# jnbraun/bcnn

Measured on AMD Instinct MI355X. Metric: images/sec fwd+bwd, higher is better.
Workload: dtype f32; 1 GPU; ResNet-18 224x224 (BASELINE configs[2]), N=128 per GPU, fwd+bwd+SGD through bcnn_net C API; CIFAR-example topology + ImageNet stem, fc-1000; batch_per_gpu=128, global_batch=128, parallelism=dp1, comm=none (one rank)

## Files before the change

### bcnn_amd/_lib.py

```python
import ctypes as C
import os
import subprocess

_HERE = os.path.dirname(os.path.abspath(__file__))
LIB_PATH = os.environ.get("BCNN_HIP_LIB", os.path.join(_HERE, "lib", "libbcnn_hip.so"))
CSRC = os.path.join(_HERE, "csrc")

vp, i, f, sz, u64 = C.c_void_p, C.c_int, C.c_float, C.c_size_t, C.c_uint64

SIGNATURES = {
    "bcnn_hip_device_count": (i, []),
    "bcnn_hip_set_device": (None, [i]),
    "bcnn_hip_get_device": (i, []),
    "bcnn_hip_device_name": (C.c_char_p, []),
    "bcnn_hip_malloc_f32": (vp, [sz]),
    "bcnn_hip_malloc_i32": (vp, [sz]),
    "bcnn_hip_free": (None, [vp]),
    "bcnn_hip_memcpy_h2d": (None, [vp, vp, sz]),
    "bcnn_hip_memcpy_d2h": (None, [vp, vp, sz]),
    "bcnn_hip_memcpy_d2d": (None, [vp, vp, sz]),
    "bcnn_hip_fill_f32": (None, [vp, sz, f]),
    "bcnn_hip_sync": (None, []),
    "bcnn_hip_stream_create": (vp, []),
    "bcnn_hip_stream_destroy": (None, [vp]),
    "bcnn_hip_set_stream": (None, [vp]),
    "bcnn_hip_get_stream": (vp, []),
    "bcnn_hip_event_create": (vp, []),
    "bcnn_hip_event_destroy": (None, [vp]),
    "bcnn_hip_event_record": (None, [vp]),
    "bcnn_hip_event_sync": (None, [vp]),
    "bcnn_hip_event_elapsed_ms": (f, [vp, vp]),
    "bcnn_hip_profile_enable": (None, [i]),
    "bcnn_hip_profile_reset": (None, []),
    "bcnn_hip_profile_num_classes": (i, []),
    "bcnn_hip_profile_class_name": (C.c_char_p, [i]),
    "bcnn_hip_profile_read": (None, [i, C.POINTER(C.c_double), C.POINTER(C.c_longlong), C.POINTER(C.c_double), C.POINTER(C.c_double)]),
    "bcnn_hip_profile_read_useful_flops": (C.c_double, [i]),
    "bcnn_hip_conv_side_stream_mode": (i, [i]),
    "bcnn_hip_conv_side_join": (None, []),
    "bcnn_hip_trace_enable": (None, [i]),
    "bcnn_hip_trace_read": (C.c_size_t, [C.c_char_p, C.c_size_t]),
    "bcnn_hip_axpy": (None, [sz, f, vp, vp]),
    "bcnn_hip_scal": (None, [sz, f, vp]),
    "bcnn_hip_copy_f32": (None, [sz, vp, vp]),
    "bcnn_hip_add_bias": (None, [vp, vp, i, i, i]),
    "bcnn_hip_grad_bias": (None, [vp, vp, i, i, i]),
    "bcnn_hip_scales": (None, [vp, vp, i, i, i]),
    "bcnn_hip_grad_scales": (None, [vp, vp, i, i, i, vp]),
    "bcnn_hip_gemm": (None, [i, i, i, i, i, f, vp, i, vp, i, f, vp, i]),
    "bcnn_hip_im2col": (None, [vp, i, i, i, i, i, i, vp]),
    "bcnn_hip_col2im": (None, [vp, i, i, i, i, i, i, vp]),
    "bcnn_hip_activation_forward": (None, [vp, sz, i, vp, i, i]),
    "bcnn_hip_activation_backward": (None, [vp, vp, sz, i, vp, vp, i, i]),
    "bcnn_hip_batchnorm_forward": (None, [vp] * 10 + [i, i, i, i, i]),
    "bcnn_hip_batchnorm_backward": (None, [vp, vp, vp, i] + [vp] * 9 + [i, i, i]),
    "bcnn_hip_conv_workspace_size": (sz, [i] * 9),
    "bcnn_hip_conv_forward": (None, [vp, vp, vp, vp] + [i] * 10 + [vp, i, vp, vp, vp, vp, vp, vp, vp, i]),
    "bcnn_hip_conv_forward_bf16": (i, [vp, vp, vp, vp] + [i] * 10 + [vp, i, vp, vp, vp, vp, vp, vp, vp, i]),
    "bcnn_hip_conv_backward": (None, [vp] * 8 + [i] * 10 + [vp, vp, i] + [vp] * 8 + [vp, sz]),
    "bcnn_hip_maxpool_forward": (None, [vp, vp, vp] + [i] * 8),
    "bcnn_hip_maxpool_backward": (None, [vp, vp, vp] + [i] * 9),
    "bcnn_hip_avgpool_forward": (None, [vp, vp, i, i, i, i]),
    "bcnn_hip_avgpool_backward": (None, [vp, vp, i, i, i, i]),
    "bcnn_hip_depthwise_forward": (None, [vp, vp, vp, vp] + [i] * 8),
    "bcnn_hip_depthwise_backward": (None, [vp] * 7 + [i] * 9),
    "bcnn_hip_depthwise_stats_size": (sz, [i] * 7),
    "bcnn_hip_depthwise_forward_stats": (i, [vp, vp, vp, vp] + [i] * 8 + [vp, sz]),
    "bcnn_hip_batchnorm_forward_stats": (None, [vp] * 10 + [i, i, i, i, i, vp, i]),
    "bcnn_hip_batchnorm_forward_stats_only": (None, [vp] * 7 + [i, i, i, vp, i]),
    "bcnn_hip_conv_bnfold_fusable": (i, [i] * 5), "bcnn_hip_conv_set_input_bnfold": (None, [vp] * 4),
    "bcnn_hip_depthwise_bn_fusable": (i, [i] * 8),
    "bcnn_hip_batchnorm_backward_sums": (None, [vp] * 9 + [i, i, i]),
    "bcnn_hip_depthwise_backward_bn": (None, [vp] * 7 + [i] * 9 + [vp] * 5),
    "bcnn_hip_batchnorm_backward_apply": (None, [vp] * 8 + [i, i, i]),
    "bcnn_hip_depthwise_bnin_fusable": (i, [i] * 9),
    "bcnn_hip_conv_bnsums_size": (sz, [i] * 4),
    "bcnn_hip_conv_backward_bnsums": (i, [vp] * 8 + [i] * 10 + [vp, vp, i] + [vp] * 8 + [vp, sz] + [vp, vp, vp, sz]),
    "bcnn_hip_batchnorm_backward_finalize": (None, [vp, i] + [vp] * 6 + [i]),
    "bcnn_hip_depthwise_forward_bnin": (i, [vp, vp, vp, vp] + [i] * 8 + [vp, sz] + [vp] * 4 + [i]),
    "bcnn_hip_depthwise_backward_bnin": (None, [vp] * 7 + [i] * 9 + [vp] * 4 + [i]),
    "bcnn_hip_depthwise_backward_bn_bnin": (None, [vp] * 7 + [i] * 9 + [vp] * 5 + [vp] * 4 + [i]),
    "bcnn_hip_conv_residual_fusable": (i, [i, i, i, i, vp, vp, vp]),
    "bcnn_hip_conv_forward_residual": (None, [vp, vp, vp] + [i] * 9 + [vp] * 7 + [sz, i, vp]),
    "bcnn_hip_conv_backward_residual": (None, [vp] * 7 + [i] * 9 + [vp] * 7 + [vp, sz, vp, vp, i, vp, vp, sz]),
    "bcnn_hip_batchnorm_apply": (None, [vp] * 6 + [i, i, i, i]),
    "bcnn_hip_conv_prepack": (None, [vp, i, i]),
    "bcnn_hip_maxpool_forward_bn_keep": (None, [vp, vp, vp] + [i] * 8 + [vp] * 4 + [i, vp]),
    "bcnn_hip_maxpool_bn_backward_fusable": (i, [i] * 9 + [vp] * 4),
    "bcnn_hip_maxpool_bn_backward": (None, [vp] * 5 + [i] * 8 + [vp] * 8 + [i]),
    "bcnn_hip_conv_backward_bn_done": (None, [vp] * 5 + [i] * 9 + [vp, sz]),
    "bcnn_hip_depthwise_insums_size": (sz, [i] * 7),
    "bcnn_hip_depthwise_backward_bnin_sums": (i, [vp] * 7 + [i] * 9 + [vp] * 5 + [vp] * 4 + [i] + [vp, sz]),
    "bcnn_hip_conv_backward_presummed": (i, [vp] * 8 + [i] * 10 + [vp, vp, i] + [vp] * 8 + [vp, sz] + [vp, i] + [vp, vp, vp, sz]),
    "bcnn_hip_conv_prepack_reset": (None, []),
    "bcnn_hip_conv_prepack_discard": (None, []),
    "bcnn_hip_maxpool_bn_fusable": (i, [i] * 9 + [vp]),
    "bcnn_hip_conv_forward_stats_only": (None, [vp, vp, vp] + [i] * 9 + [vp] * 6),
    "bcnn_hip_maxpool_forward_bn": (None, [vp, vp, vp] + [i] * 8 + [vp] * 4 + [i]),
    "bcnn_hip_sgd_update": (None, [vp, vp, vp, vp, sz, sz, i, f, f, f]),
    "bcnn_hip_sgd_update_chunks": (None, [vp, i, i, f, f, f]),
    "bcnn_hip_zero_chunks": (None, [vp, i]),
    "bcnn_hip_adam_update": (None, [vp, vp, vp, vp, vp, vp, sz, sz, i, i, f, f, f, f, f]),
    "bcnn_hip_eltwise_forward": (None, [vp, vp, vp, sz, sz, i]),
    "bcnn_hip_eltwise_backward": (None, [vp, vp, vp, vp, sz, sz, i, i]),
    "bcnn_hip_cost_metric": (None, [i, vp, vp, vp, i, i, vp]),
    "bcnn_hip_axpy_strided": (None, [i, f, vp, vp] + [i] * 11),
    "bcnn_hip_add_rowvec": (None, [vp, vp, i, i]),
    "bcnn_hip_softmax_forward": (None, [vp, vp, i, i, i]),
    "bcnn_hip_concat_forward": (None, [i, vp, vp, vp, i, i]),
    "bcnn_hip_concat_backward": (None, [i, vp, vp, vp, i, i]),
    "bcnn_hip_upsample_forward": (None, [vp, vp, i, i, i, i, i]),
    "bcnn_hip_upsample_backward": (None, [vp, vp, i, i, i, i, i]),
    "bcnn_hip_yolo_activate": (None, [vp, vp, i, i, i, i, i]),
    "bcnn_hip_yolo_nms_capacity": (i, []),
    "bcnn_hip_yolo_detect_result_words": (sz, [i, i, i]),
    "bcnn_hip_yolo_detect_batch": (i, [vp, i, i, vp, i, i, i, i, f, i, f, i, i, vp]),
    "bcnn_hip_fill_images": (i, [vp, i, i, i, i, i, vp, vp, vp, vp, i, f, i, f, f, f]),
    "bcnn_hip_deconv_workspace_size": (sz, [i] * 8),
    "bcnn_hip_deconv_forward": (None, [vp, vp, vp, vp] + [i] * 9),
    "bcnn_hip_deconv_backward": (None, [vp] * 7 + [i] * 9 + [vp, sz]),
    "bcnn_hip_lrn_forward": (None, [vp, vp] + [i] * 5 + [f] * 3),
    "bcnn_hip_lrn_backward": (None, [vp, vp, vp] + [i] * 5 + [f] * 3 + [i]),
    "bcnn_hip_dropout_forward": (None, [vp, sz, f, u64, u64]),
    "bcnn_hip_dropout_backward": (None, [vp, sz, f, u64, u64]),
    "bcnn_hip_lifted_struct_workspace_size": (sz, [i, i]),
    "bcnn_hip_lifted_struct_forward": (None, [vp, vp, vp, i, i, f, i, vp, vp]),
    "bcnn_hip_lifted_struct_backward": (None, [vp, i, i, f, vp]),
    "bcnn_hip_comm_init": (None, [i, i, C.c_char_p]),
    "bcnn_hip_comm_destroy": (None, []),
    "bcnn_hip_comm_retain": (None, []),
    "bcnn_hip_rendezvous_publish": (i, [C.c_char_p, vp, sz, i]),
    "bcnn_hip_rendezvous_fetch": (i, [C.c_char_p, vp, sz, i, i]),
    "bcnn_hip_comm_world": (i, []),
    "bcnn_hip_comm_rank": (i, []),
    "bcnn_hip_allreduce_sum": (None, [vp, sz]),
    "bcnn_hip_broadcast": (None, [vp, sz, i]),
    "bcnn_hip_comm_join": (None, []),
}

_lib = None


def build(verbose=False):
    out = None if verbose else subprocess.DEVNULL
    subprocess.check_call(["make", "-C", CSRC, "-j8"], stdout=out)
    return LIB_PATH


def load():
    global _lib
    if _lib is not None:
        return _lib
    try:
        import torch
    except ImportError:
        pass
    if not os.path.exists(LIB_PATH):
        raise RuntimeError(
            "bcnn_amd: %s is missing -- build it with `python -c 'import __graft_entry__ as g; g.build()'` "
            "(there is no CPU fallback)" % LIB_PATH)
    lib = C.CDLL(LIB_PATH)
    for name, (res, args) in SIGNATURES.items():
        fn = getattr(lib, name)
        fn.restype = res
        fn.argtypes = args
    _lib = lib
    return lib


def declared_symbols():
    import re
    hdr = os.path.join(os.path.dirname(_HERE), "include", "bcnn_hip.h")
    text = open(hdr).read()
    text = re.sub(r"/\*.*?\*/", "", text, flags=re.S)
    return sorted(set(re.findall(r"\b(bcnn_hip_[a-z0-9_]+)\s*\(", text)))
```

### bcnn_amd/csrc/common.h

```cpp
#pragma once
#include <hip/hip_runtime.h>

#include <cstdio>
#include <cstdlib>

#include "../../include/bcnn_hip.h"

#define HIP_CHECK(expr)                                                                        \
    do {                                                                                       \
        hipError_t _e = (expr);                                                                \
        if (_e != hipSuccess) {                                                                \
            fprintf(stderr, "[bcnn_hip] %s:%d: %s failed: %s\n", __FILE__, __LINE__, #expr,    \
                    hipGetErrorString(_e));                                                    \
            exit((int)_e);                                                                     \
        }                                                                                      \
    } while (0)

#define KERNEL_CHECK() HIP_CHECK(hipGetLastError())

#ifdef BCNN_HIP_EXPERIMENT
#define BCNN_EXP_ENV(name) getenv(name)
#else
#define BCNN_EXP_ENV(name) ((const char*)nullptr)
#endif

namespace bcnn_hip {

hipStream_t current_stream();
void set_current_stream(hipStream_t st);

constexpr int kMaxDevices = 64;
int current_device();

enum ScratchSlot {
    SCRATCH_REDUCE,
    SCRATCH_BN_CONSTS,
    SCRATCH_FOLD_ROWCONST,
    SCRATCH_COL,
    SCRATCH_DMA,
    SCRATCH_DMA_DW,
    SCRATCH_WINO,
    SCRATCH_WINO_DW,
    SCRATCH_WINO43_U,
    SCRATCH_WINO43_TAIL,
    SCRATCH_WFUSED_U,
    SCRATCH_WFUSED_TAIL,
    SCRATCH_W43FF_U,
    SCRATCH_W43FF_TAIL,
    SCRATCH_DETECT,
    SCRATCH_IMAGES,
    SCRATCH_SLOTS
};
float* scratch(ScratchSlot slot, size_t floats);
inline float4* scratch_f4(ScratchSlot slot, size_t n) { return reinterpret_cast<float4*>(scratch(slot, n * 4)); }

void activation_backward_grad_bias(const float* y, float* dy, float* dbias, int n, int c, int hw, int act);

enum KClass { K_CONV_FWD = 0, K_CONV_DW, K_CONV_DX, K_BN_FWD, K_BN_BWD, K_POOL, K_ELTWISE_ACT, K_GEMM, K_SGD,
              K_DEPTHWISE_FWD, K_DEPTHWISE_BWD,
              K_CONV_FWD_WINO, K_CONV_DX_WINO, K_CONV_DW_WINO,
              K_CONV_FWD_WINO43, K_CONV_DX_WINO43,
              K_CONV_DW_WINO43,
              K_NUM };
struct KTimer {
    int idx;
    KTimer(int cls, double flops, double bytes, double useful_flops = -1.0);
    ~KTimer();
};

extern thread_local bool g_trace_on;
void trace_kernel_slow(const char* name);
inline void trace_kernel(const char* name) { if (g_trace_on) trace_kernel_slow(name); }

constexpr int kWave = 64;
constexpr int kCUs = 256;
constexpr int kXCDs = 8;

inline int ceil_div(long long a, long long b) { return (int)((a + b - 1) / b); }

#ifndef STREAM_GRID_PER_CU
#define STREAM_GRID_PER_CU 8
#endif
inline int stream_grid(size_t work_items, int block) {
    size_t need = (work_items + block - 1) / block;
    size_t cap = (size_t)kCUs * STREAM_GRID_PER_CU;
    if (need < 1) need = 1;
    return (int)(need < cap ? need : cap);
}

#ifdef __HIPCC__
__device__ __forceinline__ int xcd_remap(int bid, int nblk) {
    const int q = nblk / kXCDs, r = nblk % kXCDs;
    const int xcd = bid % kXCDs, idx = bid / kXCDs;
    const int base = (xcd < r) ? xcd * (q + 1) : r * (q + 1) + (xcd - r) * q;
    return base + idx;
}

__device__ __forceinline__ float wave_sum(float v) {
#pragma unroll
    for (int off = 32; off > 0; off >>= 1) v += __shfl_down(v, off, 64);
    return v;
}

__device__ __forceinline__ float wave_sum_dpp(float v) {
    v += __builtin_bit_cast(float, __builtin_amdgcn_update_dpp(0, __builtin_bit_cast(int, v), 0xB1, 0xf, 0xf, false));
    v += __builtin_bit_cast(float, __builtin_amdgcn_update_dpp(0, __builtin_bit_cast(int, v), 0x4E, 0xf, 0xf, false));
    v += __builtin_bit_cast(float, __builtin_amdgcn_update_dpp(0, __builtin_bit_cast(int, v), 0x141, 0xf, 0xf, false));
    v += __builtin_bit_cast(float, __builtin_amdgcn_update_dpp(0, __builtin_bit_cast(int, v), 0x140, 0xf, 0xf, false));
    v += __builtin_bit_cast(float, __builtin_amdgcn_update_dpp(0, __builtin_bit_cast(int, v), 0x142, 0xa, 0xf, false));
    v += __builtin_bit_cast(float, __builtin_amdgcn_update_dpp(0, __builtin_bit_cast(int, v), 0x143, 0xc, 0xf, false));
    return v;
}

__device__ __forceinline__ float block_sum(float v, float* red) {
    v = wave_sum(v);
    const int lane = threadIdx.x & 63, wid = threadIdx.x >> 6;
    __syncthreads();
    if (lane == 0) red[wid] = v;
    __syncthreads();
    float t = 0.f;
    if (threadIdx.x == 0) {
        const int nw = (blockDim.x + 63) >> 6;
        for (int i = 0; i < nw; ++i) t += red[i];
    }
    return t;
}

__device__ __forceinline__ float act_fwd(float x, int act, float slope) {
    switch (act) {
        case BCNN_HIP_ACT_TANH: {
            const float t = 2 * x;
            const double e = exp((double)t);
            return (float)(e - 1) / ((float)e + 1);
        }
        case BCNN_HIP_ACT_RELU: return x * (float)(x > 0);
        case BCNN_HIP_ACT_LRELU: return x > 0 ? x : 0.1f * x;
        case BCNN_HIP_ACT_RAMP: return x * (float)(x > 0) + 0.1f * x;
        case BCNN_HIP_ACT_SOFTPLUS: return (float)log((double)(1.0f + (float)exp((double)x)));
        case BCNN_HIP_ACT_ABS: return fabsf(x);
        case BCNN_HIP_ACT_CLAMP: return (x < 0) ? 0.f : ((x > 1) ? 1.f : x);
        case BCNN_HIP_ACT_LOGISTIC: return 1.0f / (1.0f + (float)exp((double)(-x)));
        case BCNN_HIP_ACT_PRELU: return x > 0 ? x : slope * x;
        default: return x;
    }
}

__host__ __device__ __forceinline__ bool act_is_cheap(int act) {
    return act != BCNN_HIP_ACT_TANH && act != BCNN_HIP_ACT_SOFTPLUS && act != BCNN_HIP_ACT_LOGISTIC;
}
__device__ __forceinline__ float act_fwd_cheap(float x, int act, float slope) {
    switch (act) {
        case BCNN_HIP_ACT_RELU: return x * (float)(x > 0);
        case BCNN_HIP_ACT_LRELU: return x > 0 ? x : 0.1f * x;
        case BCNN_HIP_ACT_RAMP: return x * (float)(x > 0) + 0.1f * x;
        case BCNN_HIP_ACT_ABS: return fabsf(x);
        case BCNN_HIP_ACT_CLAMP: return (x < 0) ? 0.f : ((x > 1) ? 1.f : x);
        case BCNN_HIP_ACT_PRELU: return x > 0 ? x : slope * x;
        default: return x;
    }
}
__device__ __forceinline__ float act_bwd_cheap(float y, int act, float slope) {
    switch (act) {
        case BCNN_HIP_ACT_TANH: return 1 - y * y;
        case BCNN_HIP_ACT_RELU: return (float)(y > 0);
        case BCNN_HIP_ACT_LRELU: return y > 0 ? 1.0f : 0.1f;
        case BCNN_HIP_ACT_RAMP: return (float)(y > 0) + 0.1f;
        case BCNN_HIP_ACT_ABS: return y >= 0 ? 1.0f : -1.0f;
        case BCNN_HIP_ACT_CLAMP: return (float)(y > 0.0f && y < 1.0f);
        case BCNN_HIP_ACT_LOGISTIC: return (1 - y) * y;
        case BCNN_HIP_ACT_PRELU: return y > 0 ? 1.0f : slope;
        default: return 1.0f;
    }
}
__host__ __device__ __forceinline__ bool act_bwd_is_cheap(int act) { return act != BCNN_HIP_ACT_SOFTPLUS; }

__device__ __forceinline__ float act_bwd_factor(float y, int act, float slope) {
    switch (act) {
        case BCNN_HIP_ACT_TANH: return 1 - y * y;
        case BCNN_HIP_ACT_RELU: return (float)(y > 0);
        case BCNN_HIP_ACT_LRELU: return y > 0 ? 1.0f : 0.1f;
        case BCNN_HIP_ACT_RAMP: return (float)(y > 0) + 0.1f;
        case BCNN_HIP_ACT_SOFTPLUS: return 1.0f / (1.0f + (float)exp((double)(-y)));
        case BCNN_HIP_ACT_ABS: return y >= 0 ? 1.0f : -1.0f;
        case BCNN_HIP_ACT_CLAMP: return (float)(y > 0.0f && y < 1.0f);
        case BCNN_HIP_ACT_LOGISTIC: return (1 - y) * y;
        case BCNN_HIP_ACT_PRELU: return y > 0 ? 1.0f : slope;
        default: return 1.0f;
    }
}
#endif

}
```

### bcnn_amd/csrc/conv.hip

```cpp
#include "batchnorm.h"
#include "conv_paths.h"
#include <algorithm>
#include <cstring>
#include <vector>

namespace bcnn_hip {
static thread_local BnFold g_fold_pending = {nullptr, nullptr, nullptr, nullptr};
static BnFold take_fold() {
    const BnFold f = g_fold_pending;
    g_fold_pending = BnFold{nullptr, nullptr, nullptr, nullptr};
    return f;
}
static bool bnfold_shape_ok(const ConvShape& s) {
    return s.ksz == 1 && s.stride == 1 && s.pad == 0 && s.groups == 1 && conv_dma_fwd_wanted(s) &&
           conv_dw_dma_workspace_floats(s) > 0;
}
__global__ __launch_bounds__(256) void bnfold_rowconst_kernel(const float* __restrict__ w, const BnFold fold, int F, int C,
                                                              float* __restrict__ rowc) {
    const int f = blockIdx.x * 4 + (threadIdx.x >> 6), lane = threadIdx.x & 63;
    if (f >= F) return;
    double acc = 0.0;
    for (int c = lane; c < C; c += 64) {
        float bv = fold.bias[c];
        if (bv == 1.0f) bv = 0.f;
        const float b = bv - fold.mean[c] * bnfold_a(fold.var, fold.scales, c);
        acc += (double)w[(size_t)f * C + c] * (double)b;
    }
#pragma unroll
    for (int o = 32; o > 0; o >>= 1) acc += __shfl_xor(acc, o);
    if (lane == 0) rowc[f] = (float)acc;
}
static float* fold_rowconst(const BnFold& fold, const float* w, int C, int F) {
    float* rowc = scratch(SCRATCH_FOLD_ROWCONST, (size_t)F);
    bnfold_rowconst_kernel<<<ceil_div(F, 4), 256, 0, current_stream()>>>(w, fold, F, C, rowc);
    KERNEL_CHECK();
    return rowc;
}


struct SideStream {
    hipStream_t stream = nullptr;
    hipEvent_t ready = nullptr, done = nullptr;
    bool pending = false;
};
static thread_local SideStream g_side[kMaxDevices];
static thread_local int g_side_mode = 0;
bool conv_side_stream_deferred() { return g_side_mode == 2; }
static SideStream* side_stream() {
    SideStream& ss = g_side[current_device()];
    if (ss.stream == nullptr) {
        int prio_lo = 0, prio_hi = 0;
        HIP_CHECK(hipDeviceGetStreamPriorityRange(&prio_lo, &prio_hi));
        HIP_CHECK(hipStreamCreateWithPriority(&ss.stream, hipStreamNonBlocking, BCNN_EXP_ENV("BCNN_HIP_SIDE_PRIO_SAME") ? prio_hi : prio_lo));
        HIP_CHECK(hipEventCreateWithFlags(&ss.ready, hipEventDisableTiming));
        HIP_CHECK(hipEventCreateWithFlags(&ss.done, hipEventDisableTiming));
    }
    return &ss;
}

struct PrepackEntry {
    const float* w;
    int kind, mode;
    float* buf;
    size_t cap, floats;
    unsigned long long epoch;
    bool fresh;
};
struct PrepackStore {
    std::vector<PrepackEntry> entries;
    unsigned long long epoch = 0;
    int dev = -1;
    void* table_dev[PREPACK_KINDS][2] = {{nullptr, nullptr}, {nullptr, nullptr}};
    size_t table_cap[PREPACK_KINDS][2] = {{0, 0}, {0, 0}};
    std::vector<char> table_host[PREPACK_KINDS][2];
};
static thread_local PrepackStore g_prepack;

float* prepack_take(const float* w, int kind, int mode, size_t floats) {
    PrepackStore& st = g_prepack;
    for (PrepackEntry& e : st.entries)
        if (e.w == w && e.kind == kind && e.mode == mode && e.fresh && e.epoch == st.epoch && e.floats == floats) {
            e.fresh = false;
            return e.buf;
        }
    return nullptr;
}

static void prepack_free_all(PrepackStore& st) {
    HIP_CHECK(hipDeviceSynchronize());
    for (PrepackEntry& e : st.entries)
        if (e.buf) HIP_CHECK(hipFree(e.buf));
    st.entries.clear();
    for (int k = 0; k < PREPACK_KINDS; ++k)
        for (int m = 0; m < 2; ++m) {
            if (st.table_dev[k][m]) HIP_CHECK(hipFree(st.table_dev[k][m]));
            st.table_dev[k][m] = nullptr;
            st.table_cap[k][m] = 0;
            st.table_host[k][m].clear();
        }
}

static PrepackEntry* prepack_entry(PrepackStore& st, const float* w, int kind, int mode, size_t floats) {
    PrepackEntry* e = nullptr;
    for (PrepackEntry& c : st.entries)
        if (c.w == w && c.kind == kind && c.mode == mode) { e = &c; break; }
    if (!e) {
        st.entries.push_back(PrepackEntry{w, kind, mode, nullptr, 0, 0, 0, false});
        e = &st.entries.back();
    }
    if (e->cap < floats) {
        if (e->buf) {
            HIP_CHECK(hipStreamSynchronize(current_stream()));
            HIP_CHECK(hipFree(e->buf));
        }
        HIP_CHECK(hipMalloc((void**)&e->buf, floats * sizeof(float)));
        e->cap = floats;
    }
    e->floats = floats;
    e->epoch = st.epoch;
    e->fresh = true;
    return e;
}

static const void* prepack_table(PrepackStore& st, int kind, int mode, const void* jobs, size_t bytes) {
    std::vector<char>& host = st.table_host[kind][mode];
    if (host.size() == bytes && memcmp(host.data(), jobs, bytes) == 0) return st.table_dev[kind][mode];
    HIP_CHECK(hipStreamSynchronize(current_stream()));
    if (st.table_cap[kind][mode] < bytes) {
        if (st.table_dev[kind][mode]) HIP_CHECK(hipFree(st.table_dev[kind][mode]));
        HIP_CHECK(hipMalloc(&st.table_dev[kind][mode], bytes * 2));
        st.table_cap[kind][mode] = bytes * 2;
    }
    HIP_CHECK(hipMemcpy(st.table_dev[kind][mode], jobs, bytes, hipMemcpyHostToDevice));
    host.assign((const char*)jobs, (const char*)jobs + bytes);
    return st.table_dev[kind][mode];
}

enum ConvGate { GATE_NONE, GATE_WINDOW, GATE_DMA, GATE_SMALLC_DX, GATE_COUNT };
static bool gate_open(ConvGate g) {
    static const bool off[GATE_COUNT] = {false, BCNN_EXP_ENV("BCNN_HIP_NO_WINDOW") != nullptr,
                                         BCNN_EXP_ENV("BCNN_HIP_NO_DMA") != nullptr,
                                         BCNN_EXP_ENV("BCNN_HIP_NO_SMALLC_DX") != nullptr};
    return !off[g];
}
struct ConvPack {
    bool (*wino)(const ConvShape& s, int dx_mode, WinoPackJob* job, size_t* floats);
    bool (*igemm)(const ConvShape& s, int dx_mode, IgemmPackJob* job, size_t* floats);
};
constexpr ConvPack kNoPack = {nullptr, nullptr};
template <class Call>
struct ConvFamily {
    bool (*wanted)(const ConvShape& s, int raw);
    bool (*usable)(const Call& c);
    void (*run)(const Call& c);
    ConvPack pack;
    ConvGate gate;
};
static const ConvFamily<ConvFwdCall> kConvFwdFamilies[] = {
    {conv_window_fwd_wanted, nullptr, conv_forward_window, kNoPack, GATE_WINDOW},
    {conv_stem_fwd_wanted, nullptr, conv_forward_stem, kNoPack, GATE_WINDOW},
    {conv_direct_fwd_wanted, nullptr, conv_forward_direct, kNoPack, GATE_NONE},
    {conv_winograd43_fwd_wanted, conv_winograd43_fwd_usable, conv_forward_winograd43, {wino43_pack_plan, nullptr}, GATE_NONE},
    {conv_winograd_fused_fwd_wanted, nullptr, conv_forward_winograd_fused, {wino_fused_pack_plan, nullptr}, GATE_NONE},
    {conv_winograd_fwd_wanted, nullptr, conv_forward_winograd, kNoPack, GATE_NONE},
    {conv_large_wanted, nullptr, conv_forward_large, kNoPack, GATE_NONE},
    {conv_dma_fwd_wanted, nullptr, conv_forward_dma_timed, {nullptr, dma_pack_plan}, GATE_DMA},
    {conv_small_c_fwd_wanted, nullptr, conv_forward_small_c, kNoPack, GATE_DMA},
    {[](const ConvShape&, int) { return true; }, nullptr, conv_forward_igemm, kNoPack, GATE_NONE},
};
static const ConvFamily<ConvDxCall> kConvDxFamilies[] = {
    {conv_winograd43_dx_wanted, conv_winograd43_dx_usable, conv_backward_data_winograd43, {wino43_pack_plan, nullptr}, GATE_NONE},
    {conv_winograd_fused_dx_wanted, nullptr, conv_backward_data_winograd_fused, {wino_fused_pack_plan, nullptr}, GATE_NONE},
    {conv_winograd_dx_wanted, nullptr, conv_backward_data_winograd, kNoPack, GATE_NONE},
    {conv_large_wanted, nullptr, conv_backward_data_large, kNoPack, GATE_NONE},
    {conv_small_c_dx_wanted, nullptr, conv_backward_data_small_c, kNoPack, GATE_SMALLC_DX},
    {conv_dma_dx_wanted, nullptr, conv_backward_data_dma, {nullptr, dma_pack_plan}, GATE_DMA},
    {[](const ConvShape&, int) { return true; }, nullptr, conv_backward_data_igemm, kNoPack, GATE_NONE},
};

template <class Call, size_t R>
static void conv_run_first(const ConvFamily<Call> (&rows)[R], const Call& c, int raw) {
    for (const ConvFamily<Call>& fam : rows)
        if (gate_open(fam.gate) && fam.wanted(c.s, raw) && (!fam.usable || fam.usable(c))) {
            fam.run(c);
            return;
        }
}
template <class Call, size_t R>
static ConvPack conv_planned_pack(const ConvFamily<Call> (&rows)[R], const ConvShape& s) {
    for (const ConvFamily<Call>& fam : rows)
        if (gate_open(fam.gate) && fam.wanted(s, 1)) return fam.pack;
    return kNoPack;
}

static void conv_fwd_any(const float* x, const float* w, const float* bias, const float* slopes, float* y,
                         const ConvShape& s, int act, int raw, ConvStats* stats = nullptr, bool bf16 = false) {
    if (stats) stats->splits = 0;
    if (s.total_q <= 0 || s.Mg == 0) return;
    if (bf16) conv_forward_bf16(x, w, bias, slopes, y, s, act, raw, stats);
    else conv_run_first(kConvFwdFamilies, ConvFwdCall{x, w, bias, slopes, y, s, act, raw, stats}, raw);
}

static void conv_dx_any(const float* w, const float* dy, float* dx, const ConvShape& s, DxBnSums* bs) {
    if (bs) bs->splits = 0;
    if (s.total_p == 0 || s.Cg == 0) return;
    conv_run_first(kConvDxFamilies, ConvDxCall{w, dy, dx, s, bs}, 0);
}

struct DwFamily {
    size_t (*workspace_floats)(const ConvShape& s);
    bool (*run)(const float* x, const float* dy, float* dw, float* dbias, const ConvShape& s, float* workspace,
                size_t workspace_floats, bool* bias_done);
    ConvGate gate;
};
static const DwFamily kDwFamilies[] = {
    {conv_dw_window_workspace_floats, conv_backward_weights_window, GATE_WINDOW},
    {conv_dw_stem_workspace_floats, conv_backward_weights_stem, GATE_WINDOW},
    {conv_dw_direct_workspace_floats, conv_backward_weights_direct, GATE_NONE},
    {conv_dw_winograd43_workspace_floats, conv_backward_weights_winograd43, GATE_NONE},
    {conv_dw_winograd_fused_workspace_floats, conv_backward_weights_winograd_fused, GATE_NONE},
    {conv_dw_winograd_workspace_floats, conv_backward_weights_winograd, GATE_NONE},
    {conv_dw_dma_workspace_floats, conv_backward_weights_dma_timed, GATE_DMA},
    {conv_dw_small_c_workspace_floats, conv_backward_weights_small_c, GATE_DMA},
    {conv_dw_large_workspace_floats, conv_backward_weights_large, GATE_NONE},
    {conv_dw_workspace_floats, conv_backward_weights, GATE_NONE},
};
}

using namespace bcnn_hip;

extern "C" {

void bcnn_hip_conv_prepack(const bcnn_hip_conv_desc* layers, int count, int data_gradient) {
    PrepackStore& st = g_prepack;
    int dev = 0;
    HIP_CHECK(hipGetDevice(&dev));
    if (st.dev != dev) {
        if (st.dev >= 0) prepack_free_all(st);
        st.dev = dev;
    }
    ++st.epoch;
    (void)take_fold();
    const int mode = data_gradient ? 1 : 0;
    std::vector<WinoPackJob> wj;
    std::vector<IgemmPackJob> ij;
    int wmax = 0, imax = 0;
    for (int i = 0; i < count; ++i) {
        const bcnn_hip_conv_desc& d = layers[i];
        if (!d.w_d || d.groups <= 0 || d.n <= 0) continue;
        const ConvShape s = make_conv_shape(d.n, d.c, d.h, d.w, d.f, d.k, d.stride, d.pad, d.groups);
        if (s.total_q <= 0 || s.Mg == 0 || s.Cg == 0) continue;
        const ConvPack pack = mode ? conv_planned_pack(kConvDxFamilies, s) : conv_planned_pack(kConvFwdFamilies, s);
        WinoPackJob w1;
        IgemmPackJob i1;
        memset(&w1, 0, sizeof(w1));
        memset(&i1, 0, sizeof(i1));
        size_t floats = 0;
        if (pack.wino && pack.wino(s, mode, &w1, &floats)) {
            PrepackEntry* e = prepack_entry(st, d.w_d, PREPACK_WINO, mode, floats);
            w1.w = d.w_d; w1.u = e->buf;
            if (w1.blocks > wmax) wmax = w1.blocks;
            wj.push_back(w1);
        }
        if (pack.igemm && pack.igemm(s, mode, &i1, &floats)) {
            PrepackEntry* e = prepack_entry(st, d.w_d, PREPACK_IGEMM, mode, floats);
            i1.w = d.w_d; i1.at = e->buf;
            const int blocks = i1.gx * i1.gy * i1.gz;
            if (blocks > imax) imax = blocks;
            ij.push_back(i1);
        }
    }
    if (!wj.empty()) {
        const void* t = prepack_table(st, PREPACK_WINO, mode, wj.data(), wj.size() * sizeof(WinoPackJob));
        wino_fused_pack_launch((const WinoPackJob*)t, (int)wj.size(), wmax);
    }
    if (!ij.empty()) {
        const void* t = prepack_table(st, PREPACK_IGEMM, mode, ij.data(), ij.size() * sizeof(IgemmPackJob));
        dma_pack_launch((const IgemmPackJob*)t, (int)ij.size(), imax);
    }
}

void bcnn_hip_conv_prepack_discard(void) { ++g_prepack.epoch; }

void bcnn_hip_conv_prepack_reset(void) {
    PrepackStore& st = g_prepack;
    if (st.dev < 0) return;
    prepack_free_all(st);
    ++st.epoch;
}

size_t bcnn_hip_conv_workspace_size(int n, int c, int h, int w, int f, int k, int stride, int pad, int groups) {
    const ConvShape s = make_conv_shape(n, c, h, w, f, k, stride, pad, groups);
    size_t m = 0;
    for (const DwFamily& fam : kDwFamilies) m = std::max(m, fam.workspace_floats(s));
    return m;
}

static void conv_forward_impl(const float* x, const float* w, const float* bias, float* y, int n, int c, int h,
                              int wd, int f, int k, int stride, int pad, int groups, int act, const float* slopes,
                              int batch_norm, float* run_mean, float* run_var, const float* scales,
                              float* saved_mean, float* saved_var, float* x_norm, float* bn_workspace, int mode,
                              const BnResidual* res, float* res_out, bool stats_only = false, bool bf16 = false) {
    const ConvShape s = make_conv_shape(n, c, h, wd, f, k, stride, pad, groups);
    const BnFold fold = take_fold();
    if (fold.mean && (!batch_norm || mode != BCNN_HIP_MODE_TRAIN || !bnfold_shape_ok(s))) {
        fprintf(stderr, "[bcnn_hip] conv forward: a batch-norm fold was announced for a layer that cannot take it (ask "
                        "bcnn_hip_conv_bnfold_fusable)\n");
        exit(1);
    }
    if (!batch_norm) {
        if (act_is_cheap(act)) {
            conv_fwd_any(x, w, bias, slopes, y, s, act, 0, nullptr, bf16);
        } else {
            conv_fwd_any(x, w, bias, slopes, y, s, BCNN_HIP_ACT_NONE, 0, nullptr, bf16);
            bcnn_hip_activation_forward(y, (size_t)n * f * s.OHOW, act, slopes, s.OHOW, f);
        }
        return;
    }
    float* raw = (bn_workspace && mode != BCNN_HIP_MODE_PREDICT) ? bn_workspace : y;
    ConvStats st;
    st.partials = nullptr; st.splits = 0; st.capacity = 0;
    static const int fuse_stats = BCNN_EXP_ENV("BCNN_HIP_NO_FUSED_STATS") ? 0 : 1;
    if (fuse_stats && mode == BCNN_HIP_MODE_TRAIN && s.total_q < 0x7fffffffLL) {
        const long long tiles = (long long)n * ((s.OH + 1) / 2) * ((s.OW + 1) / 2);
        const long long slots_gemm = ceil_div(s.total_q, 64), slots_wino = 2 * ceil_div(tiles, 64);
        st.capacity = (size_t)f * (size_t)(slots_gemm > slots_wino ? slots_gemm : slots_wino) * 2;
        st.partials = scratch(SCRATCH_REDUCE, st.capacity);
    }
    const float* mean_shift = nullptr;
    if (fold.mean) {
        trace_kernel("bnfold:fwd");
        mean_shift = fold_rowconst(fold, w, c, f);
        KTimer kt(K_CONV_FWD, conv_gemm_flops(s), conv_gemm_bytes(s));
        ConvStats* stp = st.partials ? &st : nullptr;
        if (!conv_forward_dma(x, w, nullptr, nullptr, raw, s, BCNN_HIP_ACT_NONE, 1, stp, &fold)) {
            fprintf(stderr, "[bcnn_hip] conv forward: the LDS-DMA GEMM refused a folded layer\n");
            exit(1);
        }
    } else {
        conv_fwd_any(x, w, nullptr, nullptr, raw, s, BCNN_HIP_ACT_NONE, 1, st.partials ? &st : nullptr, bf16);
    }
    const int fused_act = (act == BCNN_HIP_ACT_PRELU) ? BCNN_HIP_ACT_NONE : act;
    (void)x_norm;
    batchnorm_forward_impl(raw, res ? res_out : y, run_mean, run_var, scales, bias, saved_mean, saved_var, nullptr, raw, n, f,
                           s.OHOW, mode, fused_act, &st, res, stats_only, mean_shift);
    if (stats_only) return;
    if (act == BCNN_HIP_ACT_PRELU)
        bcnn_hip_activation_forward(y, (size_t)n * f * s.OHOW, act, slopes, s.OHOW, f);
}

int bcnn_hip_conv_bnfold_fusable(int n, int c, int h, int wd, int f) {
    if (n <= 0 || c <= 0 || h <= 0 || wd <= 0 || f <= 0) return 0;
    return bnfold_shape_ok(make_conv_shape(n, c, h, wd, f, 1, 1, 0, 1)) ? 1 : 0;
}

void bcnn_hip_conv_set_input_bnfold(const float* mean, const float* var, const float* scales, const float* bias) {
    g_fold_pending = BnFold{mean, var, scales, bias};
}

void bcnn_hip_conv_forward(const float* x, const float* w, const float* bias, float* y, int n, int c, int h,
                           int wd, int f, int k, int stride, int pad, int groups, int act, const float* slopes,
                           int batch_norm, float* run_mean, float* run_var, const float* scales,
                           float* saved_mean, float* saved_var, float* x_norm, float* bn_workspace, int mode) {
    conv_forward_impl(x, w, bias, y, n, c, h, wd, f, k, stride, pad, groups, act, slopes, batch_norm, run_mean, run_var,
                      scales, saved_mean, saved_var, x_norm, bn_workspace, mode, nullptr, nullptr);
}

int bcnn_hip_conv_forward_bf16(const float* x, const float* w, const float* bias, float* y, int n, int c, int h,
                               int wd, int f, int k, int stride, int pad, int groups, int act, const float* slopes,
                               int batch_norm, float* run_mean, float* run_var, const float* scales,
                               float* saved_mean, float* saved_var, float* x_norm, float* bn_workspace, int mode) {
    if (mode != BCNN_HIP_MODE_PREDICT && mode != BCNN_HIP_MODE_VALID) return 0;
    conv_forward_impl(x, w, bias, y, n, c, h, wd, f, k, stride, pad, groups, act, slopes, batch_norm, run_mean, run_var,
                      scales, saved_mean, saved_var, x_norm, bn_workspace, mode, nullptr, nullptr, false,
                      true);
    return 1;
}

void bcnn_hip_conv_forward_stats_only(const float* x, const float* w, const float* bias, int n, int c, int h, int wd, int f,
                                      int k, int stride, int pad, int groups, float* run_mean, float* run_var,
                                      const float* scales, float* saved_mean, float* saved_var, float* bn_workspace) {
    conv_forward_impl(x, w, bias, nullptr, n, c, h, wd, f, k, stride, pad, groups, BCNN_HIP_ACT_NONE, nullptr, 1,
                      run_mean, run_var, scales, saved_mean, saved_var, nullptr, bn_workspace, BCNN_HIP_MODE_TRAIN, nullptr,
                      nullptr, true);
}

int bcnn_hip_conv_residual_fusable(int batch_norm, int act, int res_act, int mode, const float* bn_workspace,
                                   const float* res, const float* res_out) {
    auto al16 = [](const void* p) { return (reinterpret_cast<uintptr_t>(p) & 15) == 0; };
    return batch_norm && mode == BCNN_HIP_MODE_TRAIN && bn_workspace && act == BCNN_HIP_ACT_NONE && act_is_cheap(res_act) &&
           act_bwd_is_cheap(res_act) && res_act != BCNN_HIP_ACT_PRELU && al16(res) && al16(res_out) && al16(bn_workspace);
}

void bcnn_hip_conv_forward_residual(const float* x, const float* w, const float* bias, int n, int c, int h, int wd, int f,
                                    int k, int stride, int pad, int groups, float* run_mean, float* run_var,
                                    const float* scales, float* saved_mean, float* saved_var, float* bn_workspace,
                                    const float* res, size_t res_count, int res_act, float* res_out) {
    BnResidual r{res, res_count, res_act};
    conv_forward_impl(x, w, bias, nullptr, n, c, h, wd, f, k, stride, pad, groups, BCNN_HIP_ACT_NONE, nullptr, 1,
                      run_mean, run_var, scales, saved_mean, saved_var, nullptr, bn_workspace, BCNN_HIP_MODE_TRAIN, &r,
                      res_out);
}

struct ConvResidualBwd {
    const float* out;
    const float* dout;
    const float* res;
    float* dres;
    size_t res_count;
    int act;
};
static void conv_backward_impl(const float* x, const float* w, const float* bias, const float* y, float* dy, float* dx,
                               float* dw, float* dbias, int n, int c, int h, int wd, int f, int k, int stride, int pad,
                               int groups, int act, const float* slopes, float* dslopes, int batch_norm,
                               const float* scales, float* dscales, const float* saved_mean,
                               const float* saved_var, float* dmean, float* dvar, const float* x_norm,
                               const float* bn_workspace, float* workspace, size_t workspace_elems,
                               const ConvResidualBwd* rb, DxBnSums* bs = nullptr, const float* own_sums = nullptr,
                               int own_splits = 0, bool bn_done = false) {
    const ConvShape s = make_conv_shape(n, c, h, wd, f, k, stride, pad, groups);
    const size_t ysize = (size_t)n * f * s.OHOW;
    const BnFold fold = take_fold();
    if (fold.mean && (!batch_norm || !bnfold_shape_ok(s))) {
        fprintf(stderr, "[bcnn_hip] conv backward: a batch-norm fold was announced for a layer that cannot take it\n");
        exit(1);
    }
    if (rb) {
        batchnorm_backward_residual(rb->dout, rb->out, rb->act, rb->res, rb->dres, rb->res_count, dy, scales, dscales, dbias,
                                    bias, saved_mean, saved_var, dmean, dvar, bn_workspace, n, f, s.OHOW);
    } else if (batch_norm && bn_done) {
    } else if (batch_norm) {
        int fused_act = act;
        if (act == BCNN_HIP_ACT_PRELU) {
            bcnn_hip_activation_backward(y, dy, ysize, act, slopes, dslopes, s.OHOW, f);
            fused_act = BCNN_HIP_ACT_NONE;
        }
        (void)x_norm;
        if (own_sums && own_splits > 0 && fused_act == act && act_bwd_is_cheap(act))
            batchnorm_backward_presummed(dy, y, act, scales, dscales, dbias, saved_mean, saved_var, dmean, dvar, bn_workspace, n,
                                         f, s.OHOW, bias, own_sums, own_splits);
        else
            batchnorm_backward_impl(dy, nullptr, y, fused_act, scales, dscales, dbias, saved_mean, saved_var, dmean, dvar,
                                    bn_workspace, n, f, s.OHOW, bias);
    } else {
        bcnn_hip_activation_backward(y, dy, ysize, act, slopes, dslopes, s.OHOW, f);
    }
    static const int side_env = BCNN_EXP_ENV("BCNN_HIP_SIDE_STREAM") ? 1 : 0;
    const int side_mode = g_side_mode ? g_side_mode : side_env;
    SideStream* side = (side_mode == 2 || (side_mode == 1 && dx)) ? side_stream() : nullptr;
    hipStream_t main_stream = current_stream();
    if (side) {
        HIP_CHECK(hipEventRecord(side->ready, main_stream));
        HIP_CHECK(hipStreamWaitEvent(side->stream, side->ready, 0));
        set_current_stream(side->stream);
    }
    bool bias_done = false;
    if (fold.mean) {
        trace_kernel("bnfold:dw");
        KTimer kt(K_CONV_DW, conv_gemm_flops(s), conv_gemm_bytes(s));
        if (!conv_backward_weights_dma(x, dy, dw, s, workspace, workspace_elems, &fold)) {
            fprintf(stderr, "[bcnn_hip] conv backward: the LDS-DMA weight-gradient kernel refused a folded layer\n");
            exit(1);
        }
    } else {
        for (const DwFamily& fam : kDwFamilies)
            if (gate_open(fam.gate) &&
                fam.run(x, dy, dw, batch_norm ? nullptr : dbias, s, workspace, workspace_elems, &bias_done))
                break;
    }
    if (side) {
        HIP_CHECK(hipEventRecord(side->done, side->stream));
        set_current_stream(main_stream);
    }
    if (!batch_norm && !bias_done) bcnn_hip_grad_bias(dbias, dy, n, f, s.OHOW);
    if (dx) conv_dx_any(w, dy, dx, s, bs);
    else if (bs) bs->splits = 0;
    if (side) {
        if (side_mode == 2) side->pending = true;
        else HIP_CHECK(hipStreamWaitEvent(main_stream, side->done, 0));
    }
}

int bcnn_hip_conv_side_stream_mode(int mode) {
    const int prev = g_side_mode;
    if (mode >= 0 && mode <= 2) g_side_mode = mode;
    return prev;
}

void bcnn_hip_conv_side_join(void) {
    SideStream& ss = g_side[current_device()];
    if (!ss.pending) return;
    ss.pending = false;
    HIP_CHECK(hipStreamWaitEvent(current_stream(), ss.done, 0));
}

void bcnn_hip_conv_backward(const float* x, const float* w, const float* bias, const float* y, float* dy, float* dx,
                            float* dw, float* dbias, int n, int c, int h, int wd, int f, int k, int stride, int pad,
                            int groups, int act, const float* slopes, float* dslopes, int batch_norm,
                            const float* scales, float* dscales, const float* saved_mean,
                            const float* saved_var, float* dmean, float* dvar, const float* x_norm,
                            const float* bn_workspace, float* workspace, size_t workspace_elems) {
    conv_backward_impl(x, w, bias, y, dy, dx, dw, dbias, n, c, h, wd, f, k, stride, pad, groups, act, slopes, dslopes,
                       batch_norm, scales, dscales, saved_mean, saved_var, dmean, dvar, x_norm, bn_workspace, workspace,
                       workspace_elems, nullptr);
}

size_t bcnn_hip_conv_bnsums_size(int n, int c, int h, int wd) {
    return (size_t)c * (size_t)ceil_div((long long)n * h * wd, 64) * 2;
}

int bcnn_hip_conv_backward_bnsums(const float* x, const float* w, const float* bias, const float* y, float* dy, float* dx,
                                  float* dw, float* dbias, int n, int c, int h, int wd, int f, int k, int stride, int pad,
                                  int groups, int act, const float* slopes, float* dslopes, int batch_norm,
                                  const float* scales, float* dscales, const float* saved_mean, const float* saved_var,
                                  float* dmean, float* dvar, const float* x_norm, const float* bn_workspace,
                                  float* workspace, size_t workspace_elems, const float* prev_y, const float* prev_mean,
                                  float* sums, size_t sums_floats) {
    DxBnSums bs{prev_y, prev_mean, sums, sums_floats, 0};
    conv_backward_impl(x, w, bias, y, dy, dx, dw, dbias, n, c, h, wd, f, k, stride, pad, groups, act, slopes, dslopes,
                       batch_norm, scales, dscales, saved_mean, saved_var, dmean, dvar, x_norm, bn_workspace, workspace,
                       workspace_elems, nullptr, (sums && prev_y && prev_mean) ? &bs : nullptr);
    return bs.splits;
}

void bcnn_hip_conv_backward_bn_done(const float* x, const float* w, float* dy, float* dx, float* dw, int n, int c, int h, int wd,
                                    int f, int k, int stride, int pad, int groups, float* workspace, size_t workspace_elems) {
    conv_backward_impl(x, w, nullptr, nullptr, dy, dx, dw, nullptr, n, c, h, wd, f, k, stride, pad, groups, BCNN_HIP_ACT_NONE,
                       nullptr, nullptr, 1, nullptr, nullptr, nullptr, nullptr, nullptr, nullptr, nullptr, nullptr, workspace,
                       workspace_elems, nullptr, nullptr, nullptr, 0, true);
}

int bcnn_hip_conv_backward_presummed(const float* x, const float* w, const float* bias, const float* y, float* dy, float* dx,
                                     float* dw, float* dbias, int n, int c, int h, int wd, int f, int k, int stride, int pad,
                                     int groups, int act, const float* slopes, float* dslopes, int batch_norm,
                                     const float* scales, float* dscales, const float* saved_mean, const float* saved_var,
                                     float* dmean, float* dvar, const float* x_norm, const float* bn_workspace,
                                     float* workspace, size_t workspace_elems, const float* own_sums, int own_splits,
                                     const float* prev_y, const float* prev_mean, float* prev_sums, size_t prev_sums_floats) {
    DxBnSums bs{prev_y, prev_mean, prev_sums, prev_sums_floats, 0};
    conv_backward_impl(x, w, bias, y, dy, dx, dw, dbias, n, c, h, wd, f, k, stride, pad, groups, act, slopes, dslopes,
                       batch_norm, scales, dscales, saved_mean, saved_var, dmean, dvar, x_norm, bn_workspace, workspace,
                       workspace_elems, nullptr, (prev_sums && prev_y && prev_mean) ? &bs : nullptr, own_sums, own_splits);
    return bs.splits;
}

void bcnn_hip_conv_backward_residual(const float* x, const float* w, const float* bias, float* dy, float* dx, float* dw,
                                     float* dbias, int n, int c, int h, int wd, int f, int k, int stride, int pad,
                                     int groups, const float* scales, float* dscales, const float* saved_mean,
                                     const float* saved_var, float* dmean, float* dvar, const float* bn_workspace,
                                     float* workspace, size_t workspace_elems, const float* res_out,
                                     const float* dres_out, int res_act, const float* res, float* dres, size_t res_count) {
    ConvResidualBwd rb{res_out, dres_out, res, dres, res_count, res_act};
    conv_backward_impl(x, w, bias, nullptr, dy, dx, dw, dbias, n, c, h, wd, f, k, stride, pad, groups, BCNN_HIP_ACT_NONE,
                       nullptr, nullptr, 1, scales, dscales, saved_mean, saved_var, dmean, dvar, nullptr, bn_workspace,
                       workspace, workspace_elems, &rb);
}

}
```

### bcnn_amd/csrc/conv_paths.h

```cpp
#pragma once
#include "conv_common.h"

namespace bcnn_hip {

struct ConvFwdCall {
    const float *x, *w, *bias, *slopes;
    float* y;
    ConvShape s;
    int act, raw;
    ConvStats* stats;
};
struct ConvDxCall {
    const float *w, *dy;
    float* dx;
    ConvShape s;
    DxBnSums* bs;
};

bool conv_window_fwd_wanted(const ConvShape& s, int raw);
void conv_forward_window(const ConvFwdCall& c);
bool conv_stem_fwd_wanted(const ConvShape& s, int raw);
void conv_forward_stem(const ConvFwdCall& c);
bool conv_direct_fwd_wanted(const ConvShape& s, int raw);
void conv_forward_direct(const ConvFwdCall& c);
bool conv_winograd43_fwd_wanted(const ConvShape& s, int raw);
bool conv_winograd43_fwd_usable(const ConvFwdCall& c);
void conv_forward_winograd43(const ConvFwdCall& c);
bool conv_winograd43_dx_wanted(const ConvShape& s, int);
bool conv_winograd43_dx_usable(const ConvDxCall& c);
void conv_backward_data_winograd43(const ConvDxCall& c);
bool conv_winograd_fused_fwd_wanted(const ConvShape& s, int raw);
void conv_forward_winograd_fused(const ConvFwdCall& c);
bool conv_winograd_fused_dx_wanted(const ConvShape& s, int);
void conv_backward_data_winograd_fused(const ConvDxCall& c);
bool conv_winograd_fwd_wanted(const ConvShape& s, int raw);
void conv_forward_winograd(const ConvFwdCall& c);
bool conv_winograd_dx_wanted(const ConvShape& s, int);
void conv_backward_data_winograd(const ConvDxCall& c);
bool conv_large_wanted(const ConvShape& s, int raw = 0);
void conv_forward_large(const ConvFwdCall& c);
void conv_backward_data_large(const ConvDxCall& c);
bool conv_forward_bf16(const float* x, const float* w, const float* bias, const float* slopes, float* y, const ConvShape& s,
                       int act, int raw, ConvStats* stats);
bool conv_dma_fwd_wanted(const ConvShape& s, int raw = 0);
bool conv_forward_dma(const float* x, const float* w, const float* bias, const float* slopes, float* y, const ConvShape& s,
                      int act, int raw, ConvStats* stats, const BnFold* fold = nullptr);
void conv_forward_dma_timed(const ConvFwdCall& c);
bool conv_dma_dx_wanted(const ConvShape& s, int);
void conv_backward_data_dma(const ConvDxCall& c);
bool conv_small_c_fwd_wanted(const ConvShape& s, int raw = 0);
void conv_forward_small_c(const ConvFwdCall& c);
float* conv_small_c_padded_input(const float* x, const ConvShape& s, size_t extra_floats, float** extra, int for_dw);
void conv_forward_igemm(const ConvFwdCall& c);
void conv_backward_data_igemm(const ConvDxCall& c);
bool conv_small_c_dx_wanted(const ConvShape& s, int);
void conv_backward_data_small_c(const ConvDxCall& c);
void conv_prefetch_input(const float* x, const ConvShape& s, float* sink);

size_t conv_dw_window_workspace_floats(const ConvShape& s);
bool conv_backward_weights_window(const float* x, const float* dy, float* dw, float* dbias, const ConvShape& s,
                                  float* workspace, size_t workspace_floats, bool* bias_done);
size_t conv_dw_stem_workspace_floats(const ConvShape& s);
bool conv_backward_weights_stem(const float* x, const float* dy, float* dw, float* dbias, const ConvShape& s,
                                float* workspace, size_t workspace_floats, bool* bias_done);
size_t conv_dw_direct_workspace_floats(const ConvShape& s);
bool conv_backward_weights_direct(const float* x, const float* dy, float* dw, float* dbias, const ConvShape& s,
                                  float* workspace, size_t workspace_floats, bool* bias_done);
size_t conv_dw_winograd43_workspace_floats(const ConvShape& s);
bool conv_backward_weights_winograd43(const float* x, const float* dy, float* dw, float* dbias, const ConvShape& s,
                                      float* workspace, size_t workspace_floats, bool* bias_done);
size_t conv_dw_winograd_fused_workspace_floats(const ConvShape& s);
bool conv_backward_weights_winograd_fused(const float* x, const float* dy, float* dw, float* dbias, const ConvShape& s,
                                          float* workspace, size_t workspace_floats, bool* bias_done);
size_t conv_dw_winograd_workspace_floats(const ConvShape& s);
bool conv_backward_weights_winograd(const float* x, const float* dy, float* dw, float* dbias, const ConvShape& s,
                                    float* workspace, size_t workspace_floats, bool* bias_done);
size_t conv_dw_dma_workspace_floats(const ConvShape& s);
bool conv_backward_weights_dma_timed(const float* x, const float* dy, float* dw, float* dbias, const ConvShape& s,
                                     float* workspace, size_t workspace_floats, bool* bias_done);
size_t conv_dw_small_c_workspace_floats(const ConvShape& s);
bool conv_backward_weights_small_c(const float* x, const float* dy, float* dw, float* dbias, const ConvShape& s,
                                   float* workspace, size_t workspace_floats, bool* bias_done);
size_t conv_dw_large_workspace_floats(const ConvShape& s);
bool conv_backward_weights_large(const float* x, const float* dy, float* dw, float* dbias, const ConvShape& s,
                                 float* workspace, size_t workspace_floats, bool* bias_done);
size_t conv_dw_workspace_floats(const ConvShape& s);
bool conv_backward_weights(const float* x, const float* dy, float* dw, float* dbias, const ConvShape& s,
                           float* workspace, size_t workspace_floats, bool* bias_done);
bool conv_backward_weights_dma(const float* x, const float* dy, float* dw, const ConvShape& s, float* workspace,
                               size_t workspace_floats, const BnFold* fold = nullptr);
void conv_dw_direct_finalize(const float* partials, int nparts, int groups, int Mg, int K, int MP, int bias_col, float* dw,
                             float* dbias);

void wino43b_run(const float* src, const float* w, float* dst, const ConvShape& s, int dx_mode, ConvStats* stats);
int wino43b_stats_slots(const ConvShape& s);
void wino43b_pack_dims(int J, int M, int* Jpad, int* Mpad);

}
```

### bcnn_amd/csrc/conv_window.hip

```cpp
#include "conv_paths.h"
#include "lds_dma.h"

#include <mutex>

#ifndef WABL_FWD_R
#define WABL_FWD_R 4
#endif
#ifndef WABL_NBUF
#define WABL_NBUF 2
#endif
#ifndef WABL_NW
#define WABL_NW 8
#endif
#ifndef STEM_R
#define STEM_R 8
#endif
#ifndef STEM_WAVES
#define STEM_WAVES 2
#endif
#ifndef ROWS_TM
#define ROWS_TM 1
#endif
#ifndef ROWS_NS
#define ROWS_NS 2
#endif
#ifndef ROWS_INTERLEAVE
#define ROWS_BURST 1
#endif
#ifndef DY_DMA_PLAIN
#define DY_DMA_NT 1
#endif
#ifndef STORE_AUX
#define STORE_AUX 2
#endif

namespace bcnn_hip {

constexpr int kWinOrg = 4;

enum { WD_ELEM = 0, WD_ROW = 1, WD_PLANE = 2, WD_NONE = 3 };
struct WinStep { int c, kr, kc, kind, second; };
template <int CG>
struct WinSteps {
    static constexpr int N = (CG * 9 + 1) / 2;
    WinStep st[N];
    constexpr WinSteps() : st{} {
        int n = 0;
        for (int c = 0; c < CG; ++c)
            for (int kr = 0; kr < 3; ++kr) st[n++] = WinStep{c, kr, 0, WD_ELEM, 1};
        for (int c = 0; c < CG; ++c) st[n++] = WinStep{c, 0, 2, WD_ROW, 1};
        for (int c = 0; c + 1 < CG; c += 2) st[n++] = WinStep{c, 2, 2, WD_PLANE, 1};
        if (CG & 1) st[n++] = WinStep{CG - 1, 2, 2, WD_NONE, 0};
    }
};

struct ConvWindowFwdArgs {
    const float* x;
    const float* w;
    const float* bias;
    const float* slopes;
    float* y;
    ConvShape s;
    int act, add_bias;
    int strips;
    int* sched;
};

template <int CG, int R, int PITCH>
__device__ __forceinline__ void window_fill_dma(unsigned lds_base, rsrc_i4 rx, const ConvShape& s, unsigned img_chan0, int oh0, int lane,
                                                bool valid) {
    constexpr int ROWS = R + 2, P4 = PITCH / 4, NP = CG * ROWS * P4;
#pragma unroll 4
    for (int k = 0; k < (NP + 63) / 64; ++k) {
        const int i = k * 64 + lane;
        const int c = i / (ROWS * P4), rem = i - c * (ROWS * P4);
        const int rr = rem / P4, j = rem - rr * P4;
        const int ih = oh0 - s.pad + rr, iw0 = 4 * j - kWinOrg;
        const bool ok = valid && i < NP && (unsigned)ih < (unsigned)s.H && (unsigned)iw0 < (unsigned)s.W;
        const unsigned off = ok ? ((img_chan0 + (unsigned)c) * (unsigned)s.HW + (unsigned)(ih * s.W + iw0)) * 4u : kOOB;
        dma_row_x4(rx, lds_base + (unsigned)k * 1024u, off, 0);
    }
}

template <int CG, int R, int PITCH, int TM, int ACTM, int NW>
__global__ __launch_bounds__(64 * (NW + 1), 2) void conv_fwd_window_kernel(const ConvWindowFwdArgs a) {
    constexpr int ROWS = R + 2, PLANE = ROWS * PITCH;
    constexpr int NBUF = WABL_NBUF;
    constexpr int WINSZ = (CG * PLANE + 255) & ~255;
    constexpr WinSteps<CG> steps{};
    constexpr int NT = WinSteps<CG>::N;
    constexpr bool SPARE = (CG & 1) != 0;
    constexpr int KS = SPARE ? NT : NT + 1;
    __shared__ __attribute__((aligned(1024))) float win_all[NBUF * WINSZ];
    __shared__ int next_unit[NBUF < 2 ? 2 : NBUF];
    const ConvShape& s = a.s;
    const int tid = threadIdx.x, lane = tid & 63;
    const int wid = __builtin_amdgcn_readfirstlane(tid >> 6);
    const int l31 = lane & 31, hi = lane >> 5;
    const int g = blockIdx.y;
    const rsrc_i4 rx = make_rsrc(a.x, (unsigned)((long long)s.N * s.C * s.HW * 4));
    const rsrc_i4 ry = make_rsrc(a.y, (unsigned)((long long)s.N * s.F * s.OHOW * 4));
    const int nunits = s.N * a.strips;
    if (wid == NW) {
        constexpr int NI = (CG * (R + 2) * (PITCH / 4) + 63) / 64;
        constexpr int D = NBUF - 1;
        static_assert((D - 1) * NI < 64, "vmcnt is a 6-bit counter");
        int unit = (int)blockIdx.x;
        int j = 0;
        for (int k = 0;; ++k) {
            for (; j <= k + D - 1; ++j) {
                const int n = unit / a.strips, strip = unit - n * a.strips;
                window_fill_dma<CG, R, PITCH>(lds_offset(win_all + (j % NBUF) * WINSZ), rx, s, (unsigned)(n * s.C + g * s.Cg), strip * R, lane,
                                              unit < nunits);
                if (lane == 0) next_unit[j % NBUF] = unit;
                if (unit < nunits) {
                    if (NBUF == 2 && a.sched) unit = (int)gridDim.x + __builtin_amdgcn_readfirstlane(lane == 0 ? atomicAdd(a.sched + 2 * g, 1) : 0);
                    else unit += (int)gridDim.x;
                }
            }
            dma_wait_n<(D - 1) * NI>();
            lds_barrier();
            if (__builtin_amdgcn_readfirstlane(next_unit[k % NBUF]) >= nunits) break;
        }
        dma_wait();
        if (NBUF == 2 && a.sched && lane == 0) {
            if (atomicAdd(a.sched + 2 * g + 1, 1) == (int)gridDim.x - 1) {
                a.sched[2 * g] = 0;
                a.sched[2 * g + 1] = 0;
            }
        }
        return;
    }
    const float* wg = a.w + (long long)g * s.Mg * s.K;
    float areg[TM][KS];
#pragma unroll
    for (int tm = 0; tm < TM; ++tm) {
        const int f = tm * 32 + l31;
        float bv = 0.f;
        if (a.add_bias && f < s.Mg) {
            bv = a.bias[g * s.Mg + f];
            if (bv == 1.0f) bv = 0.f;
        }
#pragma unroll
        for (int st = 0; st < NT; ++st) {
            const WinStep p = steps.st[st];
            int c = p.c, kr = p.kr, kc = p.kc;
            if (hi) {
                if (p.kind == WD_ELEM) kc += 1;
                else if (p.kind == WD_ROW) kr += 1;
                else if (p.kind == WD_PLANE) c += 1;
            }
            const int k = c * 9 + kr * 3 + kc;
            const bool ok = (!hi || p.second) && f < s.Mg;
            const float v = wg[ok ? (long long)f * s.K + k : 0];
            areg[tm][st] = ok ? v : ((hi && !p.second) ? bv : 0.f);
// ... 629 lines not shown
    int bias_col;
};

typedef float f32x4_t __attribute__((ext_vector_type(4)));
constexpr int kStemTapCols = 160;

template <int CG, int PD, int PX>
__global__ __launch_bounds__(512, 1) void conv_dw_stem_kernel(const ConvStemDwArgs a) {
    constexpr int XR = CG * 7;
    constexpr int DYS = 64 * PD, XS = XR * PX;
    constexpr int XREQ = (XR + 7) / 8, NREQ = 8 + XREQ;
    __shared__ __attribute__((aligned(16))) float lds[2 * DYS + 2 * XS + 16];
    float* cst = lds + 2 * DYS + 2 * XS;
    const ConvShape& s = a.s;
    const int tid = threadIdx.x, lane = tid & 63;
    const int wid = __builtin_amdgcn_readfirstlane(tid >> 6);
    const int l15 = lane & 15, kq = lane >> 4;
    const int fb = wid & 3, th = wid >> 2;
    const int g = blockIdx.y;
    const rsrc_i4 rx = make_rsrc(a.x, (unsigned)((long long)s.N * s.C * s.HW * 4));
    const rsrc_i4 rdy = make_rsrc(a.dy, (unsigned)((long long)s.N * s.F * s.OHOW * 4));

    for (int i = tid; i < 2 * DYS + 2 * XS; i += 512) lds[i] = 0.f;
    if (tid < 16) cst[tid] = tid < 8 ? 1.0f : 0.0f;
    __syncthreads();

    const int K = CG * 49;
    const unsigned a_lane = (unsigned)(((fb * 16 + l15) * PD + 4 * kq) * 4);
    unsigned b_lane[5], b_step[5];
#pragma unroll
    for (int b = 0; b < 5; ++b) {
        const int tap = (th * 5 + b) * 16 + l15;
        const int c = tap / 49, r49 = tap - c * 49, kr = r49 / 7, kc = r49 - kr * 7;
        const bool is_tap = tap < K;
        b_lane[b] = is_tap ? (unsigned)((2 * DYS + (c * 7 + kr) * PX + kc + (kWinOrg - s.pad) + 8 * kq) * 4)
                           : (unsigned)((2 * DYS + 2 * XS + ((tap == K && a.bias_col) ? 0 : 8)) * 4);
        b_step[b] = is_tap ? 1u : 0u;
    }
    const char* ldsb = reinterpret_cast<const char*>(lds);
    const unsigned lds0 = lds_offset(lds);
    const unsigned dma_lane = (unsigned)lane * 16u;
    const bool dy_lane_on = lane * 4 < s.OW, x_lane_on = lane * 4 < s.W;

    auto request = [&](int k, int n, int oh, int buf) {
        if (k < 8) {
            const int f = wid * 8 + k;
            const bool fok = f < s.Mg;
            const unsigned soff = __builtin_amdgcn_readfirstlane(
                fok ? ((unsigned)(n * s.F + g * s.Mg + f) * (unsigned)s.OHOW + (unsigned)(oh * s.OW)) * 4u : 0u);
            const unsigned dst = __builtin_amdgcn_readfirstlane(lds0 + (unsigned)((buf * DYS + f * PD) * 4));
            const unsigned voff = fok ? dma_lane : kOOB;
            if (dy_lane_on) dma_row_x4_nt(rdy, dst, voff, soff);
        } else {
            const int i0 = wid + 8 * (k - 8), i = i0 < XR ? i0 : XR - 1;
            const int c = i / 7, kr = i - c * 7;
            const int ih = 2 * oh - s.pad + kr;
            const bool ok = (unsigned)ih < (unsigned)s.H;
            const unsigned soff = __builtin_amdgcn_readfirstlane(
                ((unsigned)(n * s.C + g * s.Cg + c) * (unsigned)s.HW + (unsigned)((ok ? ih : 0) * s.W)) * 4u);
            const unsigned dst = __builtin_amdgcn_readfirstlane(lds0 + (unsigned)((2 * DYS + buf * XS + i * PX + kWinOrg) * 4));
            const unsigned voff = ok ? dma_lane : kOOB;
            if (x_lane_on) dma_row_x4(rx, dst, voff, soff);
        }
    };

    f32x4_t acc[5];
#pragma unroll
    for (int b = 0; b < 5; ++b) acc[b] = f32x4_t{0.f, 0.f, 0.f, 0.f};
    const int nwin = (s.OW + 15) >> 4;
    const int r0 = blockIdx.x * a.rows_per_block;
    int r1 = r0 + a.rows_per_block;
    if (r1 > a.total_rows) r1 = a.total_rows;

    if (r0 < r1) {
        const int n = r0 / s.OH, oh = r0 - n * s.OH;
        for (int k = 0; k < NREQ; ++k) request(k, n, oh, 0);
    }
    dma_wait();
    lds_barrier();
    for (int r = r0; r < r1; ++r) {
        const int buf = (r - r0) & 1;
        if (r + 1 < r1) {
            const int nn = (r + 1) / s.OH, noh = (r + 1) - nn * s.OH;
            for (int k = 0; k < NREQ; ++k) request(k, nn, noh, buf ^ 1);
        }
        unsigned va = a_lane + (unsigned)(buf * DYS * 4);
        unsigned vb[5];
#pragma unroll
        for (int b = 0; b < 5; ++b) vb[b] = b_lane[b] + b_step[b] * (unsigned)(buf * XS * 4);
        for (int w = 0; w < nwin; ++w) {
            const f32x4_t av = *reinterpret_cast<const f32x4_t*>(ldsb + va);
            float bv[5][4];
#pragma unroll
            for (int b = 0; b < 5; ++b)
#pragma unroll
                for (int e = 0; e < 4; ++e) bv[b][e] = *reinterpret_cast<const float*>(ldsb + vb[b] + 8 * e);
#pragma unroll
            for (int e = 0; e < 4; ++e)
#pragma unroll
                for (int b = 0; b < 5; ++b) acc[b] = __builtin_amdgcn_mfma_f32_16x16x4f32(av[e], bv[b][e], acc[b], 0, 0, 0);
            va += 64u;
#pragma unroll
            for (int b = 0; b < 5; ++b) vb[b] += b_step[b] * 128u;
        }
        dma_wait();
        lds_barrier();
    }
    float* out = a.partials + ((size_t)blockIdx.x * s.groups + g) * 64 * kStemTapCols;
#pragma unroll
    for (int b = 0; b < 5; ++b)
#pragma unroll
        for (int rr = 0; rr < 4; ++rr)
            out[(fb * 16 + 4 * kq + rr) * kStemTapCols + (th * 5 + b) * 16 + l15] = acc[b][rr];
}

__global__ __launch_bounds__(256) void conv_dw_stem_finalize_kernel(const float* __restrict__ partials, int nparts, int groups,
                                                                   int Mg, int K, int bias_col, float* __restrict__ dw,
                                                                   float* __restrict__ dbias) {
    __shared__ float red[16][17];
    const int kcols = K + (bias_col ? 1 : 0);
    const int total = groups * Mg * kcols;
    const int e = blockIdx.x * 16 + (threadIdx.x & 15), pl = threadIdx.x >> 4;
    float sum = 0.f;
    int g = 0, f = 0, k = 0;
    if (e < total) {
        k = e % kcols;
        const int t = e / kcols;
        f = t % Mg; g = t / Mg;
        for (int p = pl; p < nparts; p += 16) sum += partials[(((size_t)p * groups + g) * 64 + f) * kStemTapCols + k];
    }
    red[pl][threadIdx.x & 15] = sum;
    __syncthreads();
    if (pl == 0 && e < total) {
        float tot = 0.f;
#pragma unroll
        for (int i = 0; i < 16; ++i) tot += red[i][threadIdx.x & 15];
        if (k < K) dw[((size_t)g * Mg + f) * K + k] += tot;
        else dbias[g * Mg + f] += tot;
    }
}

static bool dw_stem_ok(const ConvShape& s) {
    return stem_ok(s) && (s.OW % 4) == 0 && ((s.OW + 15) & ~15) <= 120 && 2 * (((s.OW + 15) & ~15) - 1) + 7 + (kWinOrg - s.pad) <= 232;
}

static void dw_stem_plan(const ConvShape& s, int* rpb, int* blocks) {
    const int total = s.N * s.OH;
    int b = kCUs;
    if (b > total) b = total;
    *rpb = ceil_div(total, b);
    *blocks = ceil_div(total, *rpb);
}

size_t conv_dw_stem_workspace_floats(const ConvShape& s) {
    if (!dw_stem_ok(s)) return 0;
    int rpb, blocks;
    dw_stem_plan(s, &rpb, &blocks);
    return (size_t)blocks * s.groups * 64 * kStemTapCols;
}

bool conv_backward_weights_stem(const float* x, const float* dy, float* dw, float* dbias, const ConvShape& s, float* workspace,
                                size_t workspace_floats, bool* bias_done) {
    if (!dw_stem_ok(s)) return false;
    ConvStemDwArgs a;
    int blocks;
    dw_stem_plan(s, &a.rows_per_block, &blocks);
    const size_t need = (size_t)blocks * s.groups * 64 * kStemTapCols;
    conv_require_workspace(workspace, workspace_floats, need);
    KTimer kt(K_CONV_DW, conv_gemm_flops(s), conv_gemm_bytes(s));
    a.x = x; a.dy = dy; a.partials = workspace; a.s = s;
    a.total_rows = s.N * s.OH;
    a.bias_col = dbias ? 1 : 0;
    const dim3 grid((unsigned)blocks, (unsigned)s.groups);
    trace_kernel("conv_dw_stem_kernel");
    if (s.Cg == 1) conv_dw_stem_kernel<1, 120, 232><<<grid, 512, 0, current_stream()>>>(a);
    else if (s.Cg == 2) conv_dw_stem_kernel<2, 120, 232><<<grid, 512, 0, current_stream()>>>(a);
    else conv_dw_stem_kernel<3, 120, 232><<<grid, 512, 0, current_stream()>>>(a);
    KERNEL_CHECK();
    const int total = s.groups * s.Mg * (s.K + a.bias_col);
    conv_dw_stem_finalize_kernel<<<ceil_div(total, 16), 256, 0, current_stream()>>>(workspace, blocks, s.groups, s.Mg, s.K,
                                                                                    a.bias_col, dw, dbias);
    KERNEL_CHECK();
    *bias_done = dbias != nullptr;
    return true;
}

static bool dw_window_ok(const ConvShape& s) { return window_ok(s) && (s.OW % 8) == 0; }

static void dw_rows_plan(const ConvShape& s, int* rpb, int* blocks) {
    const int total = s.N * s.OH;
    const int fblocks = (s.Mg + 31) / 32;
#if ROWS_TM == 2
    int b = kCUs;
    (void)fblocks;
#else
    int b = ((window_pitch(s) == 232 && ROWS_NS == 2 ? 2 : 1) * kCUs) / fblocks;
#endif
    if (b < 1) b = 1;
    if (b > total) b = total;
    *rpb = ceil_div(total, b);
    *blocks = ceil_div(total, *rpb);
}

size_t conv_dw_window_workspace_floats(const ConvShape& s) {
    if (!dw_window_ok(s)) return 0;
    int rpb, blocks;
    dw_rows_plan(s, &rpb, &blocks);
    const int tm = (s.Mg <= 32) ? 1 : 2;
    return (size_t)blocks * s.groups * tm * 32 * 32;
}

bool conv_backward_weights_window(const float* x, const float* dy, float* dw, float* dbias, const ConvShape& s,
                                  float* workspace, size_t workspace_floats, bool* bias_done) {
    if (!dw_window_ok(s)) return false;
    ConvRowsDwArgs ra;
    int rblocks;
    dw_rows_plan(s, &ra.rows_per_block, &rblocks);
    const int tm = (s.Mg <= 32) ? 1 : 2;
    const size_t need = (size_t)rblocks * s.groups * tm * 32 * 32;
    conv_require_workspace(workspace, workspace_floats, need);
    KTimer kt(K_CONV_DW, conv_gemm_flops(s), conv_gemm_bytes(s));
    ra.x = x; ra.dy = dy; ra.partials = workspace; ra.s = s;
    ra.total_rows = s.N * s.OH;
    ra.bias_col = dbias ? 1 : 0;
    ra.mp = tm * 32;
    const int pitch = window_pitch(s);
    constexpr int RTM = ROWS_TM;
    const int wtm = tm < RTM ? tm : RTM;
    const dim3 rgrid((unsigned)rblocks, (unsigned)s.groups, (unsigned)(tm / wtm));
#define RLAUNCH2(CGv, PDv, PXv) do { if (wtm == 1) conv_dw_rows_kernel<CGv, PDv, PXv, 1><<<rgrid, 256, 0, current_stream()>>>(ra); \
                                     else conv_dw_rows_kernel<CGv, PDv, PXv, RTM><<<rgrid, 256 * RTM, 0, current_stream()>>>(ra); } while (0)
#ifndef ROWS_PX
#define ROWS_PX 232
#endif
#define RLAUNCH1(CGv) do { if (pitch == 232) RLAUNCH2(CGv, 228, ROWS_PX); else RLAUNCH2(CGv, 260, 264); } while (0)
    trace_kernel("conv_dw_rows_kernel");
    if (s.Cg == 1) RLAUNCH1(1);
    else if (s.Cg == 2) RLAUNCH1(2);
    else RLAUNCH1(3);
#undef RLAUNCH1
#undef RLAUNCH2
    KERNEL_CHECK();
    conv_dw_direct_finalize(workspace, rblocks, s.groups, s.Mg, s.K, tm * 32, ra.bias_col, dw, dbias);
    *bias_done = dbias != nullptr;
    return true;
}

}
```

### bcnn_amd/csrc/pool.hip

```cpp
#include <cfloat>

#include "batchnorm.h"
#include "bn_math.h"

namespace bcnn_hip {

__global__ __launch_bounds__(256) void maxpool_fwd_kernel(const float* __restrict__ x, float* __restrict__ y,
                                                          int* __restrict__ idx, int planes, int H, int W,
                                                          int OH, int OW, int size, int stride,
                                                          unsigned total) {
    const unsigned gstride = gridDim.x * blockDim.x;
    for (unsigned o = blockIdx.x * blockDim.x + threadIdx.x; o < total; o += gstride) {
        const unsigned j = o % (unsigned)OW, t = o / (unsigned)OW;
        const unsigned i = t % (unsigned)OH, plane = t / (unsigned)OH;
        const int base = (int)plane * H * W;
        float best = -FLT_MAX;
        int bi = -1;
        for (int r = 0; r < size; ++r) {
            const int hh = (int)i * stride + r;
            for (int q = 0; q < size; ++q) {
                const int ww = (int)j * stride + q;
                const int si = base + hh * W + ww;
                const bool ok = hh < H && ww < W;
                const float v = ok ? x[si] : -FLT_MAX;
// ... 109 lines not shown
    }
}

__global__ __launch_bounds__(256) void maxpool_bwd_kernel(const float* __restrict__ dy, const int* __restrict__ idx,
                                                          float* __restrict__ dx, int H, int W, int OH, int OW,
                                                          int size, int stride, unsigned total) {
    const unsigned gstride = gridDim.x * blockDim.x;
    for (unsigned s = blockIdx.x * blockDim.x + threadIdx.x; s < total; s += gstride) {
        const unsigned w = s % (unsigned)W, t = s / (unsigned)W;
        const unsigned h = t % (unsigned)H, plane = t / (unsigned)H;
        int i0 = ((int)h - size + stride) / stride; if ((int)h - size + 1 <= 0) i0 = 0;
        int j0 = ((int)w - size + stride) / stride; if ((int)w - size + 1 <= 0) j0 = 0;
        int i1 = (int)h / stride; if (i1 > OH - 1) i1 = OH - 1;
        int j1 = (int)w / stride; if (j1 > OW - 1) j1 = OW - 1;
        float acc = dx[s];
        bool hit = false;
        const int obase = (int)plane * OH * OW;
        for (int i = i0; i <= i1; ++i)
            for (int j = j0; j <= j1; ++j) {
                const int o = obase + i * OW + j;
                if (idx[o] == (int)s) { acc += dy[o]; hit = true; }
            }
        if (hit) dx[s] = acc;
    }
}

template <bool OVERWRITE>
__global__ __launch_bounds__(256) void maxpool_bwd_vec4_kernel(const float* __restrict__ dy, const int* __restrict__ idx,
                                                               float* __restrict__ dx, int H, int W, int OH, int OW,
                                                               int size, int stride) {
    const int W4 = W >> 2;
    const int t = blockIdx.x * 256 + threadIdx.x;
    const int plane = blockIdx.y;
    if (t >= H * W4) return;
    const int h = t / W4, w0 = (t - h * W4) * 4;
    const int s0 = (plane * H + h) * W + w0;
    int i0 = (h - size + stride) / stride; if (h - size + 1 <= 0) i0 = 0;
    int j0 = (w0 - size + stride) / stride; if (w0 - size + 1 <= 0) j0 = 0;
    int i1 = h / stride; if (i1 > OH - 1) i1 = OH - 1;
    int j1 = (w0 + 3) / stride; if (j1 > OW - 1) j1 = OW - 1;
    float4 v = OVERWRITE ? make_float4(0.f, 0.f, 0.f, 0.f) : *reinterpret_cast<const float4*>(dx + s0);
    bool hit = OVERWRITE;
    for (int i = i0; i <= i1; ++i) {
        const int o = (plane * OH + i) * OW;
        for (int j = j0; j <= j1; ++j) {
            const unsigned d = (unsigned)(idx[o + j] - s0);
            if (d < 4u) {
                const float g = dy[o + j];
                if (d == 0) v.x += g; else if (d == 1) v.y += g; else if (d == 2) v.z += g; else v.w += g;
                hit = true;
            }
        }
    }
    if (hit) *reinterpret_cast<float4*>(dx + s0) = v;
}

template <bool OVERWRITE>
__global__ __launch_bounds__(256) void maxpool_bwd_vec4_k3s2_kernel(const float* __restrict__ dy,
                                                                    const int* __restrict__ idx,
                                                                    float* __restrict__ dx, int H, int W, int OH,
                                                                    int OW) {
    const int W4 = W >> 2;
    const int t = blockIdx.x * 256 + threadIdx.x;
    const int plane = blockIdx.y;
    if (t >= H * W4) return;
    const int h = t / W4, w0 = (t - h * W4) * 4;
    const int s0 = (plane * H + h) * W + w0;
    const int i0 = h >= 2 ? (h - 1) >> 1 : 0, j0 = w0 >= 2 ? (w0 - 1) >> 1 : 0;
    int i1 = h >> 1; if (i1 > OH - 1) i1 = OH - 1;
    int j1 = (w0 + 3) >> 1; if (j1 > OW - 1) j1 = OW - 1;
    int id[2][3];
    float g[2][3];
    bool ok[2][3];
#pragma unroll
    for (int a = 0; a < 2; ++a)
#pragma unroll
        for (int b = 0; b < 3; ++b) {
            const int i = i0 + a, j = j0 + b;
            ok[a][b] = i <= i1 && j <= j1;
            const int o = (plane * OH + (i <= i1 ? i : i1)) * OW + (j <= j1 ? j : j1);
            id[a][b] = idx[o];
            g[a][b] = dy[o];
        }
    float4 v = OVERWRITE ? make_float4(0.f, 0.f, 0.f, 0.f) : *reinterpret_cast<const float4*>(dx + s0);
    bool hit = OVERWRITE;
#pragma unroll
    for (int a = 0; a < 2; ++a)
#pragma unroll
        for (int b = 0; b < 3; ++b) {
            const unsigned d = (unsigned)(id[a][b] - s0);
            if (ok[a][b] && d < 4u) {
                const float gg = g[a][b];
                if (d == 0) v.x += gg; else if (d == 1) v.y += gg; else if (d == 2) v.z += gg; else v.w += gg;
                hit = true;
            }
        }
    if (hit) *reinterpret_cast<float4*>(dx + s0) = v;
}

template <bool OVERWRITE>
__global__ __launch_bounds__(256) void maxpool_bwd_vec4_k3s2_pair_kernel(const float* __restrict__ dy,
                                                                         const int* __restrict__ idx,
                                                                         float* __restrict__ dx, int H, int W, int OH,
                                                                         int OW) {
    const int W4 = W >> 2;
    const int t = blockIdx.x * 256 + threadIdx.x;
    const int plane = blockIdx.y;
    const bool live = t < H * W4;
    const int tt = live ? t : 0;
    const int h = tt / W4, k = tt - h * W4, w0 = k * 4;
    const int s0 = (plane * H + h) * W + w0;
    const int i0 = h >= 2 ? (h - 1) >> 1 : 0;
    int i1 = h >> 1; if (i1 > OH - 1) i1 = OH - 1;
    const bool need_left = k > 0, fetch_left = need_left && (threadIdx.x & 63) == 0;
    int id[2][3];
    float g[2][3];
    bool ok[2];
#pragma unroll
    for (int a = 0; a < 2; ++a) {
        const int i = i0 + a;
        ok[a] = live && i <= i1;
        const int o = (plane * OH + (i <= i1 ? i : i1)) * OW + 2 * k;
        const int2 ip = *reinterpret_cast<const int2*>(idx + o);
        const float2 gp = *reinterpret_cast<const float2*>(dy + o);
        const int ie = idx[fetch_left ? o - 1 : o];
        const float ge = dy[fetch_left ? o - 1 : o];
        id[a][0] = __builtin_amdgcn_update_dpp(ie, ip.y, 0x138 , 0xf, 0xf, false);
        g[a][0] = __builtin_bit_cast(float, __builtin_amdgcn_update_dpp(__builtin_bit_cast(int, ge), __builtin_bit_cast(int, gp.y),
                                                                        0x138, 0xf, 0xf, false));
        id[a][1] = ip.x; g[a][1] = gp.x;
        id[a][2] = ip.y; g[a][2] = gp.y;
    }
    if (!live) return;
    float4 v = OVERWRITE ? make_float4(0.f, 0.f, 0.f, 0.f) : *reinterpret_cast<const float4*>(dx + s0);
    bool hit = OVERWRITE;
#pragma unroll
    for (int a = 0; a < 2; ++a)
#pragma unroll
        for (int b = 0; b < 3; ++b) {
            const unsigned d = (unsigned)(id[a][b] - s0);
            if (ok[a] && (b > 0 || need_left) && d < 4u) {
                const float gg = g[a][b];
                if (d == 0) v.x += gg; else if (d == 1) v.y += gg; else if (d == 2) v.z += gg; else v.w += gg;
                hit = true;
            }
        }
    if (hit) *reinterpret_cast<float4*>(dx + s0) = v;
}

__global__ __launch_bounds__(256) void maxpool_bwd_pair_bn_kernel(const float* __restrict__ dy, const int* __restrict__ idx,
                                                                  const float* __restrict__ raw, float* __restrict__ dx,
                                                                  int C, int H, int W, int OH, int OW,
                                                                  const float4* __restrict__ consts, unsigned w4_magic,
                                                                  float fM, float rfM, int act) {
    const int W4 = W >> 2;
    const int t = blockIdx.x * 256 + threadIdx.x;
    const int plane = blockIdx.y;
    const bool live = t < H * W4;
    const int tt = live ? t : 0;
    const int h = W4 > 1 ? (int)__umulhi((unsigned)tt, w4_magic) : tt, k = tt - h * W4, w0 = k * 4;
    const int s0 = (plane * H + h) * W + w0;
    const int i0 = h >= 2 ? (h - 1) >> 1 : 0;
    int i1 = h >> 1; if (i1 > OH - 1) i1 = OH - 1;
    const bool need_left = k > 0, fetch_left = need_left && (threadIdx.x & 63) == 0;
    const float4 xv = *reinterpret_cast<const float4*>(raw + s0);
    int id[2][3];
    float g[2][3];
    bool ok[2];
#pragma unroll
    for (int a = 0; a < 2; ++a) {
        const int i = i0 + a;
        ok[a] = live && i <= i1;
        const int o = (plane * OH + (i <= i1 ? i : i1)) * OW + 2 * k;
        const int2 ip = *reinterpret_cast<const int2*>(idx + o);
        const float2 gp = *reinterpret_cast<const float2*>(dy + o);
        const int ie = idx[fetch_left ? o - 1 : o];
        const float ge = dy[fetch_left ? o - 1 : o];
        id[a][0] = __builtin_amdgcn_update_dpp(ie, ip.y, 0x138 , 0xf, 0xf, false);
        g[a][0] = __builtin_bit_cast(float, __builtin_amdgcn_update_dpp(__builtin_bit_cast(int, ge), __builtin_bit_cast(int, gp.y),
                                                                        0x138, 0xf, 0xf, false));
        id[a][1] = ip.x; g[a][1] = gp.x;
        id[a][2] = ip.y; g[a][2] = gp.y;
    }
    if (!live) return;
    float4 v = make_float4(0.f, 0.f, 0.f, 0.f);
#pragma unroll
    for (int a = 0; a < 2; ++a)
#pragma unroll
        for (int b = 0; b < 3; ++b) {
            const unsigned d = (unsigned)(id[a][b] - s0);
            if (ok[a] && (b > 0 || need_left) && d < 4u) {
                const float gg = g[a][b];
                if (d == 0) v.x += gg; else if (d == 1) v.y += gg; else if (d == 2) v.z += gg; else v.w += gg;
            }
        }
    const int ch = plane % C;
    const float4 k0 = consts[3 * ch], k1 = consts[3 * ch + 1], k2 = consts[3 * ch + 2];
    const float m = k0.x, sc = k0.y, bb = k1.z, dmm = k1.w, dv = k2.x;
    const BnDiv rs{k0.z, k0.w}, rs_fwd{k1.x, k1.y}, fMd{fM, rfM};
    float dummy;
    float4 o;
    o.x = bn_bwd_one(v.x, bn_one(xv.x, m, rs_fwd, sc, bb, 0, act, &dummy), xv.x, m, rs, sc, dmm, dv, fMd, act);
    o.y = bn_bwd_one(v.y, bn_one(xv.y, m, rs_fwd, sc, bb, 0, act, &dummy), xv.y, m, rs, sc, dmm, dv, fMd, act);
    o.z = bn_bwd_one(v.z, bn_one(xv.z, m, rs_fwd, sc, bb, 0, act, &dummy), xv.z, m, rs, sc, dmm, dv, fMd, act);
    o.w = bn_bwd_one(v.w, bn_one(xv.w, m, rs_fwd, sc, bb, 0, act, &dummy), xv.w, m, rs, sc, dmm, dv, fMd, act);
    *reinterpret_cast<float4*>(dx + s0) = o;
}

__global__ __launch_bounds__(256) void avgpool_fwd_kernel(const float* __restrict__ x, float* __restrict__ y,
                                                          int planes, int HW) {
    const int lane = threadIdx.x & 63;
    const int wave = (blockIdx.x * blockDim.x + threadIdx.x) >> 6;
    const int nwaves = (gridDim.x * blockDim.x) >> 6;
    for (int p = wave; p < planes; p += nwaves) {
        const float* src = x + (long long)p * HW;
        float s = 0.f;
        for (int i = lane; i < HW; i += 64) s += src[i];
        s = wave_sum(s);
        if (lane == 0) y[p] = s / (float)HW;
    }
}

__global__ __launch_bounds__(256) void avgpool_bwd_kernel(const float* __restrict__ dy, float* __restrict__ dx,
                                                          int HW, unsigned total) {
    const unsigned gstride = gridDim.x * blockDim.x;
    for (unsigned i = blockIdx.x * blockDim.x + threadIdx.x; i < total; i += gstride) {
        const unsigned p = i / (unsigned)HW;
        dx[i] += dy[p] / (float)HW;
    }
}

}

using namespace bcnn_hip;

extern "C" {

void bcnn_hip_maxpool_forward(const float* x, float* y, int* indexes, int n, int c, int h, int w, int out_h,
                              int out_w, int size, int stride) {
    const long long total = (long long)n * c * out_h * out_w;
    if (!total) return;
    if (stride == 2 && (size == 2 || size == 3) && (w & 3) == 0 && out_w * 2 <= w + 1 &&
        (long long)n * c * h * w < 0x7fffffffLL && (reinterpret_cast<uintptr_t>(x) & 15) == 0) {
        const long long pairs = (long long)n * c * out_h * ((out_w + 1) / 2);
        const unsigned blocks = (unsigned)((pairs + 255) / 256);
        if (size == 2) maxpool_fwd_s2_kernel<2><<<blocks, 256, 0, current_stream()>>>(x, y, indexes, h, w, out_h, out_w, (unsigned)pairs);
        else maxpool_fwd_s2_kernel<3><<<blocks, 256, 0, current_stream()>>>(x, y, indexes, h, w, out_h, out_w, (unsigned)pairs);
        KERNEL_CHECK();
        return;
    }
    maxpool_fwd_kernel<<<stream_grid((size_t)total, 256), 256, 0, current_stream()>>>(
        x, y, indexes, n * c, h, w, out_h, out_w, size, stride, (unsigned)total);
    KERNEL_CHECK();
}

int bcnn_hip_maxpool_bn_fusable(int n, int c, int h, int w, int out_h, int out_w, int size, int stride, int act,
                                 const float* x) {
    return stride == 2 && (size == 2 || size == 3) && (w & 3) == 0 && out_w * 2 <= w + 1 &&
           (long long)n * c * h * w < 0x7fffffffLL && x && (reinterpret_cast<uintptr_t>(x) & 15) == 0 && act_is_cheap(act) &&
           act != BCNN_HIP_ACT_PRELU;
}

void bcnn_hip_maxpool_forward_bn_keep(const float* x, float* y, int* indexes, int n, int c, int h, int w, int out_h, int out_w,
                                      int size, int stride, const float* scales, const float* bias, const float* mean,
                                      const float* var, int act, float* raw_at_max) {
    const long long total = (long long)n * c * out_h * out_w;
    if (!total) return;
    if (!bcnn_hip_maxpool_bn_fusable(n, c, h, w, out_h, out_w, size, stride, act, x)) {
        fprintf(stderr, "[bcnn_hip] bcnn_hip_maxpool_forward_bn: not fusable (ask bcnn_hip_maxpool_bn_fusable)\n");
        exit(1);
    }
    KTimer kt(K_POOL, 0.0, 4.0 * ((double)n * c * h * w + 2.0 * (double)total));
    trace_kernel("maxpool_fwd_s2_bn_kernel");
    constexpr int R = 4;
    const long long items = (long long)n * c * ((out_h + R - 1) / R) * ((out_w + 1) / 2);
    const unsigned blocks = (unsigned)((items + 255) / 256);
    if (size == 2)
        maxpool_fwd_s2_bn_kernel<2, R><<<blocks, 256, 0, current_stream()>>>(x, y, indexes, c, h, w, out_h, out_w,
                                                                             (unsigned)items, mean, var, scales, bias, act,
                                                                             raw_at_max);
    else
        maxpool_fwd_s2_bn_kernel<3, R><<<blocks, 256, 0, current_stream()>>>(x, y, indexes, c, h, w, out_h, out_w,
                                                                             (unsigned)items, mean, var, scales, bias, act,
                                                                             raw_at_max);
    KERNEL_CHECK();
}

void bcnn_hip_maxpool_forward_bn(const float* x, float* y, int* indexes, int n, int c, int h, int w, int out_h, int out_w,
                                 int size, int stride, const float* scales, const float* bias, const float* mean,
                                 const float* var, int act) {
    bcnn_hip_maxpool_forward_bn_keep(x, y, indexes, n, c, h, w, out_h, out_w, size, stride, scales, bias, mean, var, act, nullptr);
}

int bcnn_hip_maxpool_bn_backward_fusable(int n, int c, int h, int w, int out_h, int out_w, int size, int stride, int act,
                                         const float* raw, const float* dpool, const int* indexes, const float* dx) {
    const uintptr_t p16 = reinterpret_cast<uintptr_t>(raw) | reinterpret_cast<uintptr_t>(dx);
    const uintptr_t p8 = reinterpret_cast<uintptr_t>(dpool) | reinterpret_cast<uintptr_t>(indexes);
    return size == 3 && stride == 2 && (w & 3) == 0 && out_w * 2 == w && out_h * out_w > 0 &&
           (long long)n * c * h * w < 0x7fffffffLL && (long long)n * c <= 65535 && raw && dx && (p16 & 15) == 0 && (p8 & 7) == 0 &&
           (long long)h * (w / 4) * (w / 4) < (1LL << 32) &&
           act_is_cheap(act) && act_bwd_is_cheap(act) && act != BCNN_HIP_ACT_PRELU;
}

void bcnn_hip_maxpool_bn_backward(const float* dpool, const int* indexes, const float* raw_at_max, const float* raw, float* dx,
                                  int n, int c, int h, int w, int out_h, int out_w, int size, int stride, const float* scales,
                                  float* dscales, const float* bias, float* dbias, const float* mean, const float* var,
                                  float* dmean, float* dvar, int act) {
    const long long total = (long long)n * c * h * w, ptotal = (long long)n * c * out_h * out_w;
    if (!total) return;
    if (!bcnn_hip_maxpool_bn_backward_fusable(n, c, h, w, out_h, out_w, size, stride, act, raw, dpool, indexes, dx) || !raw_at_max) {
        fprintf(stderr, "[bcnn_hip] bcnn_hip_maxpool_bn_backward: not fusable (ask bcnn_hip_maxpool_bn_backward_fusable)\n");
        exit(1);
    }
    float4* consts = scratch_f4(SCRATCH_BN_CONSTS, (size_t)c * 3);
    const float fM = (float)((long long)n * h * w);
    {
        KTimer kt(K_BN_BWD, 0.0, 4.0 * 2.0 * (double)ptotal);
        batchnorm_backward_sums(dpool, nullptr, act, scales, dscales, dbias, mean, var, dmean, dvar, raw_at_max, n, c,
                                out_h * out_w, act != BCNN_HIP_ACT_NONE ? bias : nullptr, nullptr, 0u, consts, fM);
    }
    KTimer kt(K_POOL, 0.0, 4.0 * (2.0 * (double)total + 2.0 * (double)ptotal));
    dim3 grid((unsigned)ceil_div(h * (w / 4), 256), (unsigned)(n * c));
    const unsigned w4 = (unsigned)(w / 4);
    trace_kernel("maxpool_bwd_pair_bn_kernel");
    maxpool_bwd_pair_bn_kernel<<<grid, 256, 0, current_stream()>>>(dpool, indexes, raw, dx, c, h, w, out_h, out_w, consts,
                                                                   w4 > 1 ? (unsigned)((0x100000000ULL + w4 - 1) / w4) : 0u, fM,
                                                                   1.0f / fM, act);
    KERNEL_CHECK();
}

void bcnn_hip_maxpool_backward(const float* dy, const int* indexes, float* dx, int n, int c, int h, int w,
                               int out_h, int out_w, int size, int stride, int overwrite) {
    const long long total = (long long)n * c * h * w;
    if (!total) return;
    if (!(out_h * out_w)) {
        if (overwrite) bcnn_hip_fill_f32(dx, (size_t)total, 0.f);
        return;
    }
    if ((w & 3) == 0 && total < 0x7fffffffLL && (long long)n * c <= 65535 &&
        (reinterpret_cast<uintptr_t>(dx) & 15) == 0) {
        dim3 grid((unsigned)ceil_div(h * (w / 4), 256), (unsigned)(n * c));
        const bool pairs = size == 3 && stride == 2 && out_w * 2 == w &&
                           ((reinterpret_cast<uintptr_t>(dy) | reinterpret_cast<uintptr_t>(indexes)) & 7) == 0;
        if (pairs) {
            if (overwrite) maxpool_bwd_vec4_k3s2_pair_kernel<true><<<grid, 256, 0, current_stream()>>>(dy, indexes, dx, h, w, out_h, out_w);
            else maxpool_bwd_vec4_k3s2_pair_kernel<false><<<grid, 256, 0, current_stream()>>>(dy, indexes, dx, h, w, out_h, out_w);
        } else if (size == 3 && stride == 2) {
            if (overwrite) maxpool_bwd_vec4_k3s2_kernel<true><<<grid, 256, 0, current_stream()>>>(dy, indexes, dx, h, w, out_h, out_w);
            else maxpool_bwd_vec4_k3s2_kernel<false><<<grid, 256, 0, current_stream()>>>(dy, indexes, dx, h, w, out_h, out_w);
        } else if (overwrite)
            maxpool_bwd_vec4_kernel<true><<<grid, 256, 0, current_stream()>>>(dy, indexes, dx, h, w, out_h, out_w, size, stride);
        else
            maxpool_bwd_vec4_kernel<false><<<grid, 256, 0, current_stream()>>>(dy, indexes, dx, h, w, out_h, out_w, size, stride);
        KERNEL_CHECK();
        return;
    }
    if (overwrite) bcnn_hip_fill_f32(dx, (size_t)total, 0.f);
    maxpool_bwd_kernel<<<stream_grid((size_t)total, 256), 256, 0, current_stream()>>>(
        dy, indexes, dx, h, w, out_h, out_w, size, stride, (unsigned)total);
    KERNEL_CHECK();
}

void bcnn_hip_avgpool_forward(const float* x, float* y, int n, int c, int h, int w) {
    const int planes = n * c;
    if (!planes) return;
    const int grid = stream_grid((size_t)planes * 64, 256);
    avgpool_fwd_kernel<<<grid, 256, 0, current_stream()>>>(x, y, planes, h * w);
    KERNEL_CHECK();
}

void bcnn_hip_avgpool_backward(const float* dy, float* dx, int n, int c, int h, int w) {
    const long long total = (long long)n * c * h * w;
    if (!total) return;
    avgpool_bwd_kernel<<<stream_grid((size_t)total, 256), 256, 0, current_stream()>>>(dy, dx, h * w, (unsigned)total);
    KERNEL_CHECK();
}

}
```

### bcnn_amd/host/bcnn_core.c

```c
#include <math.h>
#include <stdarg.h>
#include <string.h>

#include "bcnn_internal.h"
#include "../../include/bcnn_hip.h"

#ifndef BCNN_USE_HIP
#error "this runtime is the device build: compile with -DBCNN_USE_HIP"
#endif

void bcnn_log(bcnn_log_context ctx, bcnn_log_level level, const char *fmt, ...) {
    if (level < ctx.lvl) return;
    char msg[2048];
    va_list ap;
    va_start(ap, fmt);
    vsnprintf(msg, sizeof(msg), fmt, ap);
    va_end(ap);
    if (ctx.fct) {
        ctx.fct("%s", msg);
        return;
    }
    static const char *tag[] = {"[INFO] ", "[WARNING] ", "[ERROR] ", ""};
    fprintf(stderr, "%s%s", tag[level > 3 ? 3 : level], msg);
}
// ... 372 lines not shown
    for (int i = 0; i < net->num_nodes; ++i)
        if (net->nodes[i].type == BCNN_LAYER_CONV2D)
            ((bcnn_conv_param *)net->nodes[i].param)->conv_workspace_gpu = hc->workspace_gpu;
    if (!hc->compiled || hc->num_params != hc->arena_members) {
        invalidate_sgd_table(net);
        build_arenas(net);
        hc->compiled = 1;
        if (hc->grad_ready_fn) bcnn_set_gradient_ready_callback(net, hc->grad_ready_fn, hc->grad_ready_user);
        comm_sync_parameters(net);
    }
    relink_graph(net);
    bcnn_hip_sync();
    return BCNN_SUCCESS;
}

static void relink_graph(bcnn_net *net) {
    bcnn_hip_context *hc = hctx(net);
    mark_dead_grad_fills(net);
    for (int i = 0; i < net->num_nodes; ++i) {
        if (net->nodes[i].type != BCNN_LAYER_CONV2D) continue;
        const int t = net->nodes[i].dst[0];
        int rewritten = 0;
        for (int j = 0; j < net->num_nodes; ++j)
            rewritten |= net->nodes[j].type == BCNN_LAYER_DROPOUT && net->nodes[j].dst[0] == t;
        ((bcnn_conv_param *)net->nodes[i].param)->out_rewritten = rewritten;
    }
    bcnn_link_depthwise_batchnorm(net);
    bcnn_link_conv_eltwise(net);
    bcnn_link_conv_maxpool(net);
    bcnn_link_conv_depthwise(net);
    bcnn_link_batchnorm_conv(net);
    if (hc->fill_chunks_gpu) {
        bcnn_hip_sync();
        bcnn_hip_free(hc->fill_chunks_gpu);
        hc->fill_chunks_gpu = NULL;
    }
    hc->num_fill_chunks = -1;
}

static bcnn_status resize_private_f32(float **buf, size_t old_elems, size_t new_elems, int need_realloc) {
    if (!*buf || new_elems <= old_elems) return BCNN_SUCCESS;
    if (!need_realloc) return BCNN_INVALID_PARAMETER;
    bcnn_hip_sync();
    bcnn_hip_free(*buf);
    *buf = bcnn_hip_malloc_f32(new_elems);
    return *buf ? BCNN_SUCCESS : BCNN_FAILED_ALLOC;
}

bcnn_status bcnn_resize_net(bcnn_net *net, int w, int h, int c, int need_realloc) {
    if (!net || w <= 0 || h <= 0 || c <= 0) return BCNN_INVALID_PARAMETER;
    for (int i = 0; i < net->num_nodes; ++i) {
        const bcnn_layer_type t = net->nodes[i].type;
        BCNN_CHECK_AND_LOG(net->log_ctx, t != BCNN_LAYER_CONCAT && t != BCNN_LAYER_UPSAMPLE && t != BCNN_LAYER_YOLOV3 &&
                                             t != BCNN_LAYER_TRANSPOSE_CONV2D,
                           BCNN_INVALID_PARAMETER,
                           "bcnn_resize_net: node %d is a concat / upsample / YOLO / deconvolution node, whose resize is "
                           "not supported\n", i);
        BCNN_CHECK_AND_LOG(net->log_ctx,
                           t != BCNN_LAYER_COST || ((const bcnn_cost_param *)net->nodes[i].param)->loss != BCNN_LOSS_LIFTED_STRUCT,
                           BCNN_INVALID_PARAMETER,
                           "bcnn_resize_net: node %d is a lifted-structure cost node, whose resize is not supported\n", i);
    }
    bcnn_set_input_shape(net, w, h, c, 1);
    for (int i = 0; i < net->num_nodes; ++i) {
        bcnn_node *nd = &net->nodes[i];
        if (nd->num_src < 1 || nd->num_dst < 1) continue;
        if (nd->type == BCNN_LAYER_DROPOUT) continue;
        const bcnn_tensor *s = &net->tensors[nd->src[0]];
        bcnn_tensor *d = &net->tensors[nd->dst[0]];
        const size_t old_elems = (size_t)bcnn_tensor_size(d);
        if (nd->type == BCNN_LAYER_CONV2D) {
            const bcnn_conv_param *p = (const bcnn_conv_param *)nd->param;
            bcnn_tensor_set_shape(d, s->n, p->num, (s->h + 2 * p->pad - p->size) / p->stride + 1,
                                  (s->w + 2 * p->pad - p->size) / p->stride + 1, 1);
        } else if (nd->type == BCNN_LAYER_MAXPOOL) {
            const bcnn_maxpool_param *p = (const bcnn_maxpool_param *)nd->param;
            bcnn_tensor_set_shape(d, s->n, s->c, (s->h - 1) / p->stride + 1, (s->w - 1) / p->stride + 1, 1);
        } else {
            bcnn_tensor_set_shape(d, s->n, s->c, s->h, s->w, 1);
        }
        if (need_realloc) BCNN_CHECK_STATUS(bcnn_tensor_allocate(d, net->mode));
        const size_t new_elems = (size_t)bcnn_tensor_size(d);
        if (nd->type == BCNN_LAYER_CONV2D) {
            bcnn_conv_param *p = (bcnn_conv_param *)nd->param;
            BCNN_CHECK_STATUS(resize_private_f32(&p->bn_workspace_gpu, old_elems, new_elems, need_realloc));
            BCNN_CHECK_STATUS(resize_private_f32(&p->x_norm_gpu, old_elems, new_elems, need_realloc));
        } else if (nd->type == BCNN_LAYER_BATCHNORM) {
            bcnn_batchnorm_param *p = (bcnn_batchnorm_param *)nd->param;
            BCNN_CHECK_STATUS(resize_private_f32(&p->workspace_gpu, old_elems, new_elems, need_realloc));
            BCNN_CHECK_STATUS(resize_private_f32(&p->x_norm_gpu, old_elems, new_elems, need_realloc));
        } else if (nd->type == BCNN_LAYER_MAXPOOL && new_elems > old_elems) {
            bcnn_maxpool_param *p = (bcnn_maxpool_param *)nd->param;
            if (!need_realloc) return BCNN_INVALID_PARAMETER;
            bcnn_hip_sync();
            bcnn_hip_free(p->indexes_gpu);
            p->indexes_gpu = bcnn_hip_malloc_i32(new_elems);
            int *host = (int *)realloc(p->indexes, new_elems * sizeof(int));
            if (!host || !p->indexes_gpu) return BCNN_FAILED_ALLOC;
            p->indexes = host;
            if (p->raw_at_max_gpu) {
                bcnn_hip_free(p->raw_at_max_gpu);
                p->raw_at_max_gpu = NULL;
            }
        }
    }
    if (hctx(net)->compiled) return bcnn_compile_net(net);
    return BCNN_SUCCESS;
}

bcnn_status bcnn_set_mode(bcnn_net *net, bcnn_mode mode) {
    if (net->mode == mode) return BCNN_SUCCESS;
    if (mode == BCNN_MODE_TRAIN)
        for (int i = 0; i < net->num_nodes; ++i)
            BCNN_CHECK_AND_LOG(net->log_ctx, net->nodes[i].type != BCNN_LAYER_YOLOV3, BCNN_INVALID_PARAMETER,
                               "bcnn_set_mode: the net holds a YOLO node, whose TRAIN-mode loss is not built\n");
    net->mode = mode;
    if (net->data_loader) bcnn_switch_data_handles(net, net->data_loader);
    return BCNN_SUCCESS;
}

static void build_fill_table(bcnn_net *net) {
    bcnn_hip_context *hc = hctx(net);
    int cap = 256, n = 0;
    bcnn_hip_fill_chunk *tab = (bcnn_hip_fill_chunk *)malloc((size_t)cap * sizeof(*tab));
    unsigned char *seen = (unsigned char *)calloc((size_t)net->num_tensors + 1, 1);
    for (int i = 0; i < net->num_nodes; ++i)
        for (int d = 0; d < net->nodes[i].num_dst; ++d) {
            const int id = net->nodes[i].dst[d];
            bcnn_tensor *t = &net->tensors[id];
            if (seen[id] || !t->grad_data_gpu) continue;
            seen[id] = 1;
            if (hc->grad_fill_dead && id < hc->grad_fill_count && hc->grad_fill_dead[id]) continue;
            const size_t sz = (size_t)bcnn_tensor_size(t);
            for (size_t off = 0; off < sz; off += BCNN_HIP_FILL_CHUNK) {
                if (n == cap) {
                    cap *= 2;
                    tab = (bcnn_hip_fill_chunk *)realloc(tab, (size_t)cap * sizeof(*tab));
                }
                tab[n].p_d = t->grad_data_gpu + off;
                tab[n].count = (unsigned int)((sz - off < BCNN_HIP_FILL_CHUNK) ? (sz - off) : BCNN_HIP_FILL_CHUNK);
                tab[n].reserved = 0;
                ++n;
            }
        }
    free(seen);
    hc->num_fill_chunks = n;
    if (n > 0) {
        hc->fill_chunks_gpu = bcnn_hip_malloc_f32(((size_t)n * sizeof(*tab) + 3) / 4);
        bcnn_hip_memcpy_h2d(hc->fill_chunks_gpu, tab, (size_t)n * sizeof(*tab));
    }
    free(tab);
}

void bcnn_forward(bcnn_net *net) {
    bcnn_hip_context *hc = hctx(net);
    if (net->mode == BCNN_MODE_TRAIN) {
        if (hc->num_fill_chunks < 0) build_fill_table(net);
        bcnn_hip_zero_chunks((const bcnn_hip_fill_chunk *)hc->fill_chunks_gpu, hc->num_fill_chunks);
    }
    bcnn_drop_pending_gradients(net);
    bcnn_prepack_conv_weights(net, 0);
    hc->in_pass = 1;
    for (int i = 0; i < net->num_nodes; ++i) net->nodes[i].forward(net, &net->nodes[i]);
    hc->in_pass = 0;
    bcnn_hip_conv_prepack_discard();
}

static void comm_flush(bcnn_hip_context *hc) {
    if (hc->comm_lo < hc->comm_hi) {
        bcnn_hip_allreduce_sum(hc->grad_arena_gpu + hc->comm_lo, hc->comm_hi - hc->comm_lo);
        hc->comm_hi = hc->comm_lo;
    }
}

static void comm_on_ready(size_t first, size_t count, void *user) {
    bcnn_hip_context *hc = (bcnn_hip_context *)user;
    (void)count;
    hc->comm_lo = first;
    if (hc->comm_hi - hc->comm_lo >= hc->comm_bucket) comm_flush(hc);
}

void bcnn_backward(bcnn_net *net) {
    bcnn_hip_context *hc = hctx(net);
    size_t ready_from = hc->arena_size;
    if (hc->comm_active) hc->comm_lo = hc->comm_hi = hc->arena_size;
    bcnn_prepack_conv_weights(net, 1);
    hc->in_pass = 2;
    const int side_prev = bcnn_hip_conv_side_stream_mode((hc->no_side_stream || BCNN_EXP_ENV("BCNN_NO_SIDE_STREAM")) ? 0 : 2);
    for (int i = net->num_nodes - 1; i >= 0; --i) {
        net->nodes[i].backward(net, &net->nodes[i]);
        if (hc->grad_ready_fn && hc->node_grad_first && hc->node_grad_first[i] < ready_from) {
            bcnn_hip_conv_side_join();
            hc->grad_ready_fn(hc->node_grad_first[i], ready_from - hc->node_grad_first[i], hc->grad_ready_user);
            ready_from = hc->node_grad_first[i];
        }
    }
    hc->in_pass = 0;
    bcnn_hip_conv_side_join();
    bcnn_hip_conv_side_stream_mode(side_prev);
    bcnn_hip_conv_prepack_discard();
    if (hc->grad_ready_fn && ready_from > 0 && hc->arena_size > 0)
        hc->grad_ready_fn(0, ready_from, hc->grad_ready_user);
    if (hc->comm_active) {
        comm_flush(hc);
        bcnn_hip_comm_join();
    }
}

void bcnn_set_weight_gradient_stream(bcnn_net *net, int enable) { hctx(net)->no_side_stream = enable ? 0 : 1; }

bcnn_status bcnn_set_inference_precision(bcnn_net *net, bcnn_precision p) {
    if (!net || (p != BCNN_PRECISION_FP32 && p != BCNN_PRECISION_BF16)) return BCNN_INVALID_PARAMETER;
    hctx(net)->inference_precision = (int)p;
    return BCNN_SUCCESS;
}

bcnn_precision bcnn_get_inference_precision(const bcnn_net *net) {
    return (bcnn_precision)((const bcnn_hip_context *)net->hip_ctx)->inference_precision;
}

void bcnn_set_gradient_ready_callback(bcnn_net *net, bcnn_gradient_ready_fn fn, void *user) {
    bcnn_hip_context *hc = hctx(net);
    hc->grad_ready_fn = fn;
    hc->grad_ready_user = user;
    free(hc->node_grad_first);
    hc->node_grad_first = NULL;
    if (!fn || !hc->grad_arena_gpu) return;
    hc->node_grad_first = (size_t *)malloc((size_t)net->num_nodes * sizeof(size_t));
    for (int i = 0; i < net->num_nodes; ++i) {
        size_t first = (size_t)-1;
        for (int k = 0; k < net->nodes[i].num_src; ++k) {
            const bcnn_tensor *t = &net->tensors[net->nodes[i].src[k]];
            if (!t->grad_data_gpu || t->grad_data_gpu < hc->grad_arena_gpu ||
                t->grad_data_gpu >= hc->grad_arena_gpu + hc->arena_size)
                continue;
            const size_t off = (size_t)(t->grad_data_gpu - hc->grad_arena_gpu);
            if (off < first) first = off;
        }
        hc->node_grad_first[i] = first;
    }
}

static void step_learning_rate(bcnn_net *net) {
    bcnn_learner *ln = net->learner;
    const int global_batch = net->batch_size * hctx(net)->dp_world;
    ln->seen += global_batch;
    const int iter = ln->seen / global_batch;
    switch (ln->decay_type) {
        case BCNN_LR_DECAY_STEP:
            ln->learning_rate = ln->base_learning_rate * (float)pow(ln->scale, iter / ln->step);
            break;
        case BCNN_LR_DECAY_INV:
            ln->learning_rate = ln->base_learning_rate * (float)pow(1.0f + ln->gamma * iter, -ln->power);
            break;
        case BCNN_LR_DECAY_EXP:
            ln->learning_rate = ln->base_learning_rate * (float)pow(ln->gamma, iter);
            break;
        case BCNN_LR_DECAY_POLY:
            ln->learning_rate = ln->base_learning_rate * (float)pow(1 - (float)iter / ln->max_batches, ln->power);
            break;
        case BCNN_LR_DECAY_SIGMOID:
            ln->learning_rate = ln->base_learning_rate * (1.0f / (1.0f + (float)exp(ln->gamma * (iter - ln->step))));
            break;
        default:
            break;
    }
}

static void sgd_table_add(bcnn_hip_context *hc, float *w, float *g, size_t n, int use_decay) {
    for (size_t off = 0; off < n; off += BCNN_HIP_SGD_CHUNK) {
        if (hc->num_sgd_chunks == hc->cap_sgd_chunks) {
            hc->cap_sgd_chunks = hc->cap_sgd_chunks ? 2 * hc->cap_sgd_chunks : 1024;
            hc->sgd_chunks_host = (bcnn_hip_sgd_chunk *)realloc(hc->sgd_chunks_host,
                                                                (size_t)hc->cap_sgd_chunks * sizeof(bcnn_hip_sgd_chunk));
        }
        bcnn_hip_sgd_chunk *c = &hc->sgd_chunks_host[hc->num_sgd_chunks++];
        c->w_d = w + off;
        c->g_d = g + off;
        c->count = (unsigned int)((n - off < BCNN_HIP_SGD_CHUNK) ? (n - off) : BCNN_HIP_SGD_CHUNK);
        c->use_decay = (unsigned int)use_decay;
    }
}

static int update_is_tabled(const bcnn_node *nd) {
    return nd->update == bcnn_update_conv_layer || nd->update == bcnn_update_depthwise_conv_layer ||
           nd->update == bcnn_update_fullc_layer || nd->update == bcnn_update_deconv_layer;
}

void bcnn_update(bcnn_net *net) {
    bcnn_hip_context *hc = hctx(net);
    step_learning_rate(net);
    if (net->learner->optimizer == BCNN_OPTIM_ADAM) {
        for (int i = 0; i < net->num_nodes; ++i)
            if (net->nodes[i].update) net->nodes[i].update(net, &net->nodes[i]);
        return;
    }
    if (hc->sgd_chunks_gpu == NULL) {
        hc->sgd_collecting = 1;
        hc->num_sgd_chunks = 0;
        for (int i = 0; i < net->num_nodes; ++i)
            if (net->nodes[i].update && update_is_tabled(&net->nodes[i])) net->nodes[i].update(net, &net->nodes[i]);
        hc->sgd_collecting = 0;
        if (hc->num_sgd_chunks > 0) {
            hc->sgd_chunks_gpu = bcnn_hip_malloc_f32(((size_t)hc->num_sgd_chunks * sizeof(bcnn_hip_sgd_chunk) + 3) / 4);
            bcnn_hip_memcpy_h2d(hc->sgd_chunks_gpu, hc->sgd_chunks_host,
                                (size_t)hc->num_sgd_chunks * sizeof(bcnn_hip_sgd_chunk));
        }
    }
    const bcnn_learner *ln = net->learner;
    if (hc->num_sgd_chunks > 0)
        bcnn_hip_sgd_update_chunks((const bcnn_hip_sgd_chunk *)hc->sgd_chunks_gpu, hc->num_sgd_chunks,
                                   net->batch_size * hc->dp_world, ln->learning_rate,
                                   ln->momentum / (float)hc->dp_world, ln->decay);
    for (int i = 0; i < net->num_nodes; ++i)
        if (net->nodes[i].update && !update_is_tabled(&net->nodes[i])) net->nodes[i].update(net, &net->nodes[i]);
}

void bcnn_node_sgd_step(bcnn_net *net, bcnn_tensor *weights, bcnn_tensor *biases) {
    const bcnn_learner *ln = net->learner;
    const int world = hctx(net)->dp_world;
    if (hctx(net)->sgd_collecting) {
        if (biases && biases->data_gpu && biases->grad_data_gpu)
            sgd_table_add(hctx(net), biases->data_gpu, biases->grad_data_gpu, (size_t)bcnn_tensor_size(biases), 0);
        if (weights && weights->data_gpu && weights->grad_data_gpu)
            sgd_table_add(hctx(net), weights->data_gpu, weights->grad_data_gpu, (size_t)bcnn_tensor_size(weights), 1);
        return;
    }
    bcnn_hip_sgd_update(weights ? weights->data_gpu : NULL, biases ? biases->data_gpu : NULL,
                        weights ? weights->grad_data_gpu : NULL, biases ? biases->grad_data_gpu : NULL,
                        weights ? (size_t)bcnn_tensor_size(weights) : 0, biases ? (size_t)bcnn_tensor_size(biases) : 0,
                        net->batch_size * world, ln->learning_rate, ln->momentum / (float)world, ln->decay);
}

void bcnn_node_optim_step(bcnn_net *net, bcnn_tensor *weights, bcnn_tensor *biases, float **adam_m_gpu,
                          float **adam_v_gpu) {
    const bcnn_learner *ln = net->learner;
    if (ln->optimizer != BCNN_OPTIM_ADAM || adam_m_gpu == NULL) {
        bcnn_node_sgd_step(net, weights, biases);
        return;
// ... 255 lines not shown
```

### bcnn_amd/host/bcnn_layers_hot.c

```c
#include <math.h>
#include <string.h>

#include "bcnn_internal.h"
#include "../../include/bcnn_hip.h"

static bcnn_hip_context *hctx(bcnn_net *net) { return (bcnn_hip_context *)net->hip_ctx; }

static bcnn_status attach_source(bcnn_net *net, bcnn_node *node, const char *src_id, const char *what) {
    if (net->num_nodes == 0) return bcnn_node_add_input(net, node, 0);
    const int idx = bcnn_net_find_tensor(net, src_id);
    BCNN_CHECK_AND_LOG(net->log_ctx, idx >= 0, BCNN_INVALID_PARAMETER, "%s layer: invalid input node name %s\n",
                       what, src_id);
    return bcnn_node_add_input(net, node, idx);
}

static bcnn_status add_vector_param(bcnn_net *net, bcnn_node *node, int count, int has_grad, const char *src_id,
                                    const char *suffix, float fill, int trainable) {
    char name[256];
    snprintf(name, sizeof(name), "%s_%s", src_id, suffix);
    bcnn_tensor t = {0};
    bcnn_tensor_create(&t, 1, 1, 1, count, has_grad, name, net->mode);
    if (fill != 0.0f) {
        bcnn_tensor_filler f = {.value = fill, .type = BCNN_FILLER_FIXED};
        bcnn_tensor_fill(&t, f);
// ... 35 lines not shown
    if (size == 1 && oh * ow > sh * sw) {
        free(node.src);
        BCNN_CHECK_AND_LOG(net->log_ctx, 0, BCNN_INVALID_PARAMETER,
                           "Convolution layer %s: a 1x1 kernel with pad %d gives %d x %d outputs from %d x %d inputs; "
                           "the raw-view addressing of 1x1 kernels would run past the source tensor\n",
                           dst_id, pad, ow, oh, sw, sh);
    }

    char name[256];
    snprintf(name, sizeof(name), "%s_w", src_id);
    bcnn_tensor weights = {0};
    bcnn_tensor_create(&weights, num_filters, cg, size, size, 1, name, net->mode);
    bcnn_tensor_filler wf = {.range = size * size * cg, .type = init};
    bcnn_tensor_fill(&weights, wf);
    BCNN_CHECK_STATUS(bcnn_net_add_tensor(net, weights));
    BCNN_CHECK_STATUS(bcnn_node_add_input(net, &node, net->num_tensors - 1));
    bcnn_net_register_param(net, net->num_tensors - 1);
    BCNN_CHECK_STATUS(add_vector_param(net, &node, num_filters, 1, src_id, "b", 0.0f, 1));

    node.type = BCNN_LAYER_CONV2D;
    node.param_size = sizeof(bcnn_conv_param);
    bcnn_conv_param *param = (bcnn_conv_param *)calloc(1, node.param_size);
    node.param = param;
    param->activation = activation;
    param->pad = pad; param->num = num_filters; param->size = size; param->stride = stride;
    param->num_groups = num_groups;
    param->elt_node = -1;
    param->pool_node = -1;
    param->dw_node = -1;
    param->bnsums_node = -1;
    param->fold_bn = -1;
    node.forward = bcnn_forward_conv_layer;
    node.backward = bcnn_backward_conv_layer;
    node.update = bcnn_update_conv_layer;
    node.release_param = bcnn_release_param_conv_layer;

    BCNN_CHECK_STATUS(add_output(net, &node, sn, num_filters, oh, ow, dst_id));
    if (batch_norm) {
        param->batch_norm = 1;
        snprintf(name, sizeof(name), "%s_sav_mean", src_id);
        bcnn_tensor_create(&param->saved_mean, 1, 1, 1, num_filters, 1, name, net->mode);
        snprintf(name, sizeof(name), "%s_sav_var", src_id);
        bcnn_tensor_create(&param->saved_variance, 1, 1, 1, num_filters, 1, name, net->mode);
        BCNN_CHECK_STATUS(add_vector_param(net, &node, num_filters, 0, src_id, "run_mean", 0.0f, 0));
        BCNN_CHECK_STATUS(add_vector_param(net, &node, num_filters, 0, src_id, "run_var", 0.0f, 0));
        BCNN_CHECK_STATUS(add_vector_param(net, &node, num_filters, 1, src_id, "scales", 1.0f, 0));
        if (net->mode != BCNN_MODE_PREDICT)
            param->bn_workspace_gpu = bcnn_hip_malloc_f32((size_t)sn * num_filters * oh * ow);
    }
    if (activation == BCNN_ACT_PRELU)
        BCNN_CHECK_STATUS(add_vector_param(net, &node, num_filters, 0, src_id, "prelu_slopes", 0.0f, 0));
    BCNN_CHECK_STATUS(bcnn_net_add_node(net, node));
    BCNN_INFO(net->log_ctx, "[Conv2D%s%s] %-8s (%4d x%4d x%4d) -> %-8s (%4d x%4d x%4d) %d x %d / %d pad %d groups %d\n",
              batch_norm ? "+BN" : "", activation != BCNN_ACT_NONE ? "+act" : "", src_id, sw, sh, sc, dst_id, ow, oh,
              num_filters, size, size, stride, pad, num_groups);
    return BCNN_SUCCESS;
}

typedef struct {
    bcnn_tensor *x, *w, *b, *y, *run_mean, *run_var, *scales, *slopes;
} conv_io;

static conv_io conv_tensors(bcnn_net *net, bcnn_node *node) {
    conv_io io = {0};
    bcnn_conv_param *p = (bcnn_conv_param *)node->param;
    io.x = &net->tensors[node->src[0]];
    io.w = &net->tensors[node->src[1]];
    io.b = &net->tensors[node->src[2]];
    io.y = &net->tensors[node->dst[0]];
    if (p->batch_norm) {
        io.run_mean = &net->tensors[node->src[3]];
        io.run_var = &net->tensors[node->src[4]];
        io.scales = &net->tensors[node->src[5]];
    }
    if (p->activation == BCNN_ACT_PRELU) io.slopes = &net->tensors[node->src[3 + 3 * p->batch_norm]];
    return io;
}

static const float *announce_bnfold(bcnn_net *net, const bcnn_conv_param *p) {
    const bcnn_node *bn = &net->nodes[p->fold_bn];
    const bcnn_batchnorm_param *bp = (const bcnn_batchnorm_param *)bn->param;
    bcnn_hip_conv_set_input_bnfold(bp->saved_mean.data_gpu, bp->saved_variance.data_gpu, net->tensors[bn->src[3]].data_gpu,
                                   net->tensors[bn->src[4]].data_gpu);
    return net->tensors[bn->src[0]].data_gpu;
}

static int bcnn_bf16_inference(const bcnn_net *net) {
    return net->mode != BCNN_MODE_TRAIN && ((const bcnn_hip_context *)net->hip_ctx)->inference_precision == BCNN_PRECISION_BF16;
}

void bcnn_forward_conv_layer(bcnn_net *net, bcnn_node *node) {
    bcnn_conv_param *p = (bcnn_conv_param *)node->param;
    conv_io io = conv_tensors(net, node);
    p->data_pending = 0;
    p->apply_skipped = 0;
    p->folded = 0;
    const float *xin = io.x->data_gpu;
    if (hctx(net)->in_pass == 1 && net->mode == BCNN_MODE_TRAIN && p->fold_bn >= 0 &&
        ((bcnn_batchnorm_param *)net->nodes[p->fold_bn].param)->apply_skipped) {
        ((bcnn_batchnorm_param *)net->nodes[p->fold_bn].param)->apply_skipped = 0;
        xin = announce_bnfold(net, p);
        p->folded = 1;
    }
    if (hctx(net)->in_pass == 1 && (p->pool_node >= 0 || p->dw_node >= 0) && net->mode == BCNN_MODE_TRAIN) {
        bcnn_hip_conv_forward_stats_only(xin, io.w->data_gpu, io.b->data_gpu, io.x->n, io.x->c, io.x->h, io.x->w,
                                         p->num, p->size, p->stride, p->pad, p->num_groups, io.run_mean->data_gpu,
                                         io.run_var->data_gpu, io.scales->data_gpu, p->saved_mean.data_gpu,
                                         p->saved_variance.data_gpu, p->bn_workspace_gpu);
        p->apply_skipped = 1;
        p->data_pending = 1;
        return;
    }
    if (hctx(net)->in_pass == 1 && p->elt_node >= 0 && net->mode == BCNN_MODE_TRAIN) {
        bcnn_node *en = &net->nodes[p->elt_node];
        bcnn_eltwise_param *ep = (bcnn_eltwise_param *)en->param;
        bcnn_tensor *r = &net->tensors[en->src[1]], *out = &net->tensors[en->dst[0]];
        bcnn_hip_conv_forward_residual(xin, io.w->data_gpu, io.b->data_gpu, io.x->n, io.x->c, io.x->h, io.x->w,
                                       p->num, p->size, p->stride, p->pad, p->num_groups, io.run_mean->data_gpu,
                                       io.run_var->data_gpu, io.scales->data_gpu, p->saved_mean.data_gpu,
                                       p->saved_variance.data_gpu, p->bn_workspace_gpu, r->data_gpu,
                                       (size_t)ep->min_dim[0] * out->h * out->w, (int)ep->activation, out->data_gpu);
        ep->done_forward = 1;
        p->data_pending = 1;
        return;
    }
    if (bcnn_bf16_inference(net)) {
        bcnn_hip_conv_forward_bf16(xin, io.w->data_gpu, io.b->data_gpu, io.y->data_gpu, io.x->n, io.x->c, io.x->h, io.x->w,
                                   p->num, p->size, p->stride, p->pad, p->num_groups, (int)p->activation,
                                   io.slopes ? io.slopes->data_gpu : NULL, p->batch_norm,
                                   io.run_mean ? io.run_mean->data_gpu : NULL, io.run_var ? io.run_var->data_gpu : NULL,
                                   io.scales ? io.scales->data_gpu : NULL, p->saved_mean.data_gpu,
                                   p->saved_variance.data_gpu, p->x_norm_gpu, p->bn_workspace_gpu, (int)net->mode);
        return;
    }
    bcnn_hip_conv_forward(xin, io.w->data_gpu, io.b->data_gpu, io.y->data_gpu, io.x->n, io.x->c, io.x->h,
                          io.x->w, p->num, p->size, p->stride, p->pad, p->num_groups, (int)p->activation,
                          io.slopes ? io.slopes->data_gpu : NULL, p->batch_norm,
                          io.run_mean ? io.run_mean->data_gpu : NULL, io.run_var ? io.run_var->data_gpu : NULL,
                          io.scales ? io.scales->data_gpu : NULL, p->saved_mean.data_gpu,
                          p->saved_variance.data_gpu, p->x_norm_gpu, p->bn_workspace_gpu, (int)net->mode);
}

void bcnn_backward_conv_layer(bcnn_net *net, bcnn_node *node) {
    bcnn_conv_param *p = (bcnn_conv_param *)node->param;
    conv_io io = conv_tensors(net, node);
    const float *xin = io.x->data_gpu;
    if (hctx(net)->in_pass == 2 && p->folded && p->fold_bn >= 0)
        xin = announce_bnfold(net, p);
    if (hctx(net)->in_pass == 2 && p->pool_bwd_pending) {
        bcnn_node *pn = &net->nodes[p->pool_node];
        bcnn_maxpool_param *mp = (bcnn_maxpool_param *)pn->param;
        const bcnn_tensor *py = &net->tensors[pn->dst[0]];
        p->pool_bwd_pending = 0;
        bcnn_hip_maxpool_bn_backward(py->grad_data_gpu, mp->indexes_gpu, mp->raw_at_max_gpu, p->bn_workspace_gpu,
                                     io.y->grad_data_gpu, io.y->n, io.y->c, io.y->h, io.y->w, py->h, py->w, mp->size,
                                     mp->stride, io.scales->data_gpu, io.scales->grad_data_gpu, io.b->data_gpu,
                                     io.b->grad_data_gpu, p->saved_mean.data_gpu, p->saved_variance.data_gpu,
                                     p->saved_mean.grad_data_gpu, p->saved_variance.grad_data_gpu, (int)p->activation);
        bcnn_hip_conv_backward_bn_done(xin, io.w->data_gpu, io.y->grad_data_gpu, io.x->grad_data_gpu,
                                       io.w->grad_data_gpu, io.x->n, io.x->c, io.x->h, io.x->w, p->num, p->size, p->stride,
                                       p->pad, p->num_groups, p->conv_workspace_gpu, hctx(net)->workspace_size);
        return;
    }
    if (hctx(net)->in_pass == 2 && p->elt_node >= 0 && ((bcnn_eltwise_param *)net->nodes[p->elt_node].param)->deferred) {
        bcnn_node *en = &net->nodes[p->elt_node];
        bcnn_eltwise_param *ep = (bcnn_eltwise_param *)en->param;
        bcnn_tensor *r = &net->tensors[en->src[1]], *out = &net->tensors[en->dst[0]];
        ep->deferred = 0;
        ep->grad_pending = 1;
        bcnn_hip_conv_backward_residual(xin, io.w->data_gpu, io.b->data_gpu, io.y->grad_data_gpu, io.x->grad_data_gpu,
                                        io.w->grad_data_gpu, io.b->grad_data_gpu, io.x->n, io.x->c, io.x->h, io.x->w,
                                        p->num, p->size, p->stride, p->pad, p->num_groups, io.scales->data_gpu,
                                        io.scales->grad_data_gpu, p->saved_mean.data_gpu, p->saved_variance.data_gpu,
                                        p->saved_mean.grad_data_gpu, p->saved_variance.grad_data_gpu, p->bn_workspace_gpu,
                                        p->conv_workspace_gpu, hctx(net)->workspace_size, out->data_gpu,
                                        out->grad_data_gpu, (int)ep->activation, r->data_gpu, r->grad_data_gpu,
                                        (size_t)ep->min_dim[0] * out->h * out->w);
        return;
    }
    const int own_splits = hctx(net)->in_pass == 2 ? p->insums_splits : 0;
    p->insums_splits = 0;
    const int to_bn = hctx(net)->in_pass == 2 && p->bnsums_node >= 0 && io.x->grad_data_gpu;
    if (to_bn || own_splits > 0) {
        bcnn_node *bn = to_bn ? &net->nodes[p->bnsums_node] : NULL;
        bcnn_batchnorm_param *bp = bn ? (bcnn_batchnorm_param *)bn->param : NULL;
        const int splits = bcnn_hip_conv_backward_presummed(
            xin, io.w->data_gpu, p->out_rewritten ? NULL : io.b->data_gpu, io.y->data_gpu, io.y->grad_data_gpu, io.x->grad_data_gpu,
            io.w->grad_data_gpu, io.b->grad_data_gpu, io.x->n, io.x->c, io.x->h, io.x->w, p->num, p->size, p->stride, p->pad,
            p->num_groups, (int)p->activation, io.slopes ? io.slopes->data_gpu : NULL,
            io.slopes ? io.slopes->grad_data_gpu : NULL, p->batch_norm, io.scales ? io.scales->data_gpu : NULL,
            io.scales ? io.scales->grad_data_gpu : NULL, p->saved_mean.data_gpu, p->saved_variance.data_gpu,
            p->saved_mean.grad_data_gpu, p->saved_variance.grad_data_gpu, p->x_norm_gpu, p->bn_workspace_gpu,
            p->conv_workspace_gpu, hctx(net)->workspace_size, own_splits > 0 ? p->insums_gpu : NULL, own_splits,
            bn ? net->tensors[bn->src[0]].data_gpu : NULL, bp ? bp->saved_mean.data_gpu : NULL, bp ? bp->bsums_gpu : NULL,
            bp ? bp->bsums_floats : 0);
        if (bp) bp->bsums_splits = splits;
        return;
    }
    bcnn_hip_conv_backward(xin, io.w->data_gpu, p->out_rewritten ? NULL : io.b->data_gpu ,
                           io.y->data_gpu, io.y->grad_data_gpu,
                           io.x->grad_data_gpu , io.w->grad_data_gpu,
                           io.b->grad_data_gpu, io.x->n, io.x->c, io.x->h, io.x->w, p->num, p->size, p->stride,
                           p->pad, p->num_groups, (int)p->activation, io.slopes ? io.slopes->data_gpu : NULL,
                           io.slopes ? io.slopes->grad_data_gpu : NULL, p->batch_norm,
                           io.scales ? io.scales->data_gpu : NULL, io.scales ? io.scales->grad_data_gpu : NULL,
                           p->saved_mean.data_gpu, p->saved_variance.data_gpu, p->saved_mean.grad_data_gpu,
                           p->saved_variance.grad_data_gpu, p->x_norm_gpu, p->bn_workspace_gpu,
                           p->conv_workspace_gpu, hctx(net)->workspace_size);
}

void bcnn_prepack_conv_weights(bcnn_net *net, int data_gradient) {
    int n = 0;
    if (BCNN_EXP_ENV("BCNN_NO_PREPACK")) return;
    if (net->num_nodes < 1) return;
    const int none = !data_gradient && bcnn_bf16_inference(net);
    bcnn_hip_conv_desc *d = (bcnn_hip_conv_desc *)malloc((size_t)net->num_nodes * sizeof(*d));
    if (!d) return;
    for (int i = 0; i < net->num_nodes; ++i) {
        bcnn_node *node = &net->nodes[i];
        if (node->type != BCNN_LAYER_CONV2D || none) continue;
        const bcnn_conv_param *p = (const bcnn_conv_param *)node->param;
        const bcnn_tensor *x = &net->tensors[node->src[0]], *w = &net->tensors[node->src[1]];
        if (!w->data_gpu || (data_gradient && !x->grad_data_gpu)) continue;
        if (!data_gradient && net->mode == BCNN_MODE_TRAIN && p->fold_bn >= 0) continue;
        d[n].w_d = w->data_gpu;
        d[n].n = x->n; d[n].c = x->c; d[n].h = x->h; d[n].w = x->w;
        d[n].f = p->num; d[n].k = p->size; d[n].stride = p->stride; d[n].pad = p->pad; d[n].groups = p->num_groups;
        ++n;
    }
    bcnn_hip_conv_prepack(d, n, data_gradient);
    free(d);
}

void bcnn_update_conv_layer(bcnn_net *net, bcnn_node *node) {
    bcnn_conv_param *p = (bcnn_conv_param *)node->param;
    bcnn_node_optim_step(net, &net->tensors[node->src[1]], &net->tensors[node->src[2]], &p->adam_m_gpu, &p->adam_v_gpu);
}

void bcnn_release_param_conv_layer(bcnn_node *node) {
    bcnn_conv_param *p = (bcnn_conv_param *)node->param;
    bcnn_tensor_destroy(&p->saved_mean);
    bcnn_tensor_destroy(&p->saved_variance);
    bcnn_hip_free(p->bn_workspace_gpu);
    bcnn_hip_free(p->insums_gpu);
    bcnn_hip_free(p->x_norm_gpu);
    bcnn_hip_free(p->adam_m_gpu);
    bcnn_hip_free(p->adam_v_gpu);
}

bcnn_status bcnn_add_depthwise_conv_layer(bcnn_net *net, int size, int stride, int pad, int batch_norm,
                                          bcnn_filler_type init, bcnn_activation activation, const char *src_id,
                                          const char *dst_id) {
    (void)batch_norm;
    bcnn_node node = {0};
    BCNN_CHECK_STATUS(attach_source(net, &node, src_id, "Depthwise convolution"));
    const bcnn_tensor s = net->tensors[node.src[0]];
    char name[256];
    snprintf(name, sizeof(name), "%s_w", src_id);
    bcnn_tensor weights = {0};
    bcnn_tensor_create(&weights, 1, 1, 1, s.c * size * size, 1, name, net->mode);
    bcnn_tensor_filler wf = {.range = size * size * s.c, .type = init};
    bcnn_tensor_fill(&weights, wf);
    BCNN_CHECK_STATUS(bcnn_net_add_tensor(net, weights));
    BCNN_CHECK_STATUS(bcnn_node_add_input(net, &node, net->num_tensors - 1));
    bcnn_net_register_param(net, net->num_tensors - 1);
    BCNN_CHECK_STATUS(add_vector_param(net, &node, s.c, 1, src_id, "b", 0.0f, 1));
    node.type = BCNN_LAYER_DEPTHWISE_CONV2D;
    node.param_size = sizeof(bcnn_depthwise_conv_param);
    bcnn_depthwise_conv_param *param = (bcnn_depthwise_conv_param *)calloc(1, node.param_size);
    node.param = param;
    param->activation = activation; param->size = size; param->stride = stride; param->pad = pad;
    param->bn_node = -1;
    param->conv_node = -1;
    node.forward = bcnn_forward_depthwise_conv_layer;
    node.backward = bcnn_backward_depthwise_conv_layer;
    node.update = bcnn_update_depthwise_conv_layer;
    node.release_param = bcnn_release_param_depthwise_conv_layer;
    const int oh = (s.h + 2 * pad - size) / stride + 1, ow = (s.w + 2 * pad - size) / stride + 1;
    BCNN_CHECK_STATUS(add_output(net, &node, s.n, s.c, oh, ow, dst_id));
    BCNN_CHECK_STATUS(bcnn_net_add_node(net, node));
    BCNN_INFO(net->log_ctx, "[DepthwiseConv2D] %-8s (%4d x%4d x%4d) -> %-8s (%4d x%4d x%4d) %d x %d / %d\n", src_id,
              s.w, s.h, s.c, dst_id, ow, oh, s.c, size, size, stride);
    return BCNN_SUCCESS;
}

void bcnn_forward_depthwise_conv_layer(bcnn_net *net, bcnn_node *node) {
    bcnn_depthwise_conv_param *p = (bcnn_depthwise_conv_param *)node->param;
    bcnn_tensor *x = &net->tensors[node->src[0]], *w = &net->tensors[node->src[1]];
    bcnn_tensor *b = &net->tensors[node->src[2]], *y = &net->tensors[node->dst[0]];
    p->stats_splits = 0;
    p->raw_input = 0;
    if (hctx(net)->in_pass == 1 && p->conv_node >= 0 && ((bcnn_conv_param *)net->nodes[p->conv_node].param)->apply_skipped) {
        bcnn_node *cn = &net->nodes[p->conv_node];
        bcnn_conv_param *cp = (bcnn_conv_param *)cn->param;
        const int want_stats = net->mode == BCNN_MODE_TRAIN && p->bn_node >= 0 && p->stats_gpu;
        cp->apply_skipped = 0;
        p->raw_input = 1;
        p->stats_splits = bcnn_hip_depthwise_forward_bnin(cp->bn_workspace_gpu, w->data_gpu, b->data_gpu, y->data_gpu, x->n,
                                                          x->c, x->h, x->w, p->size, p->stride, p->pad, (int)p->activation,
                                                          want_stats ? p->stats_gpu : NULL, want_stats ? p->stats_floats : 0,
                                                          cp->saved_mean.data_gpu, cp->saved_variance.data_gpu,
                                                          net->tensors[cn->src[5]].data_gpu,
                                                          net->tensors[cn->src[2]].data_gpu, (int)cp->activation);
        return;
    }
    if (hctx(net)->in_pass == 1 && net->mode == BCNN_MODE_TRAIN && p->bn_node >= 0 && p->stats_gpu) {
        p->stats_splits = bcnn_hip_depthwise_forward_stats(x->data_gpu, w->data_gpu, b->data_gpu, y->data_gpu, x->n, x->c,
                                                           x->h, x->w, p->size, p->stride, p->pad, (int)p->activation,
                                                           p->stats_gpu, p->stats_floats);
        return;
    }
    bcnn_hip_depthwise_forward(x->data_gpu, w->data_gpu, b->data_gpu, y->data_gpu, x->n, x->c, x->h, x->w, p->size,
                               p->stride, p->pad, (int)p->activation);
}
// ... 620 lines not shown
```

### include/bcnn_hip.h

```cpp
#ifndef BCNN_HIP_H
#define BCNN_HIP_H

#include <stddef.h>
#include <stdint.h>

#ifdef __cplusplus
extern "C" {
#endif

enum {
    BCNN_HIP_ACT_NONE = 0, BCNN_HIP_ACT_TANH, BCNN_HIP_ACT_RELU, BCNN_HIP_ACT_RAMP,
    BCNN_HIP_ACT_SOFTPLUS, BCNN_HIP_ACT_LRELU, BCNN_HIP_ACT_ABS, BCNN_HIP_ACT_CLAMP,
    BCNN_HIP_ACT_PRELU, BCNN_HIP_ACT_LOGISTIC
};
enum { BCNN_HIP_MODE_PREDICT = 0, BCNN_HIP_MODE_TRAIN = 1, BCNN_HIP_MODE_VALID = 2 };

int bcnn_hip_device_count(void);
void bcnn_hip_set_device(int id);
int bcnn_hip_get_device(void);
const char *bcnn_hip_device_name(void);
float *bcnn_hip_malloc_f32(size_t n);
int *bcnn_hip_malloc_i32(size_t n);
void bcnn_hip_free(void *p_d);
void bcnn_hip_memcpy_h2d(void *dst_d, const void *src_h, size_t bytes);
void bcnn_hip_memcpy_d2h(void *dst_h, const void *src_d, size_t bytes);
void bcnn_hip_memcpy_d2d(void *dst_d, const void *src_d, size_t bytes);
void bcnn_hip_fill_f32(float *x_d, size_t n, float value);
void bcnn_hip_sync(void);
void *bcnn_hip_stream_create(void);
void bcnn_hip_stream_destroy(void *stream);
void bcnn_hip_set_stream(void *stream);
void *bcnn_hip_get_stream(void);
void *bcnn_hip_event_create(void);
void bcnn_hip_event_destroy(void *ev);
void bcnn_hip_event_record(void *ev);
void bcnn_hip_event_sync(void *ev);
float bcnn_hip_event_elapsed_ms(void *start, void *stop);

void bcnn_hip_profile_enable(int on);
void bcnn_hip_profile_reset(void);
int bcnn_hip_profile_num_classes(void);
const char *bcnn_hip_profile_class_name(int cls);
void bcnn_hip_profile_read(int cls, double *ms, long long *launches, double *flops, double *bytes);
double bcnn_hip_profile_read_useful_flops(int cls);

int bcnn_hip_conv_side_stream_mode(int mode);
void bcnn_hip_conv_side_join(void);

void bcnn_hip_trace_enable(int on);
size_t bcnn_hip_trace_read(char *buf, size_t cap);

void bcnn_hip_axpy(size_t n, float a, const float *x_d, float *y_d);
void bcnn_hip_scal(size_t n, float a, float *x_d);
void bcnn_hip_copy_f32(size_t n, const float *x_d, float *y_d);
void bcnn_hip_add_bias(float *y_d, const float *bias_d, int n, int c, int hw);
void bcnn_hip_grad_bias(float *dbias_d, const float *g_d, int n, int c, int hw);
void bcnn_hip_scales(float *y_d, const float *scales_d, int n, int c, int hw);
void bcnn_hip_grad_scales(const float *x_norm_d, const float *g_d, int n, int c, int hw,
                          float *dscales_d);

void bcnn_hip_gemm(int trans_a, int trans_b, int m, int n, int k, float alpha, const float *a_d,
                   int lda, const float *b_d, int ldb, float beta, float *c_d, int ldc);
void bcnn_hip_im2col(const float *im_d, int channels, int height, int width, int ksize, int pad,
                     int stride, float *col_d);
void bcnn_hip_col2im(const float *col_d, int channels, int height, int width, int ksize, int pad,
                     int stride, float *im_d);

void bcnn_hip_activation_forward(float *x_d, size_t size, int act, const float *slopes_d,
                                 int spatial, int channels);
void bcnn_hip_activation_backward(const float *x_d, float *dx_d, size_t size, int act,
                                  const float *slopes_d, float *dslopes_d, int spatial, int channels);

void bcnn_hip_batchnorm_forward(const float *x_d, float *y_d, float *run_mean_d, float *run_var_d,
                                const float *scales_d, const float *bias_d, float *saved_mean_d,
                                float *saved_var_d, float *x_norm_d, float *workspace_d, int n, int c,
                                int hw, int mode, int act);
void bcnn_hip_batchnorm_backward(float *dy_d, float *dx_d, const float *y_d, int act,
                                 const float *scales_d, float *dscales_d, float *dbias_d,
                                 const float *saved_mean_d, const float *saved_var_d, float *dmean_d,
                                 float *dvar_d, const float *x_norm_d, const float *workspace_d, int n,
                                 int c, int hw);

size_t bcnn_hip_conv_workspace_size(int n, int c, int h, int w, int f, int k, int stride, int pad,
                                    int groups);
void bcnn_hip_conv_forward(const float *x_d, const float *w_d, const float *bias_d, float *y_d, int n,
                           int c, int h, int w, int f, int k, int stride, int pad, int groups, int act,
                           const float *slopes_d,
                           int batch_norm, float *run_mean_d, float *run_var_d, const float *scales_d,
                           float *saved_mean_d, float *saved_var_d, float *x_norm_d,
                           float *bn_workspace_d, int mode);
void bcnn_hip_conv_backward(const float *x_d, const float *w_d, const float *bias_d, const float *y_d,
                            float *dy_d, float *dx_d, float *dw_d, float *dbias_d, int n, int c, int h, int w, int f,
                            int k, int stride, int pad, int groups, int act, const float *slopes_d,
                            float *dslopes_d, int batch_norm, const float *scales_d, float *dscales_d,
                            const float *saved_mean_d, const float *saved_var_d, float *dmean_d,
                            float *dvar_d, const float *x_norm_d, const float *bn_workspace_d,
                            float *workspace_d, size_t workspace_elems);
int bcnn_hip_conv_forward_bf16(const float *x_d, const float *w_d, const float *bias_d, float *y_d, int n, int c, int h,
                               int w, int f, int k, int stride, int pad, int groups, int act, const float *slopes_d,
                               int batch_norm, float *run_mean_d, float *run_var_d, const float *scales_d,
                               float *saved_mean_d, float *saved_var_d, float *x_norm_d, float *bn_workspace_d,
                               int mode);

int bcnn_hip_conv_residual_fusable(int batch_norm, int act, int res_act, int mode, const float *bn_workspace_d,
                                   const float *res_d, const float *res_out_d);
void bcnn_hip_conv_forward_residual(const float *x_d, const float *w_d, const float *bias_d, int n, int c, int h, int w,
                                    int f, int k, int stride, int pad, int groups, float *run_mean_d, float *run_var_d,
                                    const float *scales_d, float *saved_mean_d, float *saved_var_d,
                                    float *bn_workspace_d, const float *res_d, size_t res_count, int res_act,
                                    float *res_out_d);
void bcnn_hip_conv_backward_residual(const float *x_d, const float *w_d, const float *bias_d, float *dy_d, float *dx_d,
                                     float *dw_d, float *dbias_d, int n, int c, int h, int w, int f, int k, int stride,
                                     int pad, int groups, const float *scales_d, float *dscales_d,
                                     const float *saved_mean_d, const float *saved_var_d, float *dmean_d, float *dvar_d,
                                     const float *bn_workspace_d, float *workspace_d, size_t workspace_elems,
                                     const float *res_out_d, const float *dres_out_d, int res_act, const float *res_d,
                                     float *dres_d, size_t res_count);
void bcnn_hip_batchnorm_apply(const float *x_d, float *y_d, const float *scales_d, const float *bias_d,
                              const float *saved_mean_d, const float *saved_var_d, int n, int c, int hw, int act);

typedef struct {
    const float *w_d;
    int n, c, h, w, f, k, stride, pad, groups;
} bcnn_hip_conv_desc;
void bcnn_hip_conv_prepack(const bcnn_hip_conv_desc *layers, int count, int data_gradient);
void bcnn_hip_conv_prepack_reset(void);
void bcnn_hip_conv_prepack_discard(void);

void bcnn_hip_maxpool_forward(const float *x_d, float *y_d, int *indexes_d, int n, int c, int h, int w,
                              int out_h, int out_w, int size, int stride);
void bcnn_hip_maxpool_backward(const float *dy_d, const int *indexes_d, float *dx_d, int n, int c,
                               int h, int w, int out_h, int out_w, int size, int stride, int overwrite);
size_t bcnn_hip_conv_bnsums_size(int n, int c, int h, int w);
int bcnn_hip_conv_backward_bnsums(const float *x_d, const float *w_d, const float *bias_d, const float *y_d, float *dy_d,
                                  float *dx_d, float *dw_d, float *dbias_d, int n, int c, int h, int w, int f, int k,
                                  int stride, int pad, int groups, int act, const float *slopes_d, float *dslopes_d,
                                  int batch_norm, const float *scales_d, float *dscales_d, const float *saved_mean_d,
                                  const float *saved_var_d, float *dmean_d, float *dvar_d, const float *x_norm_d,
                                  const float *bn_workspace_d, float *workspace_d, size_t workspace_elems,
                                  const float *prev_y_d, const float *prev_mean_d, float *sums_d, size_t sums_floats);
size_t bcnn_hip_depthwise_insums_size(int n, int c, int h, int w, int k, int stride, int pad);
int bcnn_hip_depthwise_backward_bnin_sums(const float *x_raw_d, const float *w_d, const float *y_d, float *dy_d, float *dx_d,
                                          float *dw_d, float *dbias_d, int n, int c, int h, int w, int k, int stride, int pad,
                                          int act, int overwrite, const float *bn_mean_d, const float *bn_var_d,
                                          const float *bn_scales_d, const float *bn_dmean_d, const float *bn_dvar_d,
                                          const float *in_mean_d, const float *in_var_d, const float *in_scale_d,
                                          const float *in_bias_d, int in_act, float *in_sums_d, size_t in_sums_floats);
int bcnn_hip_conv_backward_presummed(const float *x_d, const float *w_d, const float *bias_d, const float *y_d, float *dy_d,
                                     float *dx_d, float *dw_d, float *dbias_d, int n, int c, int h, int w, int f, int k,
                                     int stride, int pad, int groups, int act, const float *slopes_d, float *dslopes_d,
                                     int batch_norm, const float *scales_d, float *dscales_d, const float *saved_mean_d,
                                     const float *saved_var_d, float *dmean_d, float *dvar_d, const float *x_norm_d,
                                     const float *bn_workspace_d, float *workspace_d, size_t workspace_elems,
                                     const float *own_sums_d, int own_splits, const float *prev_y_d,
                                     const float *prev_mean_d, float *prev_sums_d, size_t prev_sums_floats);
void bcnn_hip_batchnorm_backward_finalize(const float *sums_d, int splits, const float *scales_d, float *dscales_d,
                                          float *dbias_d, const float *saved_var_d, float *dmean_d, float *dvar_d, int c);

void bcnn_hip_conv_forward_stats_only(const float *x_d, const float *w_d, const float *bias_d, int n, int c, int h, int w,
                                      int f, int k, int stride, int pad, int groups, float *run_mean_d, float *run_var_d,
                                      const float *scales_d, float *saved_mean_d, float *saved_var_d,
                                      float *bn_workspace_d);
int bcnn_hip_maxpool_bn_fusable(int n, int c, int h, int w, int out_h, int out_w, int size, int stride, int act,
                                const float *x_d);
void bcnn_hip_maxpool_forward_bn(const float *x_d, float *y_d, int *indexes_d, int n, int c, int h, int w, int out_h,
                                 int out_w, int size, int stride, const float *scales_d, const float *bias_d,
                                 const float *saved_mean_d, const float *saved_var_d, int act);
void bcnn_hip_maxpool_forward_bn_keep(const float *x_d, float *y_d, int *indexes_d, int n, int c, int h, int w, int out_h,
                                      int out_w, int size, int stride, const float *scales_d, const float *bias_d,
                                      const float *saved_mean_d, const float *saved_var_d, int act, float *raw_at_max_d);
int bcnn_hip_maxpool_bn_backward_fusable(int n, int c, int h, int w, int out_h, int out_w, int size, int stride, int act,
                                         const float *raw_d, const float *dpool_d, const int *indexes_d, const float *dx_d);
void bcnn_hip_maxpool_bn_backward(const float *dpool_d, const int *indexes_d, const float *raw_at_max_d, const float *raw_d,
                                  float *dx_d, int n, int c, int h, int w, int out_h, int out_w, int size, int stride,
                                  const float *scales_d, float *dscales_d, const float *bias_d, float *dbias_d,
                                  const float *saved_mean_d, const float *saved_var_d, float *dmean_d, float *dvar_d, int act);
void bcnn_hip_conv_backward_bn_done(const float *x_d, const float *w_d, float *dy_d, float *dx_d, float *dw_d, int n, int c,
                                    int h, int w, int f, int k, int stride, int pad, int groups, float *workspace_d,
                                    size_t workspace_elems);
void bcnn_hip_avgpool_forward(const float *x_d, float *y_d, int n, int c, int h, int w);
void bcnn_hip_avgpool_backward(const float *dy_d, float *dx_d, int n, int c, int h, int w);

void bcnn_hip_depthwise_forward(const float *x_d, const float *w_d, const float *bias_d, float *y_d,
                                int n, int c, int h, int w, int k, int stride, int pad, int act);
void bcnn_hip_depthwise_backward(const float *x_d, const float *w_d, const float *y_d, float *dy_d,
                                 float *dx_d, float *dw_d, float *dbias_d, int n, int c, int h, int w,
                                 int k, int stride, int pad, int act, int overwrite);

size_t bcnn_hip_depthwise_stats_size(int n, int c, int h, int w, int k, int stride, int pad);
int bcnn_hip_depthwise_forward_stats(const float *x_d, const float *w_d, const float *bias_d, float *y_d, int n, int c,
                                     int h, int w, int k, int stride, int pad, int act, float *stats_d,
                                     size_t stats_floats);
void bcnn_hip_batchnorm_forward_stats(const float *x_d, float *y_d, float *run_mean_d, float *run_var_d,
                                      const float *scales_d, const float *bias_d, float *saved_mean_d,
                                      float *saved_var_d, float *x_norm_d, float *workspace_d, int n, int c, int hw,
                                      int mode, int act, const float *stats_d, int splits);
void bcnn_hip_batchnorm_forward_stats_only(const float *x_d, float *run_mean_d, float *run_var_d, const float *scales_d,
                                           const float *bias_d, float *saved_mean_d, float *saved_var_d, int n, int c,
                                           int hw, const float *stats_d, int splits);
int bcnn_hip_conv_bnfold_fusable(int n, int c, int h, int w, int f);
void bcnn_hip_conv_set_input_bnfold(const float *mean_d, const float *var_d, const float *scales_d, const float *bias_d);
int bcnn_hip_depthwise_bn_fusable(int n, int c, int h, int w, int k, int stride, int pad, int act);
void bcnn_hip_batchnorm_backward_sums(const float *dy_d, const float *scales_d, float *dscales_d, float *dbias_d,
                                      const float *saved_mean_d, const float *saved_var_d, float *dmean_d,
                                      float *dvar_d, const float *x_d, int n, int c, int hw);
void bcnn_hip_batchnorm_backward_apply(float *dy_d, float *dx_d, const float *scales_d, const float *saved_mean_d,
                                       const float *saved_var_d, const float *dmean_d, const float *dvar_d,
                                       const float *x_d, int n, int c, int hw);
void bcnn_hip_depthwise_backward_bn(const float *x_d, const float *w_d, const float *y_d, const float *dz_d,
                                    float *dx_d, float *dw_d, float *dbias_d, int n, int c, int h, int w, int k,
                                    int stride, int pad, int act, int overwrite, const float *bn_mean_d,
                                    const float *bn_var_d, const float *bn_scales_d, const float *bn_dmean_d,
                                    const float *bn_dvar_d);

int bcnn_hip_depthwise_bnin_fusable(int n, int c, int h, int w, int k, int stride, int pad, int act, int in_act);
int bcnn_hip_depthwise_forward_bnin(const float *x_raw_d, const float *w_d, const float *bias_d, float *y_d, int n, int c,
                                    int h, int w, int k, int stride, int pad, int act, float *stats_d, size_t stats_floats,
                                    const float *in_mean_d, const float *in_var_d, const float *in_scale_d,
                                    const float *in_bias_d, int in_act);
void bcnn_hip_depthwise_backward_bnin(const float *x_raw_d, const float *w_d, const float *y_d, float *dy_d, float *dx_d,
                                      float *dw_d, float *dbias_d, int n, int c, int h, int w, int k, int stride, int pad,
                                      int act, int overwrite, const float *in_mean_d, const float *in_var_d,
                                      const float *in_scale_d, const float *in_bias_d, int in_act);
void bcnn_hip_depthwise_backward_bn_bnin(const float *x_raw_d, const float *w_d, const float *y_d, const float *dz_d,
                                         float *dx_d, float *dw_d, float *dbias_d, int n, int c, int h, int w, int k,
                                         int stride, int pad, int act, int overwrite, const float *bn_mean_d,
                                         const float *bn_var_d, const float *bn_scales_d, const float *bn_dmean_d,
                                         const float *bn_dvar_d, const float *in_mean_d, const float *in_var_d,
                                         const float *in_scale_d, const float *in_bias_d, int in_act);

void bcnn_hip_sgd_update(float *w_d, float *b_d, float *dw_d, float *db_d, size_t w_size,
                         size_t b_size, int batch_size, float learning_rate, float momentum,
                         float decay);

void bcnn_hip_adam_update(float *w_d, float *b_d, float *dw_d, float *db_d, float *adam_m_d,
                          float *adam_v_d, size_t w_size, size_t b_size, int batch_size, int iter,
                          float beta1, float beta2, float learning_rate, float momentum, float decay);

#define BCNN_HIP_SGD_CHUNK 2048
typedef struct bcnn_hip_sgd_chunk {
    float *w_d;
    float *g_d;
    unsigned int count;
    unsigned int use_decay;
} bcnn_hip_sgd_chunk;
void bcnn_hip_sgd_update_chunks(const bcnn_hip_sgd_chunk *chunks_d, int num_chunks, int batch_size,
                                float learning_rate, float momentum, float decay);

#define BCNN_HIP_FILL_CHUNK 16384
typedef struct bcnn_hip_fill_chunk {
    float *p_d;
    unsigned int count;
    unsigned int reserved;
} bcnn_hip_fill_chunk;
void bcnn_hip_zero_chunks(const bcnn_hip_fill_chunk *chunks_d, int num_chunks);

void bcnn_hip_eltwise_forward(const float *a_d, const float *b_d, float *y_d, size_t n, size_t b_count, int act);
void bcnn_hip_eltwise_backward(const float *y_d, float *dy_d, float *da_d, float *db_d, size_t n, size_t b_count,
                               int act, int overwrite_a);
void bcnn_hip_cost_metric(int metric, const float *pred_d, const float *label_d, const float *grad_d, int batch,
                          int per, float *out_d);
void bcnn_hip_axpy_strided(int num_batches, float a, const float *x_d, float *y_d, int stride_y,
                           int stride_x, int x_c, int x_h, int x_w, int y_c, int y_h, int y_w, int min_c,
                           int min_h, int min_w);
void bcnn_hip_add_rowvec(float *y_d, const float *v_d, int rows, int cols);
void bcnn_hip_softmax_forward(const float *x_d, float *y_d, int n, int c, int hw);

void bcnn_hip_concat_forward(int num_src, const float *const *src_d, const int *src_size3d, float *dst_d,
                             int dst_size3d, int n);
void bcnn_hip_concat_backward(int num_src, float *const *src_grad_d, const int *src_size3d, const float *dst_grad_d,
                              int dst_size3d, int n);
void bcnn_hip_upsample_forward(const float *x_d, float *y_d, int n, int c, int h, int w, int size);
void bcnn_hip_upsample_backward(float *dx_d, const float *dy_d, int n, int c, int h, int w, int size);
void bcnn_hip_yolo_activate(const float *x_d, float *y_d, int n, int num, int coords, int classes, int hw);

#define BCNN_HIP_YOLO_MAX_HEADS 8
#define BCNN_HIP_YOLO_MAX_ANCHORS 16
#define BCNN_HIP_YOLO_RECORD_HEAD 6
typedef struct bcnn_hip_yolo_head {
    const float *out_d;
    int h, w, num, coords, classes;
    float anchor_w[BCNN_HIP_YOLO_MAX_ANCHORS], anchor_h[BCNN_HIP_YOLO_MAX_ANCHORS];
} bcnn_hip_yolo_head;
int bcnn_hip_yolo_nms_capacity(void);
size_t bcnn_hip_yolo_detect_result_words(int n, int record_cap, int max_classes);
int bcnn_hip_yolo_detect_batch(const bcnn_hip_yolo_head *heads, int num_heads, int n, const int *image_geom, int in_w,
                               int in_h, int netw, int neth, float thresh, int relative, float nms_thresh,
                               int record_cap, int nms_cap, void *result_host);

#define BCNN_HIP_IMAGE_FIT_STRETCH 0
#define BCNN_HIP_IMAGE_FIT_LETTERBOX 1
int bcnn_hip_fill_images(float *dst_d, int n, int c, int h, int w, int num_images, const uint8_t *const *images,
                         const int *widths, const int *heights, const int *strides, int fit, float norm_coeff,
                         int swap_to_bgr, float mean_r, float mean_g, float mean_b);

size_t bcnn_hip_deconv_workspace_size(int n, int c, int h, int w, int f, int k, int stride, int pad);
void bcnn_hip_deconv_forward(const float *x_d, const float *w_d, const float *bias_d, float *y_d, int n, int c, int h,
                             int w, int f, int k, int stride, int pad, int act);
void bcnn_hip_deconv_backward(const float *x_d, const float *w_d, const float *y_d, float *dy_d, float *dx_d,
                              float *dw_d, float *dbias_d, int n, int c, int h, int w, int f, int k, int stride, int pad,
                              int act, float *workspace_d, size_t workspace_elems);

void bcnn_hip_lrn_forward(const float *x_d, float *y_d, int n, int c, int h, int w, int local_size, float alpha,
                          float beta, float k);
void bcnn_hip_lrn_backward(const float *x_d, const float *dy_d, float *dx_d, int n, int c, int h, int w,
                           int local_size, float alpha, float beta, float k, int overwrite);

void bcnn_hip_dropout_forward(float *x_d, size_t size, float rate, uint64_t key, uint64_t step);
void bcnn_hip_dropout_backward(float *dx_d, size_t size, float rate, uint64_t key, uint64_t step);

typedef struct bcnn_hip_lifted_struct_record {
    float loss;
    int num_constraints;
} bcnn_hip_lifted_struct_record;
size_t bcnn_hip_lifted_struct_workspace_size(int batch, int k);
void bcnn_hip_lifted_struct_forward(const float *x_d, const float *label_d, float *g_d, int batch, int k, float margin,
                                    int accumulate, bcnn_hip_lifted_struct_record *record_d, float *workspace_d);
void bcnn_hip_lifted_struct_backward(float *g_d, int batch, int k, float scale,
                                     const bcnn_hip_lifted_struct_record *record_d);

void bcnn_hip_comm_init(int rank, int world, const char *id_path);
void bcnn_hip_comm_retain(void);
void bcnn_hip_comm_destroy(void);
int bcnn_hip_rendezvous_publish(const char *path, const void *blob, size_t n, int world);
int bcnn_hip_rendezvous_fetch(const char *path, void *blob, size_t n, int world, int timeout_ms);
int bcnn_hip_comm_world(void);
int bcnn_hip_comm_rank(void);
void bcnn_hip_allreduce_sum(float *buf_d, size_t n);
void bcnn_hip_broadcast(float *buf_d, size_t n, int root);
void bcnn_hip_comm_join(void);

#ifdef __cplusplus
// ... 4 lines not shown
```

Before: 13900 images/s.

## Overlap weight prepacking on side stream and pipeline stem backward by batch parts

```diff
diff --git a/bcnn_amd/_lib.py b/bcnn_amd/_lib.py
--- a/bcnn_amd/_lib.py
+++ b/bcnn_amd/_lib.py
@@ -89,11 +89,19 @@
     "bcnn_hip_maxpool_bn_backward_fusable": (i, [i] * 9 + [vp] * 4),
     "bcnn_hip_maxpool_bn_backward": (None, [vp] * 5 + [i] * 8 + [vp] * 8 + [i]),
     "bcnn_hip_conv_backward_bn_done": (None, [vp] * 5 + [i] * 9 + [vp, sz]),
+    "bcnn_hip_conv_tail_parts_mode": (i, [i]),
+    "bcnn_hip_conv_tail_parts": (i, [i] * 9),
+    "bcnn_hip_maxpool_bn_backward_parts": (None, [vp] * 5 + [i] * 8 + [vp] * 8 + [i, i]),
+    "bcnn_hip_conv_backward_bn_done_parts": (None, [vp] * 5 + [i] * 9 + [vp, sz, i]),
     "bcnn_hip_depthwise_insums_size": (sz, [i] * 7),
     "bcnn_hip_depthwise_backward_bnin_sums": (i, [vp] * 7 + [i] * 9 + [vp] * 5 + [vp] * 4 + [i] + [vp, sz]),
     "bcnn_hip_conv_backward_presummed": (i, [vp] * 8 + [i] * 10 + [vp, vp, i] + [vp] * 8 + [vp, sz] + [vp, i] + [vp, vp, vp, sz]),
     "bcnn_hip_conv_prepack_reset": (None, []),
     "bcnn_hip_conv_prepack_discard": (None, []),
+    "bcnn_hip_conv_prepack_side_mode": (i, [i]),
+    "bcnn_hip_conv_prepack_side_begin": (i, []),
+    "bcnn_hip_conv_prepack_side_end": (None, []),
+    "bcnn_hip_conv_prepack_side_join": (None, []),
     "bcnn_hip_maxpool_bn_fusable": (i, [i] * 9 + [vp]),
     "bcnn_hip_conv_forward_stats_only": (None, [vp, vp, vp] + [i] * 9 + [vp] * 6),
     "bcnn_hip_maxpool_forward_bn": (None, [vp, vp, vp] + [i] * 8 + [vp] * 4 + [i]),
diff --git a/bcnn_amd/csrc/common.h b/bcnn_amd/csrc/common.h
--- a/bcnn_amd/csrc/common.h
+++ b/bcnn_amd/csrc/common.h
@@ -78,6 +78,14 @@
 
 inline int ceil_div(long long a, long long b) { return (int)((a + b - 1) / b); }
 
+constexpr int kTailPartsMax = 4;
+inline void tail_part_range(int n, int parts, int p, int* first, int* count) {
+    const int base = n / parts;
+    *first = p * base;
+    *count = p == parts - 1 ? n - p * base : base;
+}
+void conv_tail_part_record(int p);
+
 #ifndef STREAM_GRID_PER_CU
 #define STREAM_GRID_PER_CU 8
 #endif
diff --git a/bcnn_amd/csrc/conv.hip b/bcnn_amd/csrc/conv.hip
--- a/bcnn_amd/csrc/conv.hip
+++ b/bcnn_amd/csrc/conv.hip
@@ -42,8 +42,14 @@
     hipStream_t stream = nullptr;
     hipEvent_t ready = nullptr, done = nullptr;
     bool pending = false;
+    hipEvent_t fork = nullptr, packs = nullptr;
+    hipStream_t packs_home = nullptr;
+    bool packs_open = false;
+    bool packs_pending = false;
+    hipEvent_t part[kTailPartsMax] = {};
 };
 static thread_local SideStream g_side[kMaxDevices];
+static thread_local int g_packs_beside = 1;
 static thread_local int g_side_mode = 0;
 bool conv_side_stream_deferred() { return g_side_mode == 2; }
 static SideStream* side_stream() {
@@ -54,8 +60,23 @@
         HIP_CHECK(hipStreamCreateWithPriority(&ss.stream, hipStreamNonBlocking, BCNN_EXP_ENV("BCNN_HIP_SIDE_PRIO_SAME") ? prio_hi : prio_lo));
         HIP_CHECK(hipEventCreateWithFlags(&ss.ready, hipEventDisableTiming));
         HIP_CHECK(hipEventCreateWithFlags(&ss.done, hipEventDisableTiming));
+        HIP_CHECK(hipEventCreateWithFlags(&ss.fork, hipEventDisableTiming));
+        HIP_CHECK(hipEventCreateWithFlags(&ss.packs, hipEventDisableTiming));
+        for (hipEvent_t& e : ss.part) HIP_CHECK(hipEventCreateWithFlags(&e, hipEventDisableTiming));
     }
     return &ss;
+}
+void conv_tail_part_record(int p) {
+    if (p < 0 || p >= kTailPartsMax) return;
+    HIP_CHECK(hipEventRecord(side_stream()->part[p], current_stream()));
+}
+static thread_local int g_tail_parts_mode = 0;
+constexpr int kTailPartsDefault = 2;
+static void packs_wait() {
+    SideStream& ss = g_side[current_device()];
+    if (!ss.packs_pending || current_stream() == ss.stream) return;
+    ss.packs_pending = false;
+    HIP_CHECK(hipStreamWaitEvent(current_stream(), ss.packs, 0));
 }
 
 struct PrepackEntry {
@@ -81,6 +102,7 @@
     for (PrepackEntry& e : st.entries)
         if (e.w == w && e.kind == kind && e.mode == mode && e.fresh && e.epoch == st.epoch && e.floats == floats) {
             e.fresh = false;
+            packs_wait();
             return e.buf;
         }
     return nullptr;
@@ -280,14 +302,49 @@
     }
 }
 
-void bcnn_hip_conv_prepack_discard(void) { ++g_prepack.epoch; }
+void bcnn_hip_conv_prepack_discard(void) {
+    packs_wait();
+    ++g_prepack.epoch;
+}
 
 void bcnn_hip_conv_prepack_reset(void) {
     PrepackStore& st = g_prepack;
     if (st.dev < 0) return;
     prepack_free_all(st);
+    for (SideStream& ss : g_side) ss.packs_pending = false;
     ++st.epoch;
 }
+
+int bcnn_hip_conv_prepack_side_mode(int enable) {
+    const int prev = g_packs_beside;
+    if (enable >= 0) g_packs_beside = enable ? 1 : 0;
+    return prev;
+}
+
+int bcnn_hip_conv_prepack_side_begin(void) {
+    static const bool off = BCNN_EXP_ENV("BCNN_HIP_PACKS_ON_CALLER") != nullptr;
+    if (off || !g_packs_beside) return 0;
+    SideStream* ss = side_stream();
+    if (ss->packs_open) return 0;
+    packs_wait();
+    HIP_CHECK(hipEventRecord(ss->fork, current_stream()));
+    HIP_CHECK(hipStreamWaitEvent(ss->stream, ss->fork, 0));
+    ss->packs_home = current_stream();
+    ss->packs_open = true;
+    set_current_stream(ss->stream);
+    return 1;
+}
+
+void bcnn_hip_conv_prepack_side_end(void) {
+    SideStream& ss = g_side[current_device()];
+    if (!ss.packs_open) return;
+    HIP_CHECK(hipEventRecord(ss.packs, ss.stream));
+    set_current_stream(ss.packs_home);
+    ss.packs_open = false;
+    ss.packs_pending = true;
+}
+
+void bcnn_hip_conv_prepack_side_join(void) { packs_wait(); }
 
 size_t bcnn_hip_conv_workspace_size(int n, int c, int h, int w, int f, int k, int stride, int pad, int groups) {
     const ConvShape s = make_conv_shape(n, c, h, w, f, k, stride, pad, groups);
@@ -417,7 +474,7 @@
                                const float* saved_var, float* dmean, float* dvar, const float* x_norm,
                                const float* bn_workspace, float* workspace, size_t workspace_elems,
                                const ConvResidualBwd* rb, DxBnSums* bs = nullptr, const float* own_sums = nullptr,
-                               int own_splits = 0, bool bn_done = false) {
+                               int own_splits = 0, bool bn_done = false, int tail_parts = 1) {
     const ConvShape s = make_conv_shape(n, c, h, wd, f, k, stride, pad, groups);
     const size_t ysize = (size_t)n * f * s.OHOW;
     const BnFold fold = take_fold();
@@ -449,13 +506,22 @@
     const int side_mode = g_side_mode ? g_side_mode : side_env;
     SideStream* side = (side_mode == 2 || (side_mode == 1 && dx)) ? side_stream() : nullptr;
     hipStream_t main_stream = current_stream();
+    const bool in_parts = side && side_mode == 2 && bn_done && batch_norm && !dx && !fold.mean && tail_parts > 1 &&
+                          gate_open(GATE_WINDOW) && conv_dw_stem_parts_ok(s, tail_parts);
     if (side) {
-        HIP_CHECK(hipEventRecord(side->ready, main_stream));
-        HIP_CHECK(hipStreamWaitEvent(side->stream, side->ready, 0));
+        if (!in_parts) {
+            HIP_CHECK(hipEventRecord(side->ready, main_stream));
+            HIP_CHECK(hipStreamWaitEvent(side->stream, side->ready, 0));
+        }
         set_current_stream(side->stream);
     }
     bool bias_done = false;
-    if (fold.mean) {
+    if (in_parts) {
+        conv_backward_weights_stem_parts(x, dy, dw, s, workspace, workspace_elems, tail_parts, [](int p) {
+            SideStream* ss = side_stream();
+            HIP_CHECK(hipStreamWaitEvent(ss->stream, ss->part[p], 0));
+        });
+    } else if (fold.mean) {
         trace_kernel("bnfold:dw");
         KTimer kt(K_CONV_DW, conv_gemm_flops(s), conv_gemm_bytes(s));
         if (!conv_backward_weights_dma(x, dy, dw, s, workspace, workspace_elems, &fold)) {
@@ -523,11 +589,32 @@
     return bs.splits;
 }
 
+void bcnn_hip_conv_backward_bn_done_parts(const float* x, const float* w, float* dy, float* dx, float* dw, int n, int c, int h,
+                                          int wd, int f, int k, int stride, int pad, int groups, float* workspace,
+                                          size_t workspace_elems, int parts) {
+    conv_backward_impl(x, w, nullptr, nullptr, dy, dx, dw, nullptr, n, c, h, wd, f, k, stride, pad, groups, BCNN_HIP_ACT_NONE,
+                       nullptr, nullptr, 1, nullptr, nullptr, nullptr, nullptr, nullptr, nullptr, nullptr, nullptr, workspace,
+                       workspace_elems, nullptr, nullptr, nullptr, 0, true, parts);
+}
+
 void bcnn_hip_conv_backward_bn_done(const float* x, const float* w, float* dy, float* dx, float* dw, int n, int c, int h, int wd,
                                     int f, int k, int stride, int pad, int groups, float* workspace, size_t workspace_elems) {
-    conv_backward_impl(x, w, nullptr, nullptr, dy, dx, dw, nullptr, n, c, h, wd, f, k, stride, pad, groups, BCNN_HIP_ACT_NONE,
-                       nullptr, nullptr, 1, nullptr, nullptr, nullptr, nullptr, nullptr, nullptr, nullptr, nullptr, workspace,
-                       workspace_elems, nullptr, nullptr, nullptr, 0, true);
+    bcnn_hip_conv_backward_bn_done_parts(x, w, dy, dx, dw, n, c, h, wd, f, k, stride, pad, groups, workspace, workspace_elems, 1);
+}
+
+int bcnn_hip_conv_tail_parts_mode(int parts) {
+    const int prev = g_tail_parts_mode;
+    if (parts == 0 || parts == 1 || parts == 2 || parts == 4) g_tail_parts_mode = parts;
+    return prev;
+}
+
+int bcnn_hip_conv_tail_parts(int n, int c, int h, int wd, int f, int k, int stride, int pad, int groups) {
+    static const char* env = BCNN_EXP_ENV("BCNN_HIP_STEM_TAIL_PARTS");
+    int parts = g_tail_parts_mode ? g_tail_parts_mode : env ? atoi(env) : kTailPartsDefault;
+    if (parts != 2 && parts != 4) return 1;
+    if (g_side_mode != 2 || n <= 0 || groups <= 0 || !gate_open(GATE_WINDOW)) return 1;
+    const ConvShape s = make_conv_shape(n, c, h, wd, f, k, stride, pad, groups);
+    return conv_dw_stem_parts_ok(s, parts) ? parts : 1;
 }
 
 int bcnn_hip_conv_backward_presummed(const float* x, const float* w, const float* bias, const float* y, float* dy, float* dx,
diff --git a/bcnn_amd/csrc/conv_paths.h b/bcnn_amd/csrc/conv_paths.h
--- a/bcnn_amd/csrc/conv_paths.h
+++ b/bcnn_amd/csrc/conv_paths.h
@@ -63,6 +63,9 @@
 size_t conv_dw_stem_workspace_floats(const ConvShape& s);
 bool conv_backward_weights_stem(const float* x, const float* dy, float* dw, float* dbias, const ConvShape& s,
                                 float* workspace, size_t workspace_floats, bool* bias_done);
+bool conv_dw_stem_parts_ok(const ConvShape& s, int parts);
+void conv_backward_weights_stem_parts(const float* x, const float* dy, float* dw, const ConvShape& s, float* workspace,
+                                      size_t workspace_floats, int parts, void (*before_part)(int p));
 size_t conv_dw_direct_workspace_floats(const ConvShape& s);
 bool conv_backward_weights_direct(const float* x, const float* dy, float* dw, float* dbias, const ConvShape& s,
                                   float* workspace, size_t workspace_floats, bool* bias_done);
diff --git a/bcnn_amd/csrc/conv_window.hip b/bcnn_amd/csrc/conv_window.hip
--- a/bcnn_amd/csrc/conv_window.hip
+++ b/bcnn_amd/csrc/conv_window.hip
@@ -1,6 +1,7 @@
 #include "conv_paths.h"
 #include "lds_dma.h"
 
+#include <algorithm>
 #include <mutex>
 
 #ifndef WABL_FWD_R
@@ -936,37 +937,85 @@
     *blocks = ceil_div(total, *rpb);
 }
 
+static ConvShape dw_stem_part_shape(const ConvShape& s, int cnt) {
+    return make_conv_shape(cnt, s.C, s.H, s.W, s.F, s.ksz, s.stride, s.pad, s.groups);
+}
+static int dw_stem_parts_blocks(const ConvShape& s, int parts) {
+    int slots = 0;
+    for (int p = 0; p < parts; ++p) {
+        int n0, cnt, rpb, blocks;
+        tail_part_range(s.N, parts, p, &n0, &cnt);
+        dw_stem_plan(dw_stem_part_shape(s, cnt), &rpb, &blocks);
+        slots += blocks;
+    }
+    return slots;
+}
+
 size_t conv_dw_stem_workspace_floats(const ConvShape& s) {
     if (!dw_stem_ok(s)) return 0;
-    int rpb, blocks;
-    dw_stem_plan(s, &rpb, &blocks);
+    int blocks = dw_stem_parts_blocks(s, 1);
+    for (int parts = 2; parts <= kTailPartsMax && parts <= s.N; parts *= 2)
+        blocks = std::max(blocks, dw_stem_parts_blocks(s, parts));
     return (size_t)blocks * s.groups * 64 * kStemTapCols;
 }
 
-bool conv_backward_weights_stem(const float* x, const float* dy, float* dw, float* dbias, const ConvShape& s, float* workspace,
-                                size_t workspace_floats, bool* bias_done) {
-    if (!dw_stem_ok(s)) return false;
+bool conv_dw_stem_parts_ok(const ConvShape& s, int parts) { return dw_stem_ok(s) && parts >= 2 && parts <= kTailPartsMax && parts <= s.N; }
+
+static int dw_stem_launch(const float* x, const float* dy, const ConvShape& s, int n0, int cnt, float* workspace, int slot0,
+                          int bias_col) {
     ConvStemDwArgs a;
     int blocks;
-    dw_stem_plan(s, &a.rows_per_block, &blocks);
-    const size_t need = (size_t)blocks * s.groups * 64 * kStemTapCols;
-    conv_require_workspace(workspace, workspace_floats, need);
-    KTimer kt(K_CONV_DW, conv_gemm_flops(s), conv_gemm_bytes(s));
-    a.x = x; a.dy = dy; a.partials = workspace; a.s = s;
-    a.total_rows = s.N * s.OH;
-    a.bias_col = dbias ? 1 : 0;
+    a.s = cnt == s.N ? s : dw_stem_part_shape(s, cnt);
+    dw_stem_plan(a.s, &a.rows_per_block, &blocks);
+    a.x = x + (size_t)n0 * s.C * s.HW;
+    a.dy = dy + (size_t)n0 * s.F * s.OHOW;
+    a.partials = workspace + (size_t)slot0 * s.groups * 64 * kStemTapCols;
+    a.total_rows = cnt * s.OH;
+    a.bias_col = bias_col;
     const dim3 grid((unsigned)blocks, (unsigned)s.groups);
-    trace_kernel("conv_dw_stem_kernel");
     if (s.Cg == 1) conv_dw_stem_kernel<1, 120, 232><<<grid, 512, 0, current_stream()>>>(a);
     else if (s.Cg == 2) conv_dw_stem_kernel<2, 120, 232><<<grid, 512, 0, current_stream()>>>(a);
     else conv_dw_stem_kernel<3, 120, 232><<<grid, 512, 0, current_stream()>>>(a);
     KERNEL_CHECK();
-    const int total = s.groups * s.Mg * (s.K + a.bias_col);
-    conv_dw_stem_finalize_kernel<<<ceil_div(total, 16), 256, 0, current_stream()>>>(workspace, blocks, s.groups, s.Mg, s.K,
-                                                                                    a.bias_col, dw, dbias);
+    return blocks;
+}
+
+static void dw_stem_finalize(const ConvShape& s, const float* workspace, int slots, int bias_col, float* dw, float* dbias) {
+    const int total = s.groups * s.Mg * (s.K + bias_col);
+    conv_dw_stem_finalize_kernel<<<ceil_div(total, 16), 256, 0, current_stream()>>>(workspace, slots, s.groups, s.Mg, s.K,
+                                                                                    bias_col, dw, dbias);
     KERNEL_CHECK();
+}
+
+bool conv_backward_weights_stem(const float* x, const float* dy, float* dw, float* dbias, const ConvShape& s, float* workspace,
+                                size_t workspace_floats, bool* bias_done) {
+    if (!dw_stem_ok(s)) return false;
+    const size_t need = (size_t)dw_stem_parts_blocks(s, 1) * s.groups * 64 * kStemTapCols;
+    conv_require_workspace(workspace, workspace_floats, need);
+    KTimer kt(K_CONV_DW, conv_gemm_flops(s), conv_gemm_bytes(s));
+    trace_kernel("conv_dw_stem_kernel");
+    const int bias_col = dbias ? 1 : 0;
+    const int blocks = dw_stem_launch(x, dy, s, 0, s.N, workspace, 0, bias_col);
+    dw_stem_finalize(s, workspace, blocks, bias_col, dw, dbias);
     *bias_done = dbias != nullptr;
     return true;
+}
+
+void conv_backward_weights_stem_parts(const float* x, const float* dy, float* dw, const ConvShape& s, float* workspace,
+                                      size_t workspace_floats, int parts, void (*before_part)(int p)) {
+    const size_t need = (size_t)dw_stem_parts_blocks(s, parts) * s.groups * 64 * kStemTapCols;
+    conv_require_workspace(workspace, workspace_floats, need);
+    KTimer kt(K_CONV_DW, conv_gemm_flops(s), conv_gemm_bytes(s));
+    trace_kernel("conv_dw_stem_kernel");
+    int slots = 0;
+    for (int p = 0; p < parts; ++p) {
+        int n0, cnt;
+        tail_part_range(s.N, parts, p, &n0, &cnt);
+        before_part(p);
+        trace_kernel("conv_dw_stem_kernel:part");
+        slots += dw_stem_launch(x, dy, s, n0, cnt, workspace, slots, 0);
+    }
+    dw_stem_finalize(s, workspace, slots, 0, dw, nullptr);
 }
 
 static bool dw_window_ok(const ConvShape& s) { return window_ok(s) && (s.OW % 8) == 0; }
diff --git a/bcnn_amd/csrc/pool.hip b/bcnn_amd/csrc/pool.hip
--- a/bcnn_amd/csrc/pool.hip
+++ b/bcnn_amd/csrc/pool.hip
@@ -285,10 +285,10 @@
                                                                   const float* __restrict__ raw, float* __restrict__ dx,
                                                                   int C, int H, int W, int OH, int OW,
                                                                   const float4* __restrict__ consts, unsigned w4_magic,
-                                                                  float fM, float rfM, int act) {
+                                                                  float fM, float rfM, int act, int plane0) {
     const int W4 = W >> 2;
     const int t = blockIdx.x * 256 + threadIdx.x;
-    const int plane = blockIdx.y;
+    const int plane = plane0 + blockIdx.y;
     const bool live = t < H * W4;
     const int tt = live ? t : 0;
     const int h = W4 > 1 ? (int)__umulhi((unsigned)tt, w4_magic) : tt, k = tt - h * W4, w0 = k * 4;
@@ -435,10 +435,10 @@
            act_is_cheap(act) && act_bwd_is_cheap(act) && act != BCNN_HIP_ACT_PRELU;
 }
 
-void bcnn_hip_maxpool_bn_backward(const float* dpool, const int* indexes, const float* raw_at_max, const float* raw, float* dx,
-                                  int n, int c, int h, int w, int out_h, int out_w, int size, int stride, const float* scales,
-                                  float* dscales, const float* bias, float* dbias, const float* mean, const float* var,
-                                  float* dmean, float* dvar, int act) {
+void bcnn_hip_maxpool_bn_backward_parts(const float* dpool, const int* indexes, const float* raw_at_max, const float* raw, float* dx,
+                                        int n, int c, int h, int w, int out_h, int out_w, int size, int stride, const float* scales,
+                                        float* dscales, const float* bias, float* dbias, const float* mean, const float* var,
+                                        float* dmean, float* dvar, int act, int parts) {
     const long long total = (long long)n * c * h * w, ptotal = (long long)n * c * out_h * out_w;
     if (!total) return;
     if (!bcnn_hip_maxpool_bn_backward_fusable(n, c, h, w, out_h, out_w, size, stride, act, raw, dpool, indexes, dx) || !raw_at_max) {
@@ -453,13 +453,28 @@
                                 out_h * out_w, act != BCNN_HIP_ACT_NONE ? bias : nullptr, nullptr, 0u, consts, fM);
     }
     KTimer kt(K_POOL, 0.0, 4.0 * (2.0 * (double)total + 2.0 * (double)ptotal));
-    dim3 grid((unsigned)ceil_div(h * (w / 4), 256), (unsigned)(n * c));
     const unsigned w4 = (unsigned)(w / 4);
     trace_kernel("maxpool_bwd_pair_bn_kernel");
-    maxpool_bwd_pair_bn_kernel<<<grid, 256, 0, current_stream()>>>(dpool, indexes, raw, dx, c, h, w, out_h, out_w, consts,
-                                                                   w4 > 1 ? (unsigned)((0x100000000ULL + w4 - 1) / w4) : 0u, fM,
-                                                                   1.0f / fM, act);
-    KERNEL_CHECK();
+    if (parts < 1 || parts > kTailPartsMax || parts > n) parts = 1;
+    for (int p = 0; p < parts; ++p) {
+        int n0, cnt;
+        tail_part_range(n, parts, p, &n0, &cnt);
+        dim3 grid((unsigned)ceil_div(h * (w / 4), 256), (unsigned)(cnt * c));
+        if (parts > 1) trace_kernel("maxpool_bwd_pair_bn_kernel:part");
+        maxpool_bwd_pair_bn_kernel<<<grid, 256, 0, current_stream()>>>(dpool, indexes, raw, dx, c, h, w, out_h, out_w, consts,
+                                                                       w4 > 1 ? (unsigned)((0x100000000ULL + w4 - 1) / w4) : 0u, fM,
+                                                                       1.0f / fM, act, n0 * c);
+        KERNEL_CHECK();
+        if (parts > 1) conv_tail_part_record(p);
+    }
+}
+
+void bcnn_hip_maxpool_bn_backward(const float* dpool, const int* indexes, const float* raw_at_max, const float* raw, float* dx,
+                                  int n, int c, int h, int w, int out_h, int out_w, int size, int stride, const float* scales,
+                                  float* dscales, const float* bias, float* dbias, const float* mean, const float* var,
+                                  float* dmean, float* dvar, int act) {
+    bcnn_hip_maxpool_bn_backward_parts(dpool, indexes, raw_at_max, raw, dx, n, c, h, w, out_h, out_w, size, stride, scales, dscales,
+                                       bias, dbias, mean, var, dmean, dvar, act, 1);
 }
 
 void bcnn_hip_maxpool_backward(const float* dy, const int* indexes, float* dx, int n, int c, int h, int w,
diff --git a/bcnn_amd/host/bcnn_core.c b/bcnn_amd/host/bcnn_core.c
--- a/bcnn_amd/host/bcnn_core.c
+++ b/bcnn_amd/host/bcnn_core.c
@@ -548,16 +548,29 @@
     free(tab);
 }
 
+static int packs_beside(const bcnn_net *net) {
+    const bcnn_hip_context *hc = (const bcnn_hip_context *)net->hip_ctx;
+    return net->mode == BCNN_MODE_TRAIN && !(hc->no_side_stream || BCNN_EXP_ENV("BCNN_NO_SIDE_STREAM"));
+}
+
 void bcnn_forward(bcnn_net *net) {
     bcnn_hip_context *hc = hctx(net);
+    const int beside = packs_beside(net) && bcnn_hip_conv_prepack_side_begin();
     if (net->mode == BCNN_MODE_TRAIN) {
         if (hc->num_fill_chunks < 0) build_fill_table(net);
         bcnn_hip_zero_chunks((const bcnn_hip_fill_chunk *)hc->fill_chunks_gpu, hc->num_fill_chunks);
     }
     bcnn_drop_pending_gradients(net);
     bcnn_prepack_conv_weights(net, 0);
+    if (beside) {
+        bcnn_hip_conv_prepack_side_end();
+        if (net->num_nodes < 1 || net->nodes[0].type != BCNN_LAYER_CONV2D) bcnn_hip_conv_prepack_side_join();
+    }
     hc->in_pass = 1;
-    for (int i = 0; i < net->num_nodes; ++i) net->nodes[i].forward(net, &net->nodes[i]);
+    for (int i = 0; i < net->num_nodes; ++i) {
+        net->nodes[i].forward(net, &net->nodes[i]);
+        if (beside && i == 0) bcnn_hip_conv_prepack_side_join();
+    }
     hc->in_pass = 0;
     bcnn_hip_conv_prepack_discard();
 }
@@ -580,7 +593,9 @@
     bcnn_hip_context *hc = hctx(net);
     size_t ready_from = hc->arena_size;
     if (hc->comm_active) hc->comm_lo = hc->comm_hi = hc->arena_size;
+    const int beside = packs_beside(net) && bcnn_hip_conv_prepack_side_begin();
     bcnn_prepack_conv_weights(net, 1);
+    if (beside) bcnn_hip_conv_prepack_side_end();
     hc->in_pass = 2;
     const int side_prev = bcnn_hip_conv_side_stream_mode((hc->no_side_stream || BCNN_EXP_ENV("BCNN_NO_SIDE_STREAM")) ? 0 : 2);
     for (int i = net->num_nodes - 1; i >= 0; --i) {
diff --git a/bcnn_amd/host/bcnn_layers_hot.c b/bcnn_amd/host/bcnn_layers_hot.c
--- a/bcnn_amd/host/bcnn_layers_hot.c
+++ b/bcnn_amd/host/bcnn_layers_hot.c
@@ -211,14 +211,18 @@
         bcnn_maxpool_param *mp = (bcnn_maxpool_param *)pn->param;
         const bcnn_tensor *py = &net->tensors[pn->dst[0]];
         p->pool_bwd_pending = 0;
-        bcnn_hip_maxpool_bn_backward(py->grad_data_gpu, mp->indexes_gpu, mp->raw_at_max_gpu, p->bn_workspace_gpu,
-                                     io.y->grad_data_gpu, io.y->n, io.y->c, io.y->h, io.y->w, py->h, py->w, mp->size,
-                                     mp->stride, io.scales->data_gpu, io.scales->grad_data_gpu, io.b->data_gpu,
-                                     io.b->grad_data_gpu, p->saved_mean.data_gpu, p->saved_variance.data_gpu,
-                                     p->saved_mean.grad_data_gpu, p->saved_variance.grad_data_gpu, (int)p->activation);
-        bcnn_hip_conv_backward_bn_done(xin, io.w->data_gpu, io.y->grad_data_gpu, io.x->grad_data_gpu,
-                                       io.w->grad_data_gpu, io.x->n, io.x->c, io.x->h, io.x->w, p->num, p->size, p->stride,
-                                       p->pad, p->num_groups, p->conv_workspace_gpu, hctx(net)->workspace_size);
+        const int parts = io.x->grad_data_gpu ? 1 : bcnn_hip_conv_tail_parts(io.x->n, io.x->c, io.x->h, io.x->w, p->num, p->size,
+                                                                            p->stride, p->pad, p->num_groups);
+        bcnn_hip_maxpool_bn_backward_parts(py->grad_data_gpu, mp->indexes_gpu, mp->raw_at_max_gpu, p->bn_workspace_gpu,
+                                           io.y->grad_data_gpu, io.y->n, io.y->c, io.y->h, io.y->w, py->h, py->w, mp->size,
+                                           mp->stride, io.scales->data_gpu, io.scales->grad_data_gpu, io.b->data_gpu,
+                                           io.b->grad_data_gpu, p->saved_mean.data_gpu, p->saved_variance.data_gpu,
+                                           p->saved_mean.grad_data_gpu, p->saved_variance.grad_data_gpu, (int)p->activation,
+                                           parts);
+        bcnn_hip_conv_backward_bn_done_parts(xin, io.w->data_gpu, io.y->grad_data_gpu, io.x->grad_data_gpu,
+                                             io.w->grad_data_gpu, io.x->n, io.x->c, io.x->h, io.x->w, p->num, p->size,
+                                             p->stride, p->pad, p->num_groups, p->conv_workspace_gpu,
+                                             hctx(net)->workspace_size, parts);
         return;
     }
     if (hctx(net)->in_pass == 2 && p->elt_node >= 0 && ((bcnn_eltwise_param *)net->nodes[p->elt_node].param)->deferred) {
diff --git a/include/bcnn_hip.h b/include/bcnn_hip.h
--- a/include/bcnn_hip.h
+++ b/include/bcnn_hip.h
@@ -126,6 +126,10 @@
 void bcnn_hip_conv_prepack(const bcnn_hip_conv_desc *layers, int count, int data_gradient);
 void bcnn_hip_conv_prepack_reset(void);
 void bcnn_hip_conv_prepack_discard(void);
+int bcnn_hip_conv_prepack_side_mode(int enable);
+int bcnn_hip_conv_prepack_side_begin(void);
+void bcnn_hip_conv_prepack_side_end(void);
+void bcnn_hip_conv_prepack_side_join(void);
 
 void bcnn_hip_maxpool_forward(const float *x_d, float *y_d, int *indexes_d, int n, int c, int h, int w,
                               int out_h, int out_w, int size, int stride);
@@ -178,6 +182,16 @@
 void bcnn_hip_conv_backward_bn_done(const float *x_d, const float *w_d, float *dy_d, float *dx_d, float *dw_d, int n, int c,
                                     int h, int w, int f, int k, int stride, int pad, int groups, float *workspace_d,
                                     size_t workspace_elems);
+int bcnn_hip_conv_tail_parts_mode(int parts);
+int bcnn_hip_conv_tail_parts(int n, int c, int h, int w, int f, int k, int stride, int pad, int groups);
+void bcnn_hip_maxpool_bn_backward_parts(const float *dpool_d, const int *indexes_d, const float *raw_at_max_d,
+                                        const float *raw_d, float *dx_d, int n, int c, int h, int w, int out_h, int out_w,
+                                        int size, int stride, const float *scales_d, float *dscales_d, const float *bias_d,
+                                        float *dbias_d, const float *saved_mean_d, const float *saved_var_d, float *dmean_d,
+                                        float *dvar_d, int act, int parts);
+void bcnn_hip_conv_backward_bn_done_parts(const float *x_d, const float *w_d, float *dy_d, float *dx_d, float *dw_d, int n,
+                                          int c, int h, int w, int f, int k, int stride, int pad, int groups,
+                                          float *workspace_d, size_t workspace_elems, int parts);
 void bcnn_hip_avgpool_forward(const float *x_d, float *y_d, int n, int c, int h, int w);
 void bcnn_hip_avgpool_backward(const float *dy_d, float *dx_d, int n, int c, int h, int w);
 
```

After: 13890 images/s. About the same (-0.1%).
